# dschleef/schroedinger

Hardware: AMD Instinct MI355X
Metric: Mpix/s IIWT+OBMC decode, 2160p s16 (higher is better)
Workload: dtype s16

## Files before the change

schroedinger_amd/csrc/obmc.hip:

```cpp

#include "schro_hip_internal.h"
#include "obmc_common.h"
#include <algorithm>

namespace schro {
namespace {

constexpr int kThreads = 256;
constexpr int kTW = 64, kTH = 4;

template < int PC, bool SIMPLE >
__global__ __launch_bounds__ (kThreads)
void obmc_kernel (const ObmcJob * __restrict__ jobs, int njobs, uint32_t * __restrict__ overflow)
{
  __shared__ int s_wx[kMaxBlk], s_wy[kMaxBlk];

  const int bid = xcd_tile_id (blockIdx.x, gridDim.x);
  const ObmcJob job = jobs[find_job (jobs, njobs, bid)];
  const int t = bid - job.tile_base;
  const int tx = t % job.tiles_x, ty = t / job.tiles_x;
  const int tid = threadIdx.x;

  if (tid < job.xblen)
    s_wx[tid] = obmc_weight_1d (tid, job.xblen, job.xoff);
  if (tid >= 64 && tid - 64 < job.yblen)
    s_wy[tid - 64] = obmc_weight_1d (tid - 64, job.yblen, job.yoff);
  __syncthreads ();

  const int px = tx * kTW + (tid % kTW);
  const int py = ty * kTH + (tid / kTW);
  if (px >= job.w || py >= job.h)
    return;

  int bi[2], wxs[2], nx = 0;
  {
    int u = px + job.xoff;
    int i0 = u / job.xbsep, r = u - i0 * job.xbsep;
    int wa = 0, wb = 0;
    bool has_a = (r < 2 * job.xoff) && (i0 - 1 >= 0) && (i0 - 1 < job.nbx);
    bool has_b = (i0 < job.nbx);
    if (r < 2 * job.xoff) {
      wa = s_wx[r + job.xbsep];
      wb = s_wx[r];
      if (!has_a) { wb += wa; }
      if (!has_b) { wa += wb; }
    } else {
      wb = 8;
    }
    if (has_a) { bi[nx] = i0 - 1; wxs[nx] = wa; nx++; }
    if (has_b) { bi[nx] = i0; wxs[nx] = wb; nx++; }
  }
  int bj[2], wys[2], ny = 0;
  {
    int u = py + job.yoff;
    int j0 = u / job.ybsep, r = u - j0 * job.ybsep;
    int wa = 0, wb = 0;
    bool has_a = (r < 2 * job.yoff) && (j0 - 1 >= 0) && (j0 - 1 < job.nby);
    bool has_b = (j0 < job.nby);
    if (r < 2 * job.yoff) {
      wa = s_wy[r + job.ybsep];
      wb = s_wy[r];
      if (!has_a) { wb += wa; }
      if (!has_b) { wa += wb; }
    } else {
      wb = 8;
    }
    if (has_a) { bj[ny] = j0 - 1; wys[ny] = wa; ny++; }
    if (has_b) { bj[ny] = j0; wys[ny] = wb; ny++; }
  }

  const int prec = job.prec;
  const int expx = 32 << prec;
  const int max_fast_x = (job.w - job.xblen) * (1 << prec);
  const int max_fast_y = (job.h - job.yblen) * (1 << prec);
  const int wsum = job.w1 + job.w2;
  const bool noscale = (wsum == (1 << job.wbits));

  int acc = 0;
  for (int b = 0; b < ny; b++) {
    for (int a = 0; a < nx; a++) {
      const int i = bi[a], jj = bj[b];
      const uint8_t *mvp = job.mvs + (size_t) 20 * ((size_t) jj * job.nbx + i);
      const uint32_t flags = gload < uint32_t > (mvp);
      const uint32_t v01 = gload < uint32_t > (mvp + 12);
      const uint32_t v23 = gload < uint32_t > (mvp + 16);
      const int mode = flags & 3;
      const bool interior = i >= 1 && i < job.max_x_blocks && jj >= 1 && jj < job.max_y_blocks;
      const int bx = job.xbsep * i - job.xoff, by = job.ybsep * jj - job.yoff;
      const int wgt = wxs[a] * wys[b];
      int pred;

      if (mode == 0) {
        int dc = job.comp == 0 ? (int16_t) (v01 & 0xffff)
            : job.comp == 1 ? (int16_t) (v01 >> 16) : (int16_t) (v23 & 0xffff);
        pred = interior ? (int) (int16_t) (dc + 128) : (int) (uint8_t) (dc + 128);
        if (overflow && (unsigned) pred > 255u)
          __hip_atomic_store (overflow, 1u, __ATOMIC_RELAXED, __HIP_MEMORY_SCOPE_SYSTEM);
      } else {
        int val[2] = { 0, 0 };
#pragma unroll
        for (int r = 0; r < 2; r++) {
          if (!(mode & (r + 1)))
            continue;
          int dx = r == 0 ? (int16_t) (v01 & 0xffff) : (int16_t) (v01 >> 16);
          int dy = r == 0 ? (int16_t) (v23 & 0xffff) : (int16_t) (v23 >> 16);
          dx >>= job.mv_shift_x;
          dy >>= job.mv_shift_y;
          int fx = clampi (bx * (1 << prec) + dx, -expx, max_fast_x + expx - 1);
          int fy = clampi (by * (1 << prec) + dy, -expx, max_fast_y + expx - 1);
          int sx = fx + (px - bx) * (1 << prec);
          int sy = fy + (py - by) * (1 << prec);
          val[r] = fetch_ref < PC > (job.ref[r], job.ref_stride[r], job.w, job.h, sx, sy, prec, job.ref_ps, job.ref_cb);
        }
        if (mode == 3) {
          if constexpr (SIMPLE) {
            pred = (val[0] + val[1] + 1) >> 1;
          } else if (interior) {
            int16_t t1 = (int16_t) (val[0] * (int16_t) (job.w1 << (6 - job.wbits)));
            int16_t t2 = (int16_t) (val[1] * (int16_t) (job.w2 << (6 - job.wbits)));
            t1 = (int16_t) (t1 + t2);
            t1 = (int16_t) (t1 + 32);
            pred = (int16_t) (t1 >> 6);
          } else {
            int16_t t1 = (int16_t) (val[0] * job.w1);
            int16_t t2 = (int16_t) (val[1] * job.w2);
            t1 = (int16_t) (t1 + t2);
            t1 = (int16_t) (t1 + (int16_t) ((1 << job.wbits) >> 1));
            t1 = (int16_t) (t1 >> job.wbits);
            pred = clampi (t1, 0, 255);
          }
        } else {
          int s = val[mode - 1];
          if constexpr (SIMPLE) {
            pred = s;
          } else if (interior) {
            int16_t t1 = (int16_t) (s * (int16_t) (wsum << (6 - job.wbits)));
            t1 = (int16_t) (t1 + 32);
            pred = (int16_t) (t1 >> 6);
          } else if (noscale) {
            pred = s;
          } else {
            pred = (uint8_t) ((s * wsum + (1 << (job.wbits - 1))) >> job.wbits);
          }
        }
      }
      acc += pred * wgt;
    }
  }

  if (job.out_s16) {
    const int16_t t = (int16_t) ((int16_t) ((int16_t) acc - 8160) >> 6);
    gstore < int16_t > ((int16_t *) (job.out + (size_t) py * job.out_stride) + px, t);
    return;
  }
  int16_t t1 = (int16_t) ((int16_t) acc + 32);
  t1 = (int16_t) (t1 >> 6);
  int16_t res;
  if (!job.residual)
    res = 0;
  else if (job.res_bpp == 2)
    res = gload < int16_t > ((const int16_t *) ((const char *) job.residual
            + (size_t) py * job.residual_stride) + px);
  else
    res = (int16_t) gload < int32_t > ((const int32_t *) ((const char *) job.residual
            + (size_t) py * job.residual_stride) + px);
  t1 = (int16_t) (res + t1);
  gstore < uint8_t > (job.out + (size_t) py * job.out_stride + px, (uint8_t) clampi (t1, 0, 255));
}


constexpr int kFTW = 128, kFTH = 32;


constexpr int kAccStride = 136;

struct BlkInfo {
  int bx, by;
  int mode_dc;
  int fx[2], fy[2];
  int off[2];
  uint32_t wpk[2];
  int pad;
};

template < int PC >
__device__ __forceinline__ void
fetch4_inside (const uint8_t * __restrict__ p, int stride, uint32_t wpk, int *val)
{
  if constexpr (PC == 0) {
    uint32_t v = gload < u32_u > (p);
    val[0] = v & 0xff;
    val[1] = (v >> 8) & 0xff;
    val[2] = (v >> 16) & 0xff;
    val[3] = v >> 24;
  } else if constexpr (PC == 1) {
    const u32x2 q = gload < u32x2_u > (p);
    const uint64_t v = q.x | ((uint64_t) q.y << 32);
    val[0] = (int) (v & 0xff);
    val[1] = (int) ((v >> 16) & 0xff);
    val[2] = (int) ((v >> 32) & 0xff);
    val[3] = (int) ((v >> 48) & 0xff);
  } else {
    const u32x2 a = gload < u32x2_u > (p), b = gload < u32x2_u > (p + stride);
    const uint32_t alo = a.x, ahi = a.y, blo = b.x, bhi = b.y;
    val[0] = (int) (__builtin_amdgcn_udot4 (__builtin_amdgcn_perm (blo, alo, 0x05040100u), wpk, 8u, false) >> 4);
    val[1] = (int) (__builtin_amdgcn_udot4 (__builtin_amdgcn_perm (blo, alo, 0x07060302u), wpk, 8u, false) >> 4);
    val[2] = (int) (__builtin_amdgcn_udot4 (__builtin_amdgcn_perm (bhi, ahi, 0x05040100u), wpk, 8u, false) >> 4);
    val[3] = (int) (__builtin_amdgcn_udot4 (__builtin_amdgcn_perm (bhi, ahi, 0x07060302u), wpk, 8u, false) >> 4);
  }
}

constexpr int kAccMargin = 4;

struct TileCtx {
  int x_lo, x_hi, y_lo, y_hi;
  int xfold_hi, yfold_hi;
};

__device__ __forceinline__ void
acc_add_wrap (int *word, int high, int value)
{
  unsigned int old = __hip_atomic_load ((unsigned int *) word, __ATOMIC_RELAXED, __HIP_MEMORY_SCOPE_WORKGROUP), assumed;
  do {
    assumed = old;
    const unsigned int upd = high ? (assumed & 0xffffu) | ((assumed + ((unsigned int) value << 16)) & 0xffff0000u)
        : (assumed & 0xffff0000u) | ((assumed + (unsigned int) value) & 0xffffu);
    old = atomicCAS ((unsigned int *) word, assumed, upd);
  } while (old != assumed);
}

template < int PC >
__device__ __forceinline__ void
obmc_item_slow (const ObmcJob & job, const BlkInfo & bi, int row, int seg, const TileCtx & tc,
    const int *s_wx, const int *s_wy, int *acc, bool exact)
{
  const int prec = job.prec;
  const int y = bi.by + row, xs = bi.bx + 4 * seg;
  const int md = bi.mode_dc, mode = md & 3;
  int pred[4];
  if (mode == 0) {
    pred[0] = pred[1] = pred[2] = pred[3] = md >> 8;
  } else {
    int val[2][4];
    for (int r = 0; r < 2; r++) {
      if (!(mode & (r + 1)))
        continue;
      if constexpr (PC == 2) {
        const int sx = bi.fx[r] + 4 * seg * (1 << prec), sy = bi.fy[r] + row * (1 << prec);
        const int x8 = prec == 2 ? sx * 2 : sx, y8 = prec == 2 ? sy * 2 : sy;
        const int hx = x8 >> 2, hy = y8 >> 2, rx = x8 & 3, ry = y8 & 3;
        const int Y0 = clampi (hy, 0, 2 * job.h - 2), Y1 = clampi (hy + 1, 0, 2 * job.h - 2);
        int p[2][9];
#pragma unroll
        for (int j = 0; j < 9; j++) {
          const int X = clampi (hx + j, 0, 2 * job.w - 2);
          p[0][j] = gload < uint8_t > (job.ref[r] + hp_offset (X, Y0, job.ref_stride[r], job.ref_ps, job.ref_cb));
          p[1][j] = gload < uint8_t > (job.ref[r] + hp_offset (X, Y1, job.ref_stride[r], job.ref_ps, job.ref_cb));
        }
#pragma unroll
        for (int e = 0; e < 4; e++) {
          const int v = (4 - ry) * ((4 - rx) * p[0][2 * e] + rx * p[0][2 * e + 1])
              + ry * ((4 - rx) * p[1][2 * e] + rx * p[1][2 * e + 1]);
          val[r][e] = (v + 8) >> 4;
        }
      } else {
        for (int e = 0; e < 4; e++)
          val[r][e] = fetch_ref < PC > (job.ref[r], job.ref_stride[r], job.w, job.h,
              bi.fx[r] + (4 * seg + e) * (1 << prec), bi.fy[r] + row * (1 << prec), prec, job.ref_ps, job.ref_cb);
      }
    }
    for (int e = 0; e < 4; e++)
      pred[e] = mode == 3 ? (val[0][e] + val[1][e] + 1) >> 1 : (mode == 1 ? val[0][e] : val[1][e]);
  }
  int wy = s_wy[row];
  if (y < job.yoff)
    wy += s_wy[2 * job.yoff - row - 1];
  if (y >= tc.yfold_hi)
    wy += s_wy[2 * (job.yblen - job.yoff) - row - 1];
  const int yrel = y - tc.y_lo;
  int *arow = acc + (yrel & (kFTH / 2 - 1)) * kAccStride + kAccMargin - tc.x_lo;
  for (int e = 0; e < 4; e++) {
    const int x = xs + e, idx = 4 * seg + e;
    if (idx >= job.xblen)
      continue;
    int wx = s_wx[idx];
    if (x < job.xoff)
      wx += s_wx[2 * job.xoff - idx - 1];
    if (x >= tc.xfold_hi)
      wx += s_wx[2 * (job.xblen - job.xoff) - idx - 1];
    if (exact)
      acc_add_wrap (arow + x, yrel & (kFTH / 2), pred[e] * wx * wy);
    else
      atomicAdd (arow + x, (pred[e] * wx * wy) << (yrel & (kFTH / 2)));
  }
}

__device__ __forceinline__ void
obmc_finish (const ObmcJob & job, const int *acc, int tid, int x_lo, int y_lo, int x_hi, int y_hi)
{
  typedef short s16x2 __attribute__ ((ext_vector_type (2)));
  if (job.out_s16) {
    for (int it = tid; it < kFTH * kFTW; it += kThreads) {
      const int xx = it % kFTW, yy = it / kFTW;
      const int x = x_lo + xx, y = y_lo + yy;
      if (y >= y_hi || x >= x_hi)
        continue;
      const int a = acc[(yy & (kFTH / 2 - 1)) * kAccStride + kAccMargin + xx] >> (yy & (kFTH / 2));
      gstore < int16_t > ((int16_t *) (job.out + (size_t) y * job.out_stride) + x, (int16_t) ((int16_t) ((int16_t) a - 8160) >> 6));
    }
    return;
  }
  const bool fast = job.res_bpp == 2 && x_hi - x_lo == kFTW
      && ((((uintptr_t) job.residual) | (uintptr_t) job.residual_stride) & 15) == 0
      && ((((uintptr_t) job.out) | (uintptr_t) job.out_stride) & 7) == 0;
  if (fast) {
    for (int it = tid; it < (kFTH / 2) * (kFTW / 8); it += kThreads) {
      const int g = it & (kFTW / 8 - 1), yy = it >> 4;
      static_assert (kFTW / 8 == 16, "8-pixel groups per tile row");
      const int x = x_lo + 8 * g;
      const int4 *ap = reinterpret_cast < const int4 * >(acc + yy * kAccStride + kAccMargin + 8 * g);
      const int4 a0 = ap[0], a1 = ap[1];
#pragma unroll
      for (int half = 0; half < 2; half++) {
        const int y = y_lo + yy + half * (kFTH / 2);
        if (y >= y_hi)
          continue;
        const uint32_t sel = half ? 0x07060302u : 0x05040100u;
        const u32x4 r = job.residual ? gload < u32x4 > ((const char *) job.residual + (size_t) y * job.residual_stride + 2 * x)
            : (u32x4) { 0u, 0u, 0u, 0u };
        const uint32_t av[4] = {
          __builtin_amdgcn_perm ((uint32_t) a0.y, (uint32_t) a0.x, sel),
          __builtin_amdgcn_perm ((uint32_t) a0.w, (uint32_t) a0.z, sel),
          __builtin_amdgcn_perm ((uint32_t) a1.y, (uint32_t) a1.x, sel),
          __builtin_amdgcn_perm ((uint32_t) a1.w, (uint32_t) a1.z, sel)
        };
        const uint32_t rv[4] = { r.x, r.y, r.z, r.w };
        uint32_t t[4];
#pragma unroll
        for (int k = 0; k < 4; k++) {
          s16x2 v = (__builtin_bit_cast (s16x2, av[k]) + (short) 32) >> 6;
          v = v + __builtin_bit_cast (s16x2, rv[k]);
          v = __builtin_elementwise_min (__builtin_elementwise_max (v, (s16x2) (short) 0), (s16x2) (short) 255);
          t[k] = __builtin_bit_cast (uint32_t, v);
        }
        u32x2 o;
        o.x = __builtin_amdgcn_perm (t[1], t[0], 0x06040200u);
        o.y = __builtin_amdgcn_perm (t[3], t[2], 0x06040200u);
        gstore < u32x2 > (job.out + (size_t) y * job.out_stride + x, o);
      }
    }
    return;
  }
  for (int it = tid; it < kFTH * kFTW / 4; it += kThreads) {
    const int g = it % (kFTW / 4), yy = it / (kFTW / 4);
    const int x = x_lo + 4 * g, y = y_lo + yy;
    if (y >= y_hi || x >= x_hi)
      continue;
    const int *ap = acc + (yy & (kFTH / 2 - 1)) * kAccStride + kAccMargin + 4 * g;
    const int hs = yy & (kFTH / 2);
    const int av[4] = { ap[0] >> hs, ap[1] >> hs, ap[2] >> hs, ap[3] >> hs };
    const char *rrow = (const char *) job.residual + (size_t) y * job.residual_stride;
    uint8_t *orow = job.out + (size_t) y * job.out_stride + x;
    __attribute__ ((aligned (8))) int16_t res[4];
    const bool full = x + 4 <= job.w;
    if (!job.residual) {
      res[0] = res[1] = res[2] = res[3] = 0;
    } else if (job.res_bpp == 2) {
      const int16_t *rp = (const int16_t *) rrow + x;
      if (full && (((uintptr_t) rp) & 7) == 0) {
        *reinterpret_cast < u32x2 * >(res) = gload < u32x2 > (rp);
      } else {
        for (int e = 0; e < 4; e++)
          res[e] = x + e < job.w ? gload < int16_t > (rp + e) : (int16_t) 0;
      }
    } else {
      const int32_t *rp = (const int32_t *) rrow + x;
      for (int e = 0; e < 4; e++)
        res[e] = x + e < job.w ? (int16_t) gload < int32_t > (rp + e) : (int16_t) 0;
    }
    uint32_t pk = 0;
#pragma unroll
    for (int e = 0; e < 4; e++) {
      int16_t t1 = (int16_t) ((int16_t) av[e] + 32);
      t1 = (int16_t) (t1 >> 6);
      t1 = (int16_t) (res[e] + t1);
      pk |= (uint32_t) clampi (t1, 0, 255) << (8 * e);
    }
    if (full && (((uintptr_t) orow) & 3) == 0) {
      gstore < uint32_t > (orow, pk);
    } else {
      for (int e = 0; e < 4 && x + e < job.w; e++)
        gstore < uint8_t > (orow + e, (uint8_t) (pk >> (8 * e)));
    }
  }
}


constexpr int kItemBlkCap = 192;
constexpr int kItemCap = 1536;
constexpr int kItemWCap = 256;

struct __attribute__ ((aligned (16))) HotBlk {
  int y, x;
  int mode_dc;
  int rows;
  int off[2];
  uint32_t wpk[2];
  int ya[2];
};

struct ItemLane {
  int slot, seg;
  int seg_bytes;
  int tw3;
  bool active;
};

template < int PC >
__device__ __forceinline__ void
hp_predict4 (const ObmcJob & job, int r, int off_r, int ya, int row, int seg, uint32_t wpk, int *val)
{
  static_assert (PC >= 1, "plain references are linear");
  const int stride = job.ref_stride[r];
  const int ps = job.ref_ps;
  const int xp = ((off_r & 0xffff) + 4 * seg) << ps, px = (off_r >> 16) & 1, py = (off_r >> 17) & 1;
  const int y = ya + row;
  const uint32_t pick = job.ref_cb ? 0x07050301u : 0x06040200u;
  auto load4 = [&](const uint8_t * p) {
    if (ps) {
      const u32x2 q = gload < u32x2_u > (p);
      return __builtin_amdgcn_perm (q.y, q.x, pick);
    }
    return gload < u32_u > (p);
  };
  const uint8_t *a = job.ref[r] + hp_row_offset (y, stride) + hp_col_offset (xp) + (px + 2 * py) * 128;
  const uint32_t A = load4 (a);
  if constexpr (PC == 1) {
    val[0] = A & 0xff;
    val[1] = (A >> 8) & 0xff;
    val[2] = (A >> 16) & 0xff;
    val[3] = A >> 24;
    (void) wpk;
  } else {
    const int dB = px ? (1 << ps) - 128 : 128;
    const uint8_t *c = job.ref[r] + hp_row_offset (y + py, stride) + hp_col_offset (xp) + (px + 2 * (py ^ 1)) * 128;
    const uint32_t B = load4 (a + dB), C = load4 (c), D = load4 (c + dB);
#pragma unroll
    for (int e = 0; e < 4; e++) {
      const uint32_t sel = 0x0c0c0000u | (uint32_t) e | ((uint32_t) (4 + e) << 8);
      const uint32_t t = __builtin_amdgcn_perm (B, A, sel), u = __builtin_amdgcn_perm (D, C, sel);
      val[e] = (int) (__builtin_amdgcn_udot4 (__builtin_amdgcn_perm (u, t, 0x05040100u), wpk, 8u, false) >> 4);
    }
  }
}

template < int PC, int CLS, bool EXACT >
__device__ __forceinline__ void
item_pass (const ObmcJob & job, const ItemLane & il, const uint16_t * s_item, const HotBlk * s_hot,
    const uint32_t * s_w4, int nseg, int *acc, int i0, int hi)
{
  constexpr int kStep = PC == 0 ? 1 : 2;
  const int it = i0 + il.slot;
  const int e = s_item[min (it, hi - 1)];
  const HotBlk & hb = s_hot[e & 0xff];
  const int row = e >> 8;
  const int yrel = hb.y + row, xrel = hb.x + 4 * il.seg;
  const uint32_t w4 = s_w4[__umul24 (row, nseg) + il.seg];
  int v0[4], v1[4];
  if constexpr (CLS == 3) {
    v0[0] = v0[1] = v0[2] = v0[3] = v1[0] = v1[1] = v1[2] = v1[3] = hb.mode_dc >> 8;
  } else {
    constexpr int r0 = CLS == 2 ? 1 : 0;
    if constexpr (PC == 0) {
      fetch4_inside < PC > (job.ref[r0] + (hb.off[r0] + (row * kStep) * job.ref_stride[r0] + il.seg_bytes),
          job.ref_stride[r0], hb.wpk[r0], v0);
      if constexpr (CLS == 0)
        fetch4_inside < PC > (job.ref[1] + (hb.off[1] + (row * kStep) * job.ref_stride[1] + il.seg_bytes),
            job.ref_stride[1], hb.wpk[1], v1);
    } else {
      hp_predict4 < PC > (job, r0, hb.off[r0], hb.ya[r0], row, il.seg, hb.wpk[r0], v0);
      if constexpr (CLS == 0)
        hp_predict4 < PC > (job, 1, hb.off[1], hb.ya[1], row, il.seg, hb.wpk[1], v1);
    }
    if constexpr (CLS != 0) {
#pragma unroll
      for (int k = 0; k < 4; k++)
        v1[k] = v0[k];
    }
  }
  if (il.active && it < hi && (unsigned) (xrel + 3) < (unsigned) il.tw3) {
    int *ap = acc + (__umul24 (yrel & (kFTH / 2 - 1), kAccStride) + kAccMargin + xrel);
    const int hs = yrel & (kFTH / 2);
    static_assert (kFTH / 2 == 16, "the high half of an accumulator word is bit 16 up");
#pragma unroll
    for (int k = 0; k < 4; k++) {
      const int pred = CLS == 0 ? (v0[k] + v1[k] + 1) >> 1 : v0[k];
      const int v = __mul24 (pred, (int) ((w4 >> (8 * k)) & 0xff));
      if constexpr (EXACT)
        acc_add_wrap (ap + k, hs, v);
      else
        atomicAdd (ap + k, v << hs);
    }
  }
}

template < int PC, int CLS >
__device__ __forceinline__ void
item_class (const ObmcJob & job, const ItemLane & il, const uint16_t * s_item, const HotBlk * s_hot,
    const uint32_t * s_w4, int nseg, int *acc, int first, int hi, int stride, bool exact)
{
  if (exact) {
    for (int i0 = first; i0 < hi; i0 += stride)
      item_pass < PC, CLS, true > (job, il, s_item, s_hot, s_w4, nseg, acc, i0, hi);
  } else {
    for (int i0 = first; i0 < hi; i0 += stride)
      item_pass < PC, CLS, false > (job, il, s_item, s_hot, s_w4, nseg, acc, i0, hi);
  }
}

template < int PC >
__global__ __launch_bounds__ (kThreads) __attribute__ ((amdgpu_waves_per_eu (5, 5)))
void obmc_item_kernel (const ObmcJob * __restrict__ jobs, int njobs, const uint32_t * __restrict__ order,
    uint32_t * __restrict__ overflow)
{
  __shared__ __attribute__ ((aligned (16))) int acc[(kFTH / 2) * kAccStride];
  __shared__ int s_wx[kMaxBlk], s_wy[kMaxBlk];
  __shared__ HotBlk s_hot[kItemBlkCap];
  __shared__ uint16_t s_item[kItemCap];
  __shared__ uint32_t s_w4[kItemWCap];
  __shared__ uint16_t s_start[kThreads + 2];
  __shared__ int s_cnt[8];
  __shared__ int s_wide;

  const int bid = xcd_tile_id (blockIdx.x, gridDim.x);
  const uint32_t entry = order ? __builtin_amdgcn_readfirstlane (gload < uint32_t > (order + bid)) : 0u;
  const ObmcJob job = jobs[order ? (int) (entry >> 16) : find_job (jobs, njobs, bid)];
  const int t = order ? (int) (entry & 0xffffu) : bid - job.tile_base;
  const int ty = mdiv (t, job.tiles_x, job.m_tiles_x), tx = t - ty * job.tiles_x;
  const int tid = threadIdx.x, lane = tid & 63, wave = tid >> 6;
  const int x_lo = tx * kFTW, y_lo = ty * kFTH;
  const int x_hi = min (x_lo + kFTW, job.w), y_hi = min (y_lo + kFTH, job.h);

  static_assert (((kFTH / 2) * kAccStride) % 4 == 0, "accumulator tile is cleared 16 bytes at a time");
  for (int it = tid; it < (kFTH / 2) * kAccStride / 4; it += kThreads)
    reinterpret_cast < int4 * >(acc)[it] = make_int4 (0, 0, 0, 0);
  if (tid < job.xblen)
    s_wx[tid] = obmc_weight_1d (tid, job.xblen, job.xoff);
  if (tid >= 64 && tid - 64 < job.yblen)
    s_wy[tid - 64] = obmc_weight_1d (tid - 64, job.yblen, job.yoff);

  const int xblen = job.xblen, yblen = job.yblen, xbsep = job.xbsep, ybsep = job.ybsep;
  const int xoff = job.xoff, yoff = job.yoff, prec = job.prec;
  const int i_lo = max (0, mdiv (x_lo + xoff - xblen + 2 * xbsep, xbsep, job.m_xbsep) - 1);
  const int i_hi = min (job.nbx - 1, mdiv (x_hi - 1 + xoff, xbsep, job.m_xbsep));
  const int j_lo = max (0, mdiv (y_lo + yoff - yblen + 2 * ybsep, ybsep, job.m_ybsep) - 1);
  const int j_hi = min (job.nby - 1, mdiv (y_hi - 1 + yoff, ybsep, job.m_ybsep));
  const int nbi = i_hi - i_lo + 1, nbj = j_hi - j_lo + 1;
  const int nblk = nbi > 0 && nbj > 0 ? nbi * nbj : 0;
  const uint32_t m_nbi = nbi > 1 && nbi <= 1024 ? kDivMagic.m[nbi] : 0u;
  const int xfold_hi = job.nbx * xbsep - xoff, yfold_hi = job.nby * ybsep - yoff;
  const int gw = PC == 0 ? job.w - 1 : 2 * job.w - 2;
  const int gh = PC == 0 ? job.h - 1 : 2 * job.h - 2;
  constexpr int kStep = PC == 0 ? 1 : 2;
  const int nseg = job.nseg, lpi = job.lpi;
  const int IPW = job.ipw, chunk_cap = job.chunk_cap;
  ItemLane il;
  il.slot = mdiv (lane, lpi, job.m_lpi);
  const int sub = lane - il.slot * lpi;
  il.seg = min (sub, nseg - 1);
  il.seg_bytes = il.seg * (4 * kStep);
  il.tw3 = x_hi - x_lo + 3;
  il.active = il.slot < IPW && sub < nseg;
  TileCtx tc;
  tc.x_lo = x_lo;
  tc.x_hi = x_hi;
  tc.y_lo = y_lo;
  tc.y_hi = y_hi;
  tc.xfold_hi = xfold_hi;
  tc.yfold_hi = yfold_hi;
  __syncthreads ();
  for (int i = tid; i < yblen * nseg && i < kItemWCap; i += kThreads) {
    const int r = mdiv (i, nseg, job.m_nseg), sg = i - r * nseg;
    uint32_t w = 0;
#pragma unroll
    for (int k = 0; k < 4; k++)
      if (4 * sg + k < xblen)
        w |= (uint32_t) (s_wx[4 * sg + k] * s_wy[r]) << (8 * k);
    s_w4[i] = w;
  }

  bool exact = false;
  for (int chunk0 = 0; chunk0 < nblk; chunk0 += chunk_cap) {
    const int nb = min (chunk_cap, nblk - chunk0);
    if (tid < 8)
      s_cnt[tid] = 0;
    if (tid == 8)
      s_wide = 0;
    __syncthreads ();
    HotBlk info;
    int key = 0, rank = 0;
    const bool have = tid < nb;
    if (have) {
      const int blk = chunk0 + tid;
      const int bj = nbi == 1 ? blk : nbi <= 1024 ? (int) __umulhi ((uint32_t) blk, m_nbi) : blk / nbi;
      const int i = i_lo + (blk - bj * nbi), jj = j_lo + bj;
      const uint8_t *mvp = job.mvs + (size_t) 20 * ((size_t) jj * job.nbx + i);
      const uint32_t flags = gload < uint32_t > (mvp);
      const uint32_t v01 = gload < uint32_t > (mvp + 12);
      const uint32_t v23 = gload < uint32_t > (mvp + 16);
      const int bx = xbsep * i - xoff, by = ybsep * jj - yoff;
      info.x = bx - x_lo;
      info.y = by - y_lo;
      const int mode = flags & 3;
      const bool interior = i >= 1 && i < job.max_x_blocks && jj >= 1 && jj < job.max_y_blocks;
      int dc = job.comp == 0 ? (int16_t) (v01 & 0xffff)
          : job.comp == 1 ? (int16_t) (v01 >> 16) : (int16_t) (v23 & 0xffff);
      int p = interior ? (int) (int16_t) (dc + 128) : (int) (uint8_t) (dc + 128);
      int md = mode | (p << 8);
#pragma unroll
      for (int r = 0; r < 2; r++) {
        int fx, fy;
        mv_origin (job, bx, by, v01, v23, r, &fx, &fy);
        int gx0, gy0, gx1, gy1;
        uint32_t wpk = 0;
        if constexpr (PC == 2) {
          const int x8 = prec == 2 ? fx * 2 : fx, y8 = prec == 2 ? fy * 2 : fy;
          const int rx = x8 & 3, ry = y8 & 3;
          gx0 = x8 >> 2;
          gy0 = y8 >> 2;
          gx1 = gx0 + 2 * (nseg * 4 - 1) + 1;
          gy1 = gy0 + 2 * (yblen - 1) + 1;
          wpk = (uint32_t) ((4 - ry) * (4 - rx)) | ((uint32_t) ((4 - ry) * rx) << 8)
              | ((uint32_t) (ry * (4 - rx)) << 16) | ((uint32_t) (ry * rx) << 24);
        } else {
          gx0 = fx;
          gy0 = fy;
          gx1 = gx0 + kStep * (nseg * 4 - 1);
          gy1 = gy0 + kStep * (yblen - 1);
        }
        bool inside = gx0 >= 0 && gy0 >= 0 && gx1 <= gw && gy1 <= gh;
        if (!inside)
          md |= 4 << r;
        if constexpr (PC == 0) {
          info.off[r] = inside ? gy0 * job.ref_stride[r] + gx0 : 0;
          info.ya[r] = 0;
        } else {
          info.off[r] = inside ? ((gx0 >> 1) + kHpApron) | ((gx0 & 1) << 16) | ((gy0 & 1) << 17) : 0;
          info.ya[r] = inside ? gy0 >> 1 : 0;
        }
        info.wpk[r] = wpk;
      }
      info.mode_dc = md;
      const int ra = max (0, -info.y), rb = min (yblen, y_hi - by);
      info.rows = ra | ((rb - ra) << 8);
      const bool clamped = ((md >> 2) & md & 3) != 0;
      const bool fold = by < yoff || by + yblen > yfold_hi || bx < xoff || bx + nseg * 4 > xfold_hi;
      const bool wide_dc = mode == 0 && (unsigned) p > 255u;
      if (wide_dc) {
        s_wide = 1;
        if (overflow)
          __hip_atomic_store (overflow, 1u, __ATOMIC_RELAXED, __HIP_MEMORY_SCOPE_SYSTEM);
      }
      key = (clamped || fold || wide_dc || yblen * nseg > kItemWCap) ? 4 : (mode == 3 ? 0 : (mode == 0 ? 3 : mode));
      if (key == 4) {
        int fx, fy;
        mv_origin (job, bx, by, v01, v23, 0, &fx, &fy);
        info.off[0] = fx;
        info.off[1] = fy;
        mv_origin (job, bx, by, v01, v23, 1, &fx, &fy);
        info.wpk[0] = (uint32_t) fx;
        info.wpk[1] = (uint32_t) fy;
      }
      rank = atomicAdd (&s_cnt[key], 1);
    }
    __syncthreads ();
    if (s_wide && !exact) {
      exact = true;
      if (chunk0 > 0) {
        __syncthreads ();
        for (int it = tid; it < (kFTH / 2) * kAccStride / 4; it += kThreads)
          reinterpret_cast < int4 * >(acc)[it] = make_int4 (0, 0, 0, 0);
        chunk0 = -chunk_cap;
        continue;
      }
    }
    int cbase[6];
    cbase[0] = 0;
#pragma unroll
    for (int k = 0; k < 5; k++)
      cbase[k + 1] = cbase[k] + s_cnt[k];
    if (have) {
      int base = 0;
#pragma unroll
      for (int k = 0; k < 5; k++)
        base = key == k ? cbase[k] : base;
      s_hot[base + rank] = info;
    }
    __syncthreads ();
    int nrows = tid < cbase[4] ? ((s_hot[tid].rows >> 8) & 0xff) : 0, incl = nrows;
#pragma unroll
    for (int d = 1; d < 64; d <<= 1) {
      const int up = __shfl_up (incl, d);
      if (lane >= d)
        incl += up;
    }
    if (lane == 63)
      s_cnt[4 + wave] = incl;
    __syncthreads ();
    {
#pragma unroll
      for (int w = 0; w < kThreads / 64 - 1; w++)
        incl += wave > w ? s_cnt[4 + w] : 0;
      const int start = incl - nrows;
      s_start[tid] = (uint16_t) start;
      if (tid == kThreads - 1)
        s_start[kThreads] = (uint16_t) incl;
      if (tid < cbase[4]) {
        const int ra = s_hot[tid].rows & 0xff;
        for (int r = 0; r < nrows; r++)
          s_item[start + r] = (uint16_t) (tid | ((ra + r) << 8));
      }
    }
    __syncthreads ();

    const int first = wave * IPW, stride = (kThreads / 64) * IPW;
    item_class < PC, 0 > (job, il, s_item, s_hot, s_w4, nseg, acc, s_start[cbase[0]] + first, s_start[cbase[1]], stride, exact);
    item_class < PC, 1 > (job, il, s_item, s_hot, s_w4, nseg, acc, s_start[cbase[1]] + first, s_start[cbase[2]], stride, exact);
    item_class < PC, 2 > (job, il, s_item, s_hot, s_w4, nseg, acc, s_start[cbase[2]] + first, s_start[cbase[3]], stride, exact);
    item_class < PC, 3 > (job, il, s_item, s_hot, s_w4, nseg, acc, s_start[cbase[3]] + first, s_start[cbase[4]], stride, exact);

    {
      const int per_block = yblen * nseg;
      const uint32_t m_per_block = div_magic (per_block);
      const int nslow = cbase[5] - cbase[4];
      for (int item = tid; item < nslow * per_block; item += kThreads) {
        const int b = mdiv (item, per_block, m_per_block);
        const int rem = item - b * per_block;
        const int r2 = mdiv (rem, nseg, job.m_nseg), s2 = rem - r2 * nseg;
        const HotBlk & hb = s_hot[cbase[4] + b];
        BlkInfo bi;
        bi.bx = hb.x + x_lo;
        bi.by = hb.y + y_lo;
        const int y = bi.by + r2, xs = bi.bx + 4 * s2;
        if (y < y_lo || y >= y_hi || xs + 3 < x_lo || xs >= x_hi)
          continue;
        bi.mode_dc = hb.mode_dc;
        bi.fx[0] = hb.off[0];
        bi.fy[0] = hb.off[1];
        bi.fx[1] = (int) hb.wpk[0];
        bi.fy[1] = (int) hb.wpk[1];
        obmc_item_slow < PC > (job, bi, r2, s2, tc, s_wx, s_wy, acc, exact);
      }
    }
  }
  __syncthreads ();
  obmc_finish (job, acc, tid, x_lo, y_lo, x_hi, y_hi);
}

template < int PC >
int
launch_one (hipStream_t stream, const ObmcJob * d_jobs, int njobs, int total_tiles, int variant,
    const uint32_t * d_order, uint32_t * overflow)
{
  static const int lds_pad = SCHRO_ENV ("SCHRO_HIP_OBMC_LDS_PAD") ? atoi (SCHRO_ENV ("SCHRO_HIP_OBMC_LDS_PAD")) : 0;
  if (variant == 1)
    SCHRO_LAUNCH ((obmc_item_kernel < PC >), dim3 (total_tiles), dim3 (kThreads), lds_pad, stream,
        d_jobs, njobs, d_order, overflow);
  else
    SCHRO_LAUNCH ((obmc_kernel < PC, false >), dim3 (total_tiles), dim3 (kThreads), 0,
        stream, d_jobs, njobs, overflow);
  hipError_t e = hipGetLastError ();
  if (e != hipSuccess)
    return set_error (SCHRO_HIP_EDEVICE, "obmc launch: %s", hipGetErrorString (e));
  return 0;
}

}

void
obmc_item_geometry (ObmcJob * j)
{
  const int nseg = (j->xblen + 3) >> 2;
  const int lpi = nseg;
  j->nseg = nseg;
  j->lpi = lpi;
  j->ipw = 64 / lpi;
  j->chunk_cap = std::min (kItemBlkCap, kItemCap / std::min (j->yblen, kFTH));
  j->m_tiles_x = div_magic (j->tiles_x);
  j->m_xbsep = div_magic (j->xbsep);
  j->m_ybsep = div_magic (j->ybsep);
  j->m_nseg = div_magic (nseg);
  j->m_lpi = div_magic (lpi);
  j->m_xramp = div_magic (2 * j->xoff - 1);
  j->m_yramp = div_magic (2 * j->yoff - 1);
}

void
obmc_tiles (int variant, int w, int h, int xoff, int *tiles_x, int *tiles_y)
{
  (void) xoff;
  if (variant >= 1) {
    const int tw = variant >= 3 ? obmc_row_tile_width (variant == 4) : kFTW;
    const int th = variant >= 3 ? obmc_row_tile_height () : kFTH;
    *tiles_x = (w + tw - 1) / tw;
    *tiles_y = (h + th - 1) / th;
  } else {
    *tiles_x = (w + kTW - 1) / kTW;
    *tiles_y = (h + kTH - 1) / kTH;
  }
}

int
launch_obmc (hipStream_t stream, const ObmcJob * d_jobs, int njobs, int total_tiles, int prec,
    int variant, const uint32_t * d_order, uint32_t * overflow)
{
  switch (prec == 0 ? 0 : (prec == 1 ? 1 : 2)) {
    case 0: return launch_one < 0 > (stream, d_jobs, njobs, total_tiles, variant, d_order, overflow);
    case 1: return launch_one < 1 > (stream, d_jobs, njobs, total_tiles, variant, d_order, overflow);
    default: return launch_one < 2 > (stream, d_jobs, njobs, total_tiles, variant, d_order, overflow);
  }
}

}
```

schroedinger_amd/csrc/obmc_row.hip:

```cpp

#include "obmc_row_body.h"

namespace schro {
namespace {

SCHRO_ROW_KERNEL (obmc_row_kernel_2_1, 6, 2, 1)
SCHRO_ROW_KERNEL (obmc_row_kernel_2_2, 6, 2, 2)
SCHRO_ROW_KERNEL (obmc_row_kernel_3_1, 7, 3, 1)
SCHRO_ROW_KERNEL (obmc_row_kernel_3_2, 5, 3, 2)
SCHRO_ROW_KERNEL (obmc_row_kernel_4_1, 6, 4, 1)
SCHRO_ROW_KERNEL (obmc_row_kernel_4_2, 5, 4, 2)
SCHRO_ROW_KERNEL (obmc_row_kernel_uv_2, 5, 2, 1, true)
SCHRO_ROW_KERNEL (obmc_row_kernel_uv_3, 7, 3, 1, true)
SCHRO_ROW_KERNEL (obmc_row_kernel_uv_4, 6, 4, 1, true)
SCHRO_ROW_KERNEL (obmc_row_kernel_p_2_1, 6, 2, 1, false, kRTH, true)
SCHRO_ROW_KERNEL (obmc_row_kernel_p_3_1, 8, 3, 1, false, kRTH, true)
#ifdef SCHRO_HIP_EXPERIMENTS
SCHRO_ROW_KERNEL (obmc_row_kernel_p_3_1_pad, 8, 3, 1, false, kRTH, true, 1, 1, false, true)
#endif
SCHRO_ROW_KERNEL (obmc_row_kernel_p_4_1, 7, 4, 1, false, kRTH, true)
SCHRO_ROW_KERNEL (obmc_row_kernel_p_uv_2, 5, 2, 1, true, kRTH, true)
SCHRO_ROW_KERNEL (obmc_row_kernel_p_uv_3, 8, 3, 1, true, kRTH, true)
SCHRO_ROW_KERNEL (obmc_row_kernel_p_uv_4, 7, 4, 1, true, kRTH, true)
SCHRO_ROW_KERNEL (obmc_row_kernel_h2_3_1, 6, 3, 1, false, kRTH, false, 1, 2)
SCHRO_ROW_KERNEL (obmc_row_kernel_h2_uv_3, 6, 3, 1, true, kRTH, false, 1, 2)
SCHRO_ROW_KERNEL (obmc_row_kernel_p_h2_3_1, 7, 3, 1, false, kRTH, true, 1, 2)
SCHRO_ROW_KERNEL (obmc_row_kernel_p_h2_uv_3, 6, 3, 1, true, kRTH, true, 1, 2)
SCHRO_ROW_KERNEL (obmc_row_kernel_h2_4_1, 5, 4, 1, false, kRTH, false, 1, 2)
SCHRO_ROW_KERNEL (obmc_row_kernel_h2_uv_4, 5, 4, 1, true, kRTH, false, 1, 2)
SCHRO_ROW_KERNEL (obmc_row_kernel_p_h2_4_1, 6, 4, 1, false, kRTH, true, 1, 2)
SCHRO_ROW_KERNEL (obmc_row_kernel_p_h2_uv_4, 6, 4, 1, true, kRTH, true, 1, 2)

SCHRO_ROW_KERNEL (obmc_row_kernel_w_3_1, 6, 3, 1, false, kRTH, false, 1, 1, true)
SCHRO_ROW_KERNEL (obmc_row_kernel_w_uv_3, 6, 3, 1, true, kRTH, false, 1, 1, true)
SCHRO_ROW_KERNEL (obmc_row_kernel_w_p_3_1, 7, 3, 1, false, kRTH, true, 1, 1, true)
SCHRO_ROW_KERNEL (obmc_row_kernel_w_p_uv_3, 7, 3, 1, true, kRTH, true, 1, 1, true)
SCHRO_ROW_KERNEL (obmc_row_kernel_w_2_1, 5, 2, 1, false, kRTH, false, 1, 1, true)
SCHRO_ROW_KERNEL (obmc_row_kernel_w_4_1, 6, 4, 1, false, kRTH, false, 1, 1, true)
SCHRO_ROW_KERNEL (obmc_row_kernel_w_uv_2, 5, 2, 1, true, kRTH, false, 1, 1, true)
SCHRO_ROW_KERNEL (obmc_row_kernel_w_uv_4, 6, 4, 1, true, kRTH, false, 1, 1, true)
SCHRO_ROW_KERNEL (obmc_row_kernel_w_h2_3_1, 6, 3, 1, false, kRTH, false, 1, 2, true)
SCHRO_ROW_KERNEL (obmc_row_kernel_w_h2_uv_3, 6, 3, 1, true, kRTH, false, 1, 2, true)
SCHRO_ROW_KERNEL (obmc_row_kernel_w_h2_4_1, 6, 4, 1, false, kRTH, false, 1, 2, true)
SCHRO_ROW_KERNEL (obmc_row_kernel_w_h2_uv_4, 6, 4, 1, true, kRTH, false, 1, 2, true)

constexpr RowEntry kHalf[] = {
  ROW_ENTRY (obmc_row_kernel_2_1), ROW_ENTRY (obmc_row_kernel_2_2), ROW_ENTRY (obmc_row_kernel_3_1), ROW_ENTRY (obmc_row_kernel_3_2),
  ROW_ENTRY (obmc_row_kernel_4_1), ROW_ENTRY (obmc_row_kernel_4_2),
  ROW_ENTRY (obmc_row_kernel_uv_2), ROW_ENTRY (obmc_row_kernel_uv_3), ROW_ENTRY (obmc_row_kernel_uv_4),
  ROW_ENTRY (obmc_row_kernel_p_2_1), ROW_ENTRY (obmc_row_kernel_p_3_1), ROW_ENTRY (obmc_row_kernel_p_4_1),
  ROW_ENTRY (obmc_row_kernel_p_uv_2), ROW_ENTRY (obmc_row_kernel_p_uv_3), ROW_ENTRY (obmc_row_kernel_p_uv_4),
  ROW_ENTRY (obmc_row_kernel_h2_3_1), ROW_ENTRY (obmc_row_kernel_h2_uv_3), ROW_ENTRY (obmc_row_kernel_p_h2_3_1), ROW_ENTRY (obmc_row_kernel_p_h2_uv_3),
  ROW_ENTRY (obmc_row_kernel_h2_4_1), ROW_ENTRY (obmc_row_kernel_h2_uv_4), ROW_ENTRY (obmc_row_kernel_p_h2_4_1), ROW_ENTRY (obmc_row_kernel_p_h2_uv_4),
  ROW_ENTRY (obmc_row_kernel_w_3_1), ROW_ENTRY (obmc_row_kernel_w_uv_3), ROW_ENTRY (obmc_row_kernel_w_p_3_1), ROW_ENTRY (obmc_row_kernel_w_p_uv_3),
  ROW_ENTRY (obmc_row_kernel_w_2_1), ROW_ENTRY (obmc_row_kernel_w_4_1), ROW_ENTRY (obmc_row_kernel_w_uv_2), ROW_ENTRY (obmc_row_kernel_w_uv_4),
  ROW_ENTRY (obmc_row_kernel_w_h2_3_1), ROW_ENTRY (obmc_row_kernel_w_h2_uv_3), ROW_ENTRY (obmc_row_kernel_w_h2_4_1), ROW_ENTRY (obmc_row_kernel_w_h2_uv_4),
};
constexpr RowTable kHalfTable = { kHalf, (int) std::size (kHalf) };
static_assert (row_table_ok (kHalfTable, 1), "obmc_row.hip: one kernel per form");
static_assert (row_find (kHalfTable, RowForm { 1, 3, 1, 2, true, true }) == obmc_row_kernel_w_h2_3_1
    && row_find (kHalfTable, RowForm { 1, 2, 2, 1, true, false }) == obmc_row_kernel_2_2 && !row_find (kHalfTable, RowForm { 1, 3, 2, 1, false, true }),
    "obmc_row.hip: a prediction_only launch without a kernel of its form takes the residual form's; no kernel of two weighted planes");

}

RowTable
obmc_row_table_half ()
{
  return kHalfTable;
}

static RowKernel
row_kernel (const RowForm & f)
{
#ifdef SCHRO_HIP_EXPERIMENTS
  static const bool pad = SCHRO_ENV ("SCHRO_HIP_OBMC_PAD") && atoi (SCHRO_ENV ("SCHRO_HIP_OBMC_PAD")) != 0;
  if (pad && f == obmc_row_kernel_p_3_1_pad_form)
    return obmc_row_kernel_p_3_1_pad;
#endif
  return row_find (f.kind == 0 ? obmc_row_table_plain () : f.kind == 3 ? obmc_row_table_eighth () : obmc_row_table_half (), f);
}

bool
obmc_row_has_kernel (const RowForm & form)
{
  return row_kernel (form) != nullptr;
}

int
launch_obmc_row (hipStream_t stream, const ObmcJob * d_jobs, int njobs, int total_tiles, const RowForm & form,
    const uint32_t * d_order, uint32_t * overflow, const uint32_t * d_wtabs)
{
  const RowKernel k = row_kernel (form);
  if (!k)
    return set_error (SCHRO_HIP_EINVAL, "obmc (row): reference kind %d, %d dwords per row x %d segments x %d planes unsupported", form.kind,
        form.nd, form.ns, form.np);
  static const int lds_pad = SCHRO_ENV ("SCHRO_HIP_OBMC_LDS_PAD") ? atoi (SCHRO_ENV ("SCHRO_HIP_OBMC_LDS_PAD")) : 0;
  SCHRO_LAUNCH (k, dim3 (total_tiles), dim3 (kRThreads), (size_t) lds_pad, stream, d_jobs, njobs, d_order, overflow, d_wtabs);
  hipError_t e = hipGetLastError ();
  if (e != hipSuccess)
    return set_error (SCHRO_HIP_EDEVICE, "obmc (row) launch: %s", hipGetErrorString (e));
  return 0;
}

struct RowCaps {
  int tw, blk, item;
};
template < int ND, bool UV, int NS > constexpr RowCaps kRowCaps = { RowGeo < ND, UV, NS >::kTW, RowGeo < ND, UV, NS >::kBlk, RowGeo < ND, UV, NS >::kItem };
template < bool UV, int NS > constexpr RowCaps kRowCapsNd[3] = { kRowCaps < 2, UV, NS >, kRowCaps < 3, UV, NS >, kRowCaps < 4, UV, NS > };
static RowCaps
row_caps (int nd, int ns, bool uv)
{
  static constexpr const RowCaps *caps[2][2] = { { kRowCapsNd < false, 1 >, kRowCapsNd < false, 2 > }, { kRowCapsNd < true, 1 >, kRowCapsNd < true, 2 > } };
  return caps[uv][ns - 1][nd - 2];
}

RowForm
obmc_row_form (const ObmcJob & j, bool uv, bool nores)
{
  const int ps = uv ? 1 : 0;
  int ns = 1;
  if (j.ref_ps != (j.prec == 0 ? 0 : ps))
    return {};
  if (j.prec < 0 || j.prec > 3 || (j.xblen & 1) || j.xblen < 2 || j.yblen > 32)
    return {};
  if (j.w1 < 0 || j.w2 < 0 || j.wbits < 0 || j.wbits > 6 || j.w1 + j.w2 != (1 << j.wbits))
    return {};
  int seg_bytes = j.xblen << ps;
  if (seg_bytes > 16) {
    if (seg_bytes > 32 || (seg_bytes & 3))
      return {};
    ns = 2;
    seg_bytes /= 2;
  }
  if (((std::max (j.w, j.h) + 32) << j.prec) > 32767)
    return {};
  if (j.prec == 0) {
    if (((((uintptr_t) j.ref[0]) | ((uintptr_t) j.ref[1])) & 3) || ((j.ref_stride[0] | j.ref_stride[1]) & 3) || j.ref_stride[0] < j.w
        || j.ref_stride[1] < j.w || j.w < 4)
      return {};
    if (uv && (!j.ref_b[0] || !j.ref_b[1] || ((((uintptr_t) j.ref_b[0]) | ((uintptr_t) j.ref_b[1])) & 3)))
      return {};
  } else {
    if ((((uintptr_t) j.ref[0]) | ((uintptr_t) j.ref[1])) & 127)
      return {};
    if (((j.ref_stride[0] | j.ref_stride[1]) & 511) || j.ref_stride[0] < hp_chunks (j.w, ps) * 512 || j.ref_stride[1] < hp_chunks (j.w, ps) * 512)
      return {};
  }
  const int need = (seg_bytes + 3) / 4, nd = need <= 2 ? 2 : need;
  const RowForm form = { j.prec == 0 ? 0 : j.prec == 3 ? 3 : 1, nd, uv ? 3 : 1, ns, nores, j.w1 != 1 || j.wbits != 1 };
  if (!row_kernel (form))
    return {};
  const RowCaps caps = row_caps (nd, ns, uv);
  if ((long long) ((j.w + caps.tw - 1) / caps.tw) * ((j.h + kRTH - 1) / kRTH) > 0xffff)
    return {};
  const int nbi = ((caps.tw - 1 + j.xblen - 1) / j.xbsep + 1) * ns, nbj = (kRTH - 1 + j.yblen - 1) / j.ybsep + 1;
  const int rows_col = std::min (kRTH * ((j.yblen + j.ybsep - 1) / j.ybsep), kRTH + (kRTH / j.ybsep + 2) * 2 * j.yoff);
  if (nbi > 255 || nbi * nbj > caps.blk || nbi * rows_col > caps.item)
    return {};
  return form;
}

int
obmc_row_weight_words (int nd, int ns)
{
  const int wrow = 2 * nd * ns;
  return 32 * wrow + 4 * (ns == 1 ? 8 : wrow) + 128 + (ns == 1 ? 16 : 32) + 32;
}
static_assert (RowGeo < 3, false, 2 >::kWTab == 32 * 12 + 48 + 128 + 32 + 32 && RowGeo < 4, true, 2 >::kWTab == 32 * 16 + 64 + 128 + 32 + 32
    && RowGeo < 3, true >::kWTab == 64 * 3 + 32 + 128 + 16 + 32, "obmc_row_weight_words");

void
obmc_row_weight_table (const ObmcJob & j, int nd, int ns, bool uv, uint32_t * out)
{
  auto ramp = [](int x, int offset) { return offset == 1 ? (x == 0 ? 3 : 5) : 1 + (6 * x + offset - 1) / (2 * offset - 1); };
  auto weight = [&](int i, int blen, int offset) {
    if (offset == 0)
      return 8;
    if (i < 2 * offset)
      return ramp (i, offset);
    if (blen - 1 - i < 2 * offset)
      return ramp (blen - 1 - i, offset);
    return 8;
  };
  const int wrow = 2 * nd * ns, xf = ns == 1 ? 8 : wrow, wxn = ns == 1 ? 16 : 32;
  int wx[32] = { 0 }, wy[32] = { 0 };
  for (int i = 0; i < j.xblen && i < wxn; i++)
    wx[i] = weight (i, j.xblen, j.xoff);
  for (int i = 0; i < j.yblen && i < 32; i++)
    wy[i] = weight (i, j.yblen, j.yoff);
  auto folded = [](const int *w1, int idx, int blen, int bsep, int off, int type) {
    if (idx >= blen)
      return 0;
    int w = w1[idx];
    if ((type & 1) && idx < 2 * off)
      w += w1[2 * off - idx - 1];
    if ((type & 2) && idx >= bsep)
      w += w1[2 * (blen - off) - idx - 1];
    return w;
  };
  const int wcap = 32 * wrow;
  const int seg_words = ns == 1 ? wrow : 2 * nd, seg_units = ns == 1 ? (uv ? j.xblen : j.xblen >> 1) : (uv ? j.xblen / 2 : j.xblen >> 2);
  auto unit_of = [&](int pr) {
    const int seg = pr / seg_words, q = pr - seg * seg_words;
    return q < seg_units ? seg * seg_units + q : -1;
  };
  for (int i = 0; i < wcap; i++) {
    const int r = i / wrow, u = unit_of (i - r * wrow);
    uint32_t v = 0;
    if (r < j.yblen && u >= 0) {
      if (uv)
        v = (uint32_t) (wx[u] * wy[r]) * 0x00010001u;
      else
        v = (uint32_t) (wx[2 * u] * wy[r]) | ((uint32_t) (wx[2 * u + 1] * wy[r]) << 16);
    }
    out[i] = v;
  }
  for (int t = 0; t < 4 * xf; t++) {
    const int type = t / xf, pr = t - type * xf;
    const int u = ns == 1 ? pr : unit_of (pr);
    out[wcap + t] = u < 0 ? 0u : uv ? (uint32_t) folded (wx, u, j.xblen, j.xbsep, j.xoff, type) * 0x00010001u
        : (uint32_t) folded (wx, 2 * u, j.xblen, j.xbsep, j.xoff, type) | ((uint32_t) folded (wx, 2 * u + 1, j.xblen, j.xbsep, j.xoff, type) << 16);
  }
  const int fy = wcap + 4 * xf;
  for (int t = 0; t < 128; t++)
    out[fy + t] = (uint32_t) folded (wy, t & 31, j.yblen, j.ybsep, j.yoff, t >> 5);
  for (int i = 0; i < wxn; i++)
    out[fy + 128 + i] = (uint32_t) wx[i];
  for (int i = 0; i < 32; i++)
    out[fy + 128 + wxn + i] = (uint32_t) wy[i];
}

void
obmc_row_tile_record (const ObmcJob & j, bool uv, int ns, int tx, int ty, uint32_t * rec)
{
  const int tw = obmc_row_tile_width (uv);
  const int x_lo = tx * tw, y_lo = ty * kRTH, x_hi = std::min (x_lo + tw, j.w), y_hi = std::min (y_lo + kRTH, j.h);
  const int i_lo = std::max (0, (x_lo + j.xoff - j.xblen + 2 * j.xbsep) / j.xbsep - 1);
  const int i_hi = std::min (j.nbx - 1, (x_hi - 1 + j.xoff) / j.xbsep);
  const int j_lo = std::max (0, (y_lo + j.yoff - j.yblen + 2 * j.ybsep) / j.ybsep - 1);
  const int j_hi = std::min (j.nby - 1, (y_hi - 1 + j.yoff) / j.ybsep);
  const int nbi = std::max (0, std::min (255, (i_hi - i_lo + 1) * ns)), nbj = std::max (0, std::min (255, j_hi - j_lo + 1));
  const uint32_t m16 = nbi > 1 ? (65536u + (uint32_t) nbi - 1u) / (uint32_t) nbi : 0u;
  rec[0] = (uint32_t) x_lo | ((uint32_t) y_lo << 16);
  rec[1] = (uint32_t) i_lo | ((uint32_t) j_lo << 16);
  rec[2] = (uint32_t) nbi | ((uint32_t) nbj << 8) | (m16 << 16);
}

int
obmc_row_tile_height ()
{
  return kRTH;
}

int
obmc_row_tile_width (bool uv)
{
  return row_caps (3, 1, uv).tw;
}

}
```

schroedinger_amd/csrc/obmc_row_body.h:

```cpp

#pragma once

#include "schro_hip_internal.h"
#include "obmc_common.h"
#include <algorithm>
#include <cstdlib>

namespace schro {
namespace {

constexpr int kRThreads = 256;
constexpr int kRTH = 32;
template < int ND, bool UV, int NS = 1 > struct RowGeo {
  static constexpr int kTW = UV ? 64 : 128;
  static constexpr int kMargin = UV ? (ND <= 3 && NS == 1 ? 5 : 8) : (ND <= 2 ? 8 : 16);
  static constexpr int kAccW = UV ? (ND <= 3 && NS == 1 ? 75 : 81) : (ND <= 2 ? 73 : 85);
  static constexpr int kBlk = ND <= 2 ? 344 : (NS > 1 ? (UV ? 208 : 144) : UV ? (ND == 3 ? 180 : 192) : 128) * kRTH / 32,
      kItem = ND <= 2 ? 1792 : (NS > 1 ? 1664 : UV ? (ND == 3 ? 960 : 1152) : (ND == 3 ? 1024 : 1152)) * kRTH / 32;
  static constexpr int kWRow = 2 * ND * NS;
  static constexpr int kWCap = 32 * kWRow;
  static constexpr int kXF = NS == 1 ? 8 : kWRow, kWxN = NS == 1 ? 16 : 32;
  static constexpr bool kPadBlk = UV || ND > 2;
  static constexpr int kWFoldY = kWCap + 4 * kXF, kWRampX = kWFoldY + 128, kWRampY = kWRampX + kWxN;
  static constexpr int kWTab = kWRampY + 32;
};
constexpr int kRBoth = 0, kRRef0 = 1, kRRef1 = 2, kRDc = 3, kREdge = 4, kRRim = 5;
constexpr int kRSlots = 16 + 4 + 4 + 3;
__host__ __device__ constexpr int
row_slot_base (int cls)
{
  return cls == kRBoth ? 0 : cls == kRRef0 ? 16 : cls == kRRef1 ? 20 : cls == kRDc ? 24 : cls == kREdge ? 25 : 26;
}

typedef unsigned short u16x2 __attribute__ ((ext_vector_type (2)));
typedef short s16x2 __attribute__ ((ext_vector_type (2)));

struct __attribute__ ((aligned (4))) RowRef {
  int base;
  uint32_t ydb;
  int dci;
};

template < bool PAD > struct alignas (PAD ? 4 : 8) RowBlkT {
  int16_t y, x;
  uint32_t fr;
  RowRef r[2];
  uint32_t pad[PAD ? 1 : 0];
};
static_assert (sizeof (RowBlkT < true >) == 36 && sizeof (RowBlkT < false >) == 32, "block records: an odd number of words / r03's");

template < typename B >
__device__ __forceinline__ uint32_t
blk_flags (const B & hb)
{
  return hb.fr >> 16;
}

template < typename B >
__device__ __forceinline__ uint32_t
blk_ry (const B & hb, int r)
{
  return (hb.fr >> (16 + 6 + r)) & 1u;
}

template < typename B >
__device__ __forceinline__ int
blk_dc (const B & hb, int pl)
{
  return pl ? hb.r[0].base >> 16 : (int) (int16_t) hb.r[0].base;
}


struct __attribute__ ((aligned (8))) PlaneIO {
  const uint8_t *ref[2];
  const void *residual;
  uint8_t *out;
  int residual_stride, out_stride;
};

__device__ __forceinline__ uint32_t
lerp1 (uint32_t a, uint32_t b)
{
  return __builtin_amdgcn_lerp (a, b, 0x01010101u);
}

__device__ __forceinline__ void
acc_add_exact (uint32_t * word, int high, uint32_t value)
{
  unsigned int old = __hip_atomic_load (word, __ATOMIC_RELAXED, __HIP_MEMORY_SCOPE_WORKGROUP), assumed;
  do {
    assumed = old;
    const unsigned int upd = high ? (assumed & 0xffffu) | ((assumed + (value << 16)) & 0xffff0000u)
        : (assumed & 0xffff0000u) | ((assumed + value) & 0xffffu);
    old = atomicCAS (word, assumed, upd);
  } while (old != assumed);
}

template < typename G, bool UV >
__device__ __forceinline__ uint32_t *
acc_word (uint32_t * acc, int par, int x, int y, int *half)
{
  if constexpr (UV) {
    *half = 0;
    return acc + y * G::kAccW + (x + G::kMargin);
  } else {
    const int idx = x + G::kMargin + par;
    *half = idx & 1;
    return acc + y * G::kAccW + (idx >> 1);
  }
}

template < int ND > struct RawRun {
  uint32_t c[ND + 1];
  uint32_t sh;
};

#if defined (SCHRO_HIP_EXPERIMENTS) && defined (SCHRO_ROW_GATHER_AUX)
constexpr int kGatherAux = SCHRO_ROW_GATHER_AUX;
#else
constexpr int kGatherAux = 0;
#endif

template < int ND >
__device__ __forceinline__ void
issue_run (__amdgpu_buffer_rsrc_t ref, uint32_t off, RawRun < ND > &r)
{
  const uint32_t al = off & ~3u;
  r.sh = off & 3u;
  if constexpr (ND == 1) {
    const u32x2 q = __builtin_amdgcn_raw_buffer_load_b64 (ref, (int) al, 0, kGatherAux);
    r.c[0] = q.x;
    r.c[1] = q.y;
  } else if constexpr (ND == 2) {
    typedef uint32_t u32x3 __attribute__ ((ext_vector_type (3)));
    const u32x3 q = __builtin_amdgcn_raw_buffer_load_b96 (ref, (int) al, 0, kGatherAux);
    r.c[0] = q.x;
    r.c[1] = q.y;
    r.c[2] = q.z;
  } else if constexpr (ND == 3) {
    const u32x4 q = __builtin_amdgcn_raw_buffer_load_b128 (ref, (int) al, 0, kGatherAux);
    r.c[0] = q.x;
    r.c[1] = q.y;
    r.c[2] = q.z;
    r.c[3] = q.w;
  } else {
    const u32x4 q = __builtin_amdgcn_raw_buffer_load_b128 (ref, (int) al, 0, kGatherAux);
    const u32x2 q2 = __builtin_amdgcn_raw_buffer_load_b64 (ref, (int) al + 16, 0, kGatherAux);
    r.c[0] = q.x;
    r.c[1] = q.y;
    r.c[2] = q.z;
    r.c[3] = q.w;
    r.c[4] = q2.x;
  }
}

template < int ND >
__device__ __forceinline__ void
align_run (const RawRun < ND > &r, uint32_t * d)
{
#pragma unroll
  for (int k = 0; k < ND; k++)
    d[k] = __builtin_amdgcn_alignbyte (r.c[k + 1], r.c[k], r.sh);
}

__device__ __forceinline__ uint32_t
row_ofs (uint32_t y, uint32_t stride)
{
  return __umul24 (y >> 2, stride) + ((y & 3u) << 5);
}

template < int ND, bool ABS = false, bool W = false >
__device__ __forceinline__ void
predict_row (const ObmcJob & job, __amdgpu_buffer_rsrc_t ref, uint32_t stride, const RowRef & rr, uint32_t ry, int row, uint32_t * out)
{
  const int dB = (int) rr.ydb >> 16;
  uint32_t offA, offC = 0;
  bool any_b, any_c;
  if constexpr (ABS) {
    const int hy = (int) (int16_t) (rr.ydb & 0xffffu) + 2 * row, gh = 2 * job.h - 2;
    const uint32_t Y0 = (uint32_t) clampi (hy, 0, gh), Y1 = (uint32_t) clampi (hy + (int) ry, 0, gh);
    offA = (uint32_t) rr.base + ((Y0 & 1u) << 8) + row_ofs (Y0 >> 1, stride);
    offC = (uint32_t) rr.base + ((Y1 & 1u) << 8) + row_ofs (Y1 >> 1, stride);
    any_b = any_c = true;
  } else {
    const uint32_t y = (rr.ydb & 0xffffu) + (uint32_t) row;
    offA = (uint32_t) rr.base + row_ofs (y, stride);
    any_b = __ballot (dB != 0) != 0;
    any_c = __ballot ((W ? rr.dci & ~0xf0 : rr.dci) != 0) != 0;
    if (any_c)
      offC = (uint32_t) (rr.base + (rr.dci >> 16)) + row_ofs (y + ((uint32_t) rr.dci & 1u), stride);
  }
  RawRun < ND > qa, qb, qc, qd;
  issue_run < ND > (ref, offA, qa);
  if (any_b)
    issue_run < ND > (ref, offA + (uint32_t) dB, qb);
  if (any_c) {
    issue_run < ND > (ref, offC, qc);
    if (any_b)
      issue_run < ND > (ref, offC + (uint32_t) dB, qd);
  }
  uint32_t a[ND];
  align_run < ND > (qa, a);
  if constexpr (W) {
    const uint32_t rx = ((uint32_t) rr.dci >> 4) & 3u, rw = ((uint32_t) rr.dci >> 6) & 3u;
    const uint32_t w00 = (4u - rw) * (4u - rx), w01 = (4u - rw) * rx, w10 = rw * (4u - rx), w11 = rw * rx;
    uint32_t lo[ND], hi[ND];
#pragma unroll
    for (int k = 0; k < ND; k++) {
      lo[k] = __umul24 (__builtin_amdgcn_perm (0u, a[k], 0x0c010c00u), w00) + 0x00080008u;
      hi[k] = __umul24 (__builtin_amdgcn_perm (0u, a[k], 0x0c030c02u), w00) + 0x00080008u;
    }
    auto add_tap = [&] (const RawRun < ND > &q, uint32_t w) {
      uint32_t t[ND];
      align_run < ND > (q, t);
#pragma unroll
      for (int k = 0; k < ND; k++) {
        lo[k] += __umul24 (__builtin_amdgcn_perm (0u, t[k], 0x0c010c00u), w);
        hi[k] += __umul24 (__builtin_amdgcn_perm (0u, t[k], 0x0c030c02u), w);
      }
    };
    if (any_b)
      add_tap (qb, w01);
    if (any_c) {
      add_tap (qc, w10);
      if (any_b)
        add_tap (qd, w11);
    }
#pragma unroll
    for (int k = 0; k < ND; k++)
      out[k] = __builtin_amdgcn_perm (hi[k] >> 4, lo[k] >> 4, 0x06040200u);
    return;
  }
  if (!any_c) {
    if (!any_b) {
#pragma unroll
      for (int k = 0; k < ND; k++)
        out[k] = a[k];
    } else {
      uint32_t b[ND];
      align_run < ND > (qb, b);
#pragma unroll
      for (int k = 0; k < ND; k++)
        out[k] = lerp1 (a[k], b[k]);
    }
  } else if (!any_b) {
    uint32_t c[ND];
    align_run < ND > (qc, c);
#pragma unroll
    for (int k = 0; k < ND; k++)
      out[k] = lerp1 (a[k], c[k]);
  } else {
    uint32_t b[ND], c[ND], d[ND];
    align_run < ND > (qb, b);
    align_run < ND > (qc, c);
    align_run < ND > (qd, d);
#pragma unroll
    for (int k = 0; k < ND; k++) {
      const uint32_t h0 = lerp1 (a[k], b[k]), h1 = lerp1 (c[k], d[k]);
      out[k] = __builtin_amdgcn_lerp (h0, h1, ~((a[k] ^ b[k]) | (c[k] ^ d[k])));
    }
  }
}

template < int ND > struct TapRuns {
  RawRun < ND > qa, qb, qc, qd;
  bool any_b, any_c;
};

template < int ND >
__device__ __forceinline__ void
issue_taps (__amdgpu_buffer_rsrc_t ref, uint32_t stride, const RowRef & rr, int row, TapRuns < ND > &t)
{
  const int dB = (int) rr.ydb >> 16;
  const uint32_t y = (rr.ydb & 0xffffu) + (uint32_t) row;
  const uint32_t offA = (uint32_t) rr.base + row_ofs (y, stride);
  t.any_b = __ballot (dB != 0) != 0;
  t.any_c = __ballot (rr.dci != 0) != 0;
  issue_run < ND > (ref, offA, t.qa);
  if (t.any_b)
    issue_run < ND > (ref, offA + (uint32_t) dB, t.qb);
  if (t.any_c) {
    const uint32_t offC = (uint32_t) (rr.base + (rr.dci >> 16)) + row_ofs (y + ((uint32_t) rr.dci & 1u), stride);
    issue_run < ND > (ref, offC, t.qc);
    if (t.any_b)
      issue_run < ND > (ref, offC + (uint32_t) dB, t.qd);
  }
}

template < int ND >
__device__ __forceinline__ void
finish_taps (const TapRuns < ND > &t, uint32_t * out)
{
  uint32_t a[ND];
  align_run < ND > (t.qa, a);
  if (!t.any_c) {
    if (!t.any_b) {
#pragma unroll
      for (int k = 0; k < ND; k++)
        out[k] = a[k];
    } else {
      uint32_t b[ND];
      align_run < ND > (t.qb, b);
#pragma unroll
      for (int k = 0; k < ND; k++)
        out[k] = lerp1 (a[k], b[k]);
    }
  } else if (!t.any_b) {
    uint32_t c[ND];
    align_run < ND > (t.qc, c);
#pragma unroll
    for (int k = 0; k < ND; k++)
      out[k] = lerp1 (a[k], c[k]);
  } else {
    uint32_t b[ND], c[ND], d[ND];
    align_run < ND > (t.qb, b);
    align_run < ND > (t.qc, c);
    align_run < ND > (t.qd, d);
#pragma unroll
    for (int k = 0; k < ND; k++) {
      const uint32_t h0 = lerp1 (a[k], b[k]), h1 = lerp1 (c[k], d[k]);
      out[k] = __builtin_amdgcn_lerp (h0, h1, ~((a[k] ^ b[k]) | (c[k] ^ d[k])));
    }
  }
}

template < int ND >
__device__ __forceinline__ void
predict_row_plain (__amdgpu_buffer_rsrc_t ref, uint32_t stride, const RowRef & rr, int row, uint32_t * out)
{
  RawRun < ND > qa;
  issue_run < ND > (ref, (uint32_t) rr.base + __umul24 ((rr.ydb & 0xffffu) + (uint32_t) row, stride), qa);
  align_run < ND > (qa, out);
}

template < int ND >
__device__ __forceinline__ void
predict_row_plain_abs (const ObmcJob & job, __amdgpu_buffer_rsrc_t ref, uint32_t stride, const RowRef & rr, int row, uint32_t * out)
{
  const int Y = clampi ((int) (int16_t) (rr.ydb & 0xffffu) + row, 0, job.h - 1);
  const uint32_t rofs = __umul24 ((uint32_t) Y, stride);
  u32x2 q[ND];
  uint32_t sh[ND];
  int d[ND];
#pragma unroll
  for (int k = 0; k < ND; k++) {
    const int t = rr.base + 4 * k, xs = clampi (t, 0, job.w - 4);
    const uint32_t off = rofs + (uint32_t) xs;
    d[k] = t - xs;
    sh[k] = off & 3u;
    q[k] = __builtin_amdgcn_raw_buffer_load_b64 (ref, (int) (off & ~3u), 0, 0);
  }
#pragma unroll
  for (int k = 0; k < ND; k++) {
    const uint32_t v = __builtin_amdgcn_alignbyte (q[k].y, q[k].x, sh[k]);
    const uint32_t sel = (uint32_t) clampi (d[k], 0, 3) | ((uint32_t) clampi (d[k] + 1, 0, 3) << 8)
        | ((uint32_t) clampi (d[k] + 2, 0, 3) << 16) | ((uint32_t) clampi (d[k] + 3, 0, 3) << 24);
    out[k] = __builtin_amdgcn_perm (0u, v, sel);
  }
}

template < int ND >
__device__ __forceinline__ void
interleave_uv (const uint32_t * u, const uint32_t * v, uint32_t * out)
{
#pragma unroll
  for (int k = 0; k < ND; k++)
    out[k] = __builtin_amdgcn_perm (v[k >> 1], u[k >> 1], (k & 1) ? 0x07030602u : 0x05010400u);
}

template < int ND, int RK, bool ABS, bool UV >
__device__ __forceinline__ void
predict (const ObmcJob & job, __amdgpu_buffer_rsrc_t ref, __amdgpu_buffer_rsrc_t ref_b, uint32_t stride, const RowRef & rr, uint32_t ry, int row,
    uint32_t * out)
{
  if constexpr (RK == 0 && UV) {
    constexpr int NH = (ND + 1) / 2;
    uint32_t u[NH], v[NH];
    if constexpr (ABS) {
      predict_row_plain_abs < NH > (job, ref, stride, rr, row, u);
      predict_row_plain_abs < NH > (job, ref_b, stride, rr, row, v);
    } else {
      RawRun < NH > qu, qv;
      const uint32_t off = (uint32_t) rr.base + __umul24 ((rr.ydb & 0xffffu) + (uint32_t) row, stride);
      issue_run < NH > (ref, off, qu);
      issue_run < NH > (ref_b, off, qv);
      align_run < NH > (qu, u);
      align_run < NH > (qv, v);
    }
    interleave_uv < ND > (u, v, out);
  } else if constexpr (RK == 0) {
    if constexpr (ABS)
      predict_row_plain_abs < ND > (job, ref, stride, rr, row, out);
    else
      predict_row_plain < ND > (ref, stride, rr, row, out);
  } else if constexpr (RK == 3) {
    predict_row < ND, ABS, true > (job, ref, stride, rr, ABS ? (((uint32_t) rr.dci & 0xc0u) ? 1u : 0u) : 0u, row, out);
  } else {
    predict_row < ND, ABS > (job, ref, stride, rr, ry, row, out);
  }
}

__device__ __forceinline__ uint32_t
blend_weighted (uint32_t a, uint32_t b, uint32_t w1, uint32_t w2, uint32_t round2, uint32_t bits)
{
  const uint32_t lo = __umul24 (__builtin_amdgcn_perm (0u, a, 0x0c010c00u), w1) + __umul24 (__builtin_amdgcn_perm (0u, b, 0x0c010c00u), w2) + round2;
  const uint32_t hi = __umul24 (__builtin_amdgcn_perm (0u, a, 0x0c030c02u), w1) + __umul24 (__builtin_amdgcn_perm (0u, b, 0x0c030c02u), w2) + round2;
  return __builtin_amdgcn_perm (hi >> bits, lo >> bits, 0x06040200u);
}

struct RowRefs {
  __amdgpu_buffer_rsrc_t rsrc[2];
  uint32_t stride[2];
  __amdgpu_buffer_rsrc_t rsrc_b[2];
};

template < bool UV, typename B >
__device__ __forceinline__ uint32_t
dc_bytes (const B & hb, int pl)
{
  if constexpr (UV)
    return ((uint32_t) (blk_dc (hb, 0) & 0xff) | ((uint32_t) (blk_dc (hb, 1) & 0xff) << 8)) * 0x00010001u;
  else
    return (uint32_t) (blk_dc (hb, pl) & 0xff) * 0x01010101u;
}

template < int ND, bool UV, int CLS, bool EXACT, int RK, int NS, bool WP, bool PAD = false >
__device__ __forceinline__ void
row_pass (const ObmcJob & job, int pl, const RowRefs & refs, const uint16_t * s_item, const RowBlkT < RowGeo < ND, UV, NS >::kPadBlk > *s_hot,
    const uint32_t * s_wp, uint32_t * acc, int par, int it, int hi)
{
  typedef RowGeo < ND, UV, NS > G;
  const int e = s_item[min (it, hi - 1)];
  const auto & hb = s_hot[e & 0x1ff];
  const int row = PAD ? (e >> 9) & 63 : e >> 9;
  constexpr bool weighted = WP;
  const uint32_t wround = WP ? (uint32_t) ((1 << job.wbits) >> 1) * 0x00010001u : 0u;
  uint32_t p[ND];
  if constexpr (CLS == kRDc) {
#pragma unroll
    for (int k = 0; k < ND; k++)
      p[k] = dc_bytes < UV > (hb, pl);
  } else if constexpr (CLS == kREdge) {
    uint32_t p1[ND];
    predict < ND, RK, true, UV > (job, refs.rsrc[0], refs.rsrc_b[0], refs.stride[0], hb.r[0], blk_ry (hb, 0), row, p);
    __builtin_amdgcn_sched_barrier (0);
    predict < ND, RK, true, UV > (job, refs.rsrc[1], refs.rsrc_b[1], refs.stride[1], hb.r[1], blk_ry (hb, 1), row, p1);
    const uint32_t mode = blk_flags (hb) & 3u;
    const uint32_t dc = dc_bytes < UV > (hb, pl);
    const uint32_t m0 = (mode & 1u) ? 0xffffffffu : 0u, m1 = (mode & 2u) ? 0xffffffffu : 0u;
#pragma unroll
    for (int k = 0; k < ND; k++) {
      const uint32_t a = (p[k] & m0) | (p1[k] & ~m0), b = (p1[k] & m1) | (p[k] & ~m1);
      p[k] = mode ? (weighted ? blend_weighted (a, b, (uint32_t) job.w1, (uint32_t) job.w2, wround, (uint32_t) job.wbits) : lerp1 (a, b)) : dc;
    }
  } else if constexpr (CLS == kRBoth) {
    uint32_t p1[ND];
#if defined (SCHRO_HIP_EXPERIMENTS) && defined (SCHRO_ROW_BOTH_AT_ONCE)
    if constexpr (RK == 1) {
      TapRuns < ND > t0, t1;
      issue_taps < ND > (refs.rsrc[0], refs.stride[0], hb.r[0], row, t0);
      issue_taps < ND > (refs.rsrc[1], refs.stride[1], hb.r[1], row, t1);
      __builtin_amdgcn_sched_barrier (0);
      finish_taps < ND > (t0, p);
      finish_taps < ND > (t1, p1);
    } else
#endif
    {
    predict < ND, RK, false, UV > (job, refs.rsrc[0], refs.rsrc_b[0], refs.stride[0], hb.r[0], 0u, row, p);
    __builtin_amdgcn_sched_barrier (0);
    predict < ND, RK, false, UV > (job, refs.rsrc[1], refs.rsrc_b[1], refs.stride[1], hb.r[1], 0u, row, p1);
    }
    if (weighted) {
#pragma unroll
      for (int k = 0; k < ND; k++)
        p[k] = blend_weighted (p[k], p1[k], (uint32_t) job.w1, (uint32_t) job.w2, wround, (uint32_t) job.wbits);
    } else {
#pragma unroll
      for (int k = 0; k < ND; k++)
        p[k] = lerp1 (p[k], p1[k]);
    }
  } else {
    constexpr int r = CLS == kRRef1 ? 1 : 0;
    predict < ND, RK, false, UV > (job, refs.rsrc[r], refs.rsrc_b[r], refs.stride[r], hb.r[r], 0u, row, p);
  }
  if (it >= hi || (PAD && (e & 0x8000)))
    return;
#if defined (SCHRO_HIP_EXPERIMENTS) && defined (SCHRO_ROW_PASS_LOADS_ONLY)
  {
    uint32_t x = 0;
#pragma unroll
    for (int k = 0; k < ND; k++)
      x ^= p[k];
    atomicAdd (acc + (it & 1023), x);
    return;
  }
#endif
  int half;
  uint32_t *aw = acc_word < G, UV > (acc, par, hb.x, hb.y + row, &half);
  const int seg_w = NS > 1 ? (int) ((blk_flags (hb) >> 8) & 1u) * 2 * ND : 0;
  uint32_t w[2 * ND];
  if constexpr (CLS == kREdge) {
    const uint32_t fb = (blk_flags (hb) >> 2) & 15u;
    const uint32_t *wxf = s_wp + G::kWCap + G::kXF * (fb >> 2) + seg_w, *wyf = s_wp + G::kWFoldY + 32 * (fb & 3u);
    const uint32_t wy2 = wyf[row] * 0x00010001u;
#pragma unroll
    for (int k = 0; k < 2 * ND; k++)
      w[k] = __builtin_bit_cast (uint32_t, (u16x2) (__builtin_bit_cast (u16x2, wxf[k]) * __builtin_bit_cast (u16x2, wy2)));
  } else {
    const u32x2 *wp = reinterpret_cast < const u32x2 * >(s_wp + G::kWRow * row + seg_w);
#pragma unroll
    for (int k = 0; k < ND; k++) {
      const u32x2 q = wp[k];
      w[2 * k] = q.x;
      w[2 * k + 1] = q.y;
    }
  }
#pragma unroll
  for (int k = 0; k < 2 * ND; k++) {
    const uint32_t px = __builtin_amdgcn_perm (0u, p[k >> 1], (k & 1) ? 0x0c030c02u : 0x0c010c00u);
    const uint32_t v = __builtin_bit_cast (uint32_t, (u16x2) (__builtin_bit_cast (u16x2, px) * __builtin_bit_cast (u16x2, w[k])));
    if constexpr (EXACT) {
      acc_add_exact (aw + k, 0, v & 0xffffu);
      acc_add_exact (aw + k, 1, v >> 16);
    } else {
      atomicAdd (aw + k, v);
    }
  }
}

template < int ND, bool UV, int CLS, int RK, int NS, bool WP, bool PAD = false >
__device__ __forceinline__ void
row_class (const ObmcJob & job, int pl, const RowRefs & refs, const uint16_t * s_item, const RowBlkT < RowGeo < ND, UV, NS >::kPadBlk > *s_hot,
    const uint32_t * s_wp, uint32_t * acc, int par, int lo, int hi, bool exact, int *turn)
{
  const int wave = __builtin_amdgcn_readfirstlane ((int) (threadIdx.x >> 6)), lane = threadIdx.x & 63;
  const int npass = (hi - lo + 63) >> 6;
  constexpr int kWaves = kRThreads / 64;
  const int k0 = (wave - *turn) & (kWaves - 1);
  *turn = (*turn + npass) & (kWaves - 1);
#if defined (SCHRO_HIP_EXPERIMENTS) && defined (SCHRO_ROW_PRIO_PASS)
  __builtin_amdgcn_s_setprio (SCHRO_ROW_PRIO_PASS);
#endif
  if (exact) {
    for (int k = k0; k < npass; k += kWaves)
      row_pass < ND, UV, CLS, true, RK, NS, WP, PAD > (job, pl, refs, s_item, s_hot, s_wp, acc, par, lo + 64 * k + lane, hi);
  } else {
    for (int k = k0; k < npass; k += kWaves)
      row_pass < ND, UV, CLS, false, RK, NS, WP, PAD > (job, pl, refs, s_item, s_hot, s_wp, acc, par, lo + 64 * k + lane, hi);
  }
}

template < int PC, typename G, bool UV >
__device__ __forceinline__ void
row_slow (const ObmcJob & job, const PlaneIO & io, int cb, int bx, int by, int md, const int *fx, const int *fy, int row, int seg,
    int x_lo, int y_lo, int xfold_hi, int yfold_hi, const int *s_wx, const int *s_wy, uint32_t * acc, int par, bool exact)
{
  constexpr int ps = UV ? 1 : 0;
  const uint8_t *const refs[2] = { io.ref[0], io.ref[1] };
  const int prec = job.prec;
  const int y = by + row, xs = bx + 4 * seg;
  const int mode = md & 3;
  int pred[4];
  if (mode == 0) {
    pred[0] = pred[1] = pred[2] = pred[3] = md >> 8;
  } else {
    int val[2][4] = { {0, 0, 0, 0}, {0, 0, 0, 0} };
#pragma unroll
    for (int r = 0; r < 2; r++) {
      if (!(mode & (r + 1)))
        continue;
      if constexpr (PC == 2) {
        const int sx = fx[r] + 4 * seg * (1 << prec), sy = fy[r] + row * (1 << prec);
        const int x8 = prec == 2 ? sx * 2 : sx, y8 = prec == 2 ? sy * 2 : sy;
        const int hx = x8 >> 2, hy = y8 >> 2, rx = x8 & 3, ry = y8 & 3;
        const int Y0 = clampi (hy, 0, 2 * job.h - 2), Y1 = clampi (hy + 1, 0, 2 * job.h - 2);
        int p0[9], p1[9];
#pragma unroll
        for (int j = 0; j < 9; j++) {
          const int X = clampi (hx + j, 0, 2 * job.w - 2);
          const bool need = (j & 1) == 0 || rx != 0;
          p0[j] = need ? (int) gload < uint8_t > (refs[r] + hp_offset (X, Y0, job.ref_stride[r], ps, cb)) : 0;
          p1[j] = need && ry != 0 ? (int) gload < uint8_t > (refs[r] + hp_offset (X, Y1, job.ref_stride[r], ps, cb)) : 0;
        }
#pragma unroll
        for (int e = 0; e < 4; e++) {
          const int v = (4 - ry) * ((4 - rx) * p0[2 * e] + rx * p0[2 * e + 1])
              + ry * ((4 - rx) * p1[2 * e] + rx * p1[2 * e + 1]);
          val[r][e] = (v + 8) >> 4;
        }
      } else {
#pragma unroll
        for (int e = 0; e < 4; e++)
          val[r][e] = fetch_ref < PC > (refs[r], job.ref_stride[r], job.w, job.h,
              fx[r] + (4 * seg + e) * (1 << prec), fy[r] + row * (1 << prec), prec, ps, cb);
      }
    }
#pragma unroll
    for (int e = 0; e < 4; e++)
      pred[e] = mode == 3 ? (val[0][e] + val[1][e] + 1) >> 1 : (mode == 1 ? val[0][e] : val[1][e]);
  }
  int wy = s_wy[row];
  if (y < job.yoff)
    wy += s_wy[2 * job.yoff - row - 1];
  if (y >= yfold_hi)
    wy += s_wy[2 * (job.yblen - job.yoff) - row - 1];
#pragma unroll
  for (int e = 0; e < 4; e++) {
    const int x = xs + e, idx = 4 * seg + e;
    if (idx >= job.xblen)
      continue;
    int wx = s_wx[idx];
    if (x < job.xoff)
      wx += s_wx[2 * job.xoff - idx - 1];
    if (x >= xfold_hi)
      wx += s_wx[2 * (job.xblen - job.xoff) - idx - 1];
    int half;
    uint32_t *aw = acc_word < G, UV > (acc, par, x - x_lo, y - y_lo, &half);
    if constexpr (UV)
      half = cb;
    const uint32_t v = (uint32_t) (pred[e] * wx * wy);
    if (exact)
      acc_add_exact (aw, half, v & 0xffffu);
    else
      atomicAdd (aw, (v & 0xffffu) << (16 * half));
  }
}

template < typename G >
__device__ __forceinline__ bool
row_finish_is_fast (const ObmcJob & job, const PlaneIO & io, int x_lo, int x_hi)
{
  return job.res_bpp == 2 && x_hi - x_lo == G::kTW
      && ((((uintptr_t) io.residual) | (uintptr_t) io.residual_stride) & 15) == 0
      && ((((uintptr_t) io.out) | (uintptr_t) io.out_stride) & 7) == 0;
}

template < int TH, typename G > constexpr int kRFinishRounds = (TH * (G::kTW / 8) + kRThreads - 1) / kRThreads;

template < int TH, typename G, int STEP, int FIRST >
__device__ __forceinline__ void
row_finish_prefetch (const PlaneIO & io, int tid, int x_lo, int y_lo, int y_hi, u32x4 * res)
{
  constexpr int kG = G::kTW / 8;
#pragma unroll
  for (int n = 0; n < kRFinishRounds < TH, G >; n++) {
    const int it = tid + n * kRThreads, g = it & (kG - 1), y = y_lo + it / kG;
    if (!io.residual)
      res[STEP * n + FIRST] = (u32x4) { 0u, 0u, 0u, 0u };
    else if (y < y_hi && it < TH * kG)
      res[STEP * n + FIRST] = __builtin_nontemporal_load ((const SCHRO_GLOBAL u32x4 *) ((const char *) io.residual + (size_t) y * io.residual_stride + 2 * (x_lo + 8 * g)));
  }
}

template < int TH, typename G, bool UV >
__device__ __forceinline__ void
row_finish_plain (const ObmcJob & job, const PlaneIO & io, int cb, const uint32_t * acc, int par, int tid, int x_lo, int y_lo,
    int x_hi, int y_hi)
{
  for (int it = tid; it < TH * G::kTW; it += kRThreads) {
    const int xx = it & (G::kTW - 1), yy = it / G::kTW;
    const int x = x_lo + xx, y = y_lo + yy;
    if (y >= y_hi || x >= x_hi)
      continue;
    int half;
    const uint32_t *aw = acc_word < G, UV > (const_cast < uint32_t * >(acc), par, xx, yy, &half);
    if constexpr (UV)
      half = cb;
    const int16_t a = (int16_t) (*aw >> (16 * half));
    const char *rrow = (const char *) io.residual + (size_t) y * io.residual_stride;
    const int16_t res = !io.residual ? (int16_t) 0 : job.res_bpp == 2 ? gload < int16_t > ((const int16_t *) rrow + x)
        : (int16_t) gload < int32_t > ((const int32_t *) rrow + x);
    int16_t t1 = (int16_t) (a + 32);
    t1 = (int16_t) (t1 >> 6);
    t1 = (int16_t) (res + t1);
    gstore < uint8_t > (io.out + (size_t) y * io.out_stride + x, (uint8_t) clampi (t1, 0, 255));
  }
}

template < int TH, typename G, bool NOCLAMP = false >
__device__ __forceinline__ void
row_finish (const ObmcJob & job, const PlaneIO & io, uint32_t * acc, int par, int tid, int x_lo, int y_lo,
    int x_hi, int y_hi, bool fast, const u32x4 * res)
{
  constexpr int kG = G::kTW / 8;
  if (fast) {
#pragma unroll
    for (int n = 0; n < kRFinishRounds < TH, G >; n++) {
      const int it = tid + n * kRThreads;
      const int g = it & (kG - 1), yy = it / kG;
      const int y = y_lo + yy;
      if (y >= y_hi || it >= TH * kG)
        continue;
      const uint32_t *ap = acc + yy * G::kAccW + (G::kMargin / 2 + 4 * g);
      uint32_t av[4];
      if (par) {
        const uint32_t w0 = ap[0], w1 = ap[1], w2 = ap[2], w3 = ap[3], w4 = ap[4];
        av[0] = __builtin_amdgcn_alignbit (w1, w0, 16);
        av[1] = __builtin_amdgcn_alignbit (w2, w1, 16);
        av[2] = __builtin_amdgcn_alignbit (w3, w2, 16);
        av[3] = __builtin_amdgcn_alignbit (w4, w3, 16);
      } else {
        av[0] = ap[0];
        av[1] = ap[1];
        av[2] = ap[2];
        av[3] = ap[3];
      }
      const int x = x_lo + 8 * g;
      const u32x4 r = res[n];
      const uint32_t rv[4] = { r.x, r.y, r.z, r.w };
      uint32_t t[4];
#pragma unroll
      for (int k = 0; k < 4; k++) {
        s16x2 v = (__builtin_bit_cast (s16x2, av[k]) + (short) 32) >> 6;
        v = v + __builtin_bit_cast (s16x2, rv[k]);
        if constexpr (!NOCLAMP)
          v = __builtin_elementwise_min (__builtin_elementwise_max (v, (s16x2) (short) 0), (s16x2) (short) 255);
        t[k] = __builtin_bit_cast (uint32_t, v);
      }
      u32x2 o;
      o.x = __builtin_amdgcn_perm (t[1], t[0], 0x06040200u);
      o.y = __builtin_amdgcn_perm (t[3], t[2], 0x06040200u);
      __builtin_nontemporal_store (o, (SCHRO_GLOBAL u32x2 *) (io.out + (size_t) y * io.out_stride + x));
    }
    return;
  }
  row_finish_plain < TH, G, false > (job, io, 0, acc, par, tid, x_lo, y_lo, x_hi, y_hi);
}

template < int TH, typename G, bool NOCLAMP = false >
__device__ __forceinline__ void
row_finish_uv (const PlaneIO & iou, const PlaneIO & iov, const uint32_t * acc, int tid, int x_lo, int y_lo, int y_hi, const u32x4 * res)
{
  constexpr int kG = G::kTW / 8;
#pragma unroll
  for (int n = 0; n < kRFinishRounds < TH, G >; n++) {
    const int it = tid + n * kRThreads;
    const int g = it & (kG - 1), yy = it / kG;
    const int y = y_lo + yy;
    if (y >= y_hi || it >= TH * kG)
      continue;
    const uint32_t *ap = acc + yy * G::kAccW + (G::kMargin + 8 * g);
    const u32x4 ru = res[2 * n], rv = res[2 * n + 1];
    const uint32_t ruw[4] = { ru.x, ru.y, ru.z, ru.w }, rvw[4] = { rv.x, rv.y, rv.z, rv.w };
    uint32_t t[8];
#pragma unroll
    for (int k = 0; k < 8; k++) {
      const uint32_t r = __builtin_amdgcn_perm (rvw[k >> 1], ruw[k >> 1], (k & 1) ? 0x07060302u : 0x05040100u);
      s16x2 v = (__builtin_bit_cast (s16x2, ap[k]) + (short) 32) >> 6;
      v = v + __builtin_bit_cast (s16x2, r);
      if constexpr (!NOCLAMP)
        v = __builtin_elementwise_min (__builtin_elementwise_max (v, (s16x2) (short) 0), (s16x2) (short) 255);
      t[k] = __builtin_bit_cast (uint32_t, v);
    }
    const uint32_t a01 = __builtin_amdgcn_perm (t[1], t[0], 0x06020400u), a23 = __builtin_amdgcn_perm (t[3], t[2], 0x06020400u);
    const uint32_t a45 = __builtin_amdgcn_perm (t[5], t[4], 0x06020400u), a67 = __builtin_amdgcn_perm (t[7], t[6], 0x06020400u);
    u32x2 ou, ov;
    ou.x = __builtin_amdgcn_perm (a23, a01, 0x05040100u);
    ou.y = __builtin_amdgcn_perm (a67, a45, 0x05040100u);
    ov.x = __builtin_amdgcn_perm (a23, a01, 0x07060302u);
    ov.y = __builtin_amdgcn_perm (a67, a45, 0x07060302u);
    const int x = x_lo + 8 * g;
    __builtin_nontemporal_store (ou, (SCHRO_GLOBAL u32x2 *) (iou.out + (size_t) y * iou.out_stride + x));
    __builtin_nontemporal_store (ov, (SCHRO_GLOBAL u32x2 *) (iov.out + (size_t) y * iov.out_stride + x));
  }
}

template < typename G >
__device__ __forceinline__ bool
row_finish_s16_is_fast (const PlaneIO & io, int x_lo, int x_hi)
{
  return x_hi - x_lo == G::kTW && ((((uintptr_t) io.out) | (uintptr_t) io.out_stride) & 15) == 0;
}

template < int TH, typename G, bool UV >
__device__ __forceinline__ void
row_finish_s16_plain (const PlaneIO & io, int cb, const uint32_t * acc, int par, int tid, int x_lo, int y_lo, int x_hi, int y_hi)
{
  for (int it = tid; it < TH * G::kTW; it += kRThreads) {
    const int xx = it & (G::kTW - 1), yy = it / G::kTW;
    const int x = x_lo + xx, y = y_lo + yy;
    if (y >= y_hi || x >= x_hi)
      continue;
    int half;
    const uint32_t *aw = acc_word < G, UV > (const_cast < uint32_t * >(acc), par, xx, yy, &half);
    if constexpr (UV)
      half = cb;
    const int16_t a = (int16_t) (*aw >> (16 * half));
    gstore < int16_t > ((int16_t *) (io.out + (size_t) y * io.out_stride) + x, (int16_t) ((int16_t) ((int16_t) a - 8160) >> 6));
  }
}

template < int TH, typename G >
__device__ __forceinline__ void
row_finish_s16 (const PlaneIO & io, const uint32_t * acc, int par, int tid, int x_lo, int y_lo, int x_hi, int y_hi, bool fast)
{
  constexpr int kG = G::kTW / 8;
  if (fast) {
#pragma unroll
    for (int n = 0; n < kRFinishRounds < TH, G >; n++) {
      const int it = tid + n * kRThreads;
      const int g = it & (kG - 1), yy = it / kG;
      const int y = y_lo + yy;
      if (y >= y_hi || it >= TH * kG)
        continue;
      const uint32_t *ap = acc + yy * G::kAccW + (G::kMargin / 2 + 4 * g);
      uint32_t av[4];
      if (par) {
        const uint32_t w0 = ap[0], w1 = ap[1], w2 = ap[2], w3 = ap[3], w4 = ap[4];
        av[0] = __builtin_amdgcn_alignbit (w1, w0, 16);
        av[1] = __builtin_amdgcn_alignbit (w2, w1, 16);
        av[2] = __builtin_amdgcn_alignbit (w3, w2, 16);
        av[3] = __builtin_amdgcn_alignbit (w4, w3, 16);
      } else {
        av[0] = ap[0];
        av[1] = ap[1];
        av[2] = ap[2];
        av[3] = ap[3];
      }
      uint32_t t[4];
#pragma unroll
      for (int k = 0; k < 4; k++)
        t[k] = __builtin_bit_cast (uint32_t, (s16x2) ((__builtin_bit_cast (s16x2, av[k]) - (short) 8160) >> 6));
      const int x = x_lo + 8 * g;
      __builtin_nontemporal_store ((u32x4) { t[0], t[1], t[2], t[3] },
          (SCHRO_GLOBAL u32x4 *) (io.out + (size_t) y * io.out_stride + 2 * x));
    }
    return;
  }
  row_finish_s16_plain < TH, G, false > (io, 0, acc, par, tid, x_lo, y_lo, x_hi, y_hi);
}

template < int TH, typename G >
__device__ __forceinline__ void
row_finish_s16_uv (const PlaneIO & iou, const PlaneIO & iov, const uint32_t * acc, int tid, int x_lo, int y_lo, int y_hi)
{
  constexpr int kG = G::kTW / 8;
#pragma unroll
  for (int n = 0; n < kRFinishRounds < TH, G >; n++) {
    const int it = tid + n * kRThreads;
    const int g = it & (kG - 1), yy = it / kG;
    const int y = y_lo + yy;
    if (y >= y_hi || it >= TH * kG)
      continue;
    const uint32_t *ap = acc + yy * G::kAccW + (G::kMargin + 8 * g);
    uint32_t t[8];
#pragma unroll
    for (int k = 0; k < 8; k++)
      t[k] = __builtin_bit_cast (uint32_t, (s16x2) ((__builtin_bit_cast (s16x2, ap[k]) - (short) 8160) >> 6));
    u32x4 ou, ov;
    ou.x = __builtin_amdgcn_perm (t[1], t[0], 0x05040100u);
    ou.y = __builtin_amdgcn_perm (t[3], t[2], 0x05040100u);
    ou.z = __builtin_amdgcn_perm (t[5], t[4], 0x05040100u);
    ou.w = __builtin_amdgcn_perm (t[7], t[6], 0x05040100u);
    ov.x = __builtin_amdgcn_perm (t[1], t[0], 0x07060302u);
    ov.y = __builtin_amdgcn_perm (t[3], t[2], 0x07060302u);
    ov.z = __builtin_amdgcn_perm (t[5], t[4], 0x07060302u);
    ov.w = __builtin_amdgcn_perm (t[7], t[6], 0x07060302u);
    const int x = x_lo + 8 * g;
    __builtin_nontemporal_store (ou, (SCHRO_GLOBAL u32x4 *) (iou.out + (size_t) y * iou.out_stride + 2 * x));
    __builtin_nontemporal_store (ov, (SCHRO_GLOBAL u32x4 *) (iov.out + (size_t) y * iov.out_stride + 2 * x));
  }
}

constexpr int kRPadItems = 344;

template < int ND, int NP, bool UV = false, int TH = kRTH, bool NORES = false, int RK = 1, int NS = 1, bool WP = false, bool PAD = false >
__device__ __forceinline__ void
obmc_row_body (const ObmcJob * __restrict__ jobs, int njobs, const uint32_t * __restrict__ order, uint32_t * __restrict__ overflow,
    const uint32_t * __restrict__ wtabs)
{
  typedef RowGeo < ND, UV, NS > G;
  static_assert (!UV || NP == 1, "a UV job is one virtual plane of (U, V) samples");
  static_assert (NS == 1 || (NS == 2 && (ND == 3 || ND == 4)), "segments: halves of 12 or 16 bytes");
  constexpr int kRTW = G::kTW, ps = UV ? 1 : 0;
  __shared__ __attribute__ ((aligned (16))) uint32_t acc[TH * G::kAccW + 3];
  static_assert (!PAD || (RK != 0 && NS == 1), "line-aligned quads: the tiled planes, one segment");
  constexpr int kRBlkCap = G::kBlk, kRItemCap = G::kItem + (PAD ? kRPadItems : 0);
  typedef RowBlkT < G::kPadBlk > RowBlk;
  __shared__ RowBlk s_hot[kRBlkCap];
  __shared__ uint16_t s_meta[kRBlkCap];
  __shared__ uint16_t s_rim[kRBlkCap];
  __shared__ uint16_t s_item[kRItemCap];
  __shared__ __attribute__ ((aligned (16))) uint32_t s_wp[G::kWTab];
  const int *const s_wx = reinterpret_cast < const int * >(s_wp + G::kWRampX), *const s_wy = reinterpret_cast < const int * >(s_wp + G::kWRampY);
  __shared__ int s_icnt[kRSlots];
  __shared__ int s_nrim, s_wide, s_padleft;

  const uint64_t t_start = __builtin_amdgcn_s_memtime ();
#if defined (SCHRO_HIP_EXPERIMENTS) && defined (SCHRO_ROW_PRIO_SETUP)
  __builtin_amdgcn_s_setprio (SCHRO_ROW_PRIO_SETUP);
#endif
  const int bid = xcd_tile_id (blockIdx.x, gridDim.x);
#ifdef SCHRO_HIP_EXPERIMENTS
  const bool have_rec = order != nullptr;
#else
  constexpr bool have_rec = true;
#endif
  const u32x4 rec = have_rec ? *reinterpret_cast < const u32x4 * >(order + 4 * (size_t) bid) : (u32x4) { 0u, 0u, 0u, 0u };
  const uint32_t entry = rec.x;
  const int ji = have_rec ? (int) (entry >> 16) : find_job (jobs, njobs, bid);
  const ObmcJob job = jobs[ji];
#ifdef SCHRO_HIP_EXPERIMENTS
#define RSTAMP(n) do { if (job.stamps && threadIdx.x == 0 && blockIdx.x < 16384) \
    job.stamps[blockIdx.x * 16 + (n)] = __builtin_amdgcn_s_memtime () - t_start; } while (0)
#else
#define RSTAMP(n) do { } while (0)
#endif
  RSTAMP (7);
  const int tid = threadIdx.x;
  int x_lo = (int) (rec.y & 0xffffu), y_lo = (int) (rec.y >> 16);
  if (!have_rec) {
    const int t = bid - job.tile_base;
    const int ty = mdiv (t, job.tiles_x, job.m_tiles_x), tx = t - ty * job.tiles_x;
    x_lo = tx * kRTW;
    y_lo = ty * TH;
  }
  const int x_hi = min (x_lo + kRTW, job.w), y_hi = min (y_lo + TH, job.h);
  constexpr int nplanes = NP;

#if defined (SCHRO_HIP_EXPERIMENTS) && defined (SCHRO_ROW_REP_SETUP)
  constexpr int kRepSetup = SCHRO_ROW_REP_SETUP;
#else
  constexpr int kRepSetup = 1;
#endif
#if defined (SCHRO_HIP_EXPERIMENTS) && defined (SCHRO_ROW_REP_PASSES)
  constexpr int kRepPasses = SCHRO_ROW_REP_PASSES;
#else
  constexpr int kRepPasses = 1;
#endif
#if defined (SCHRO_HIP_EXPERIMENTS) && defined (SCHRO_ROW_REP_FINISH)
  constexpr int kRepFinish = SCHRO_ROW_REP_FINISH;
#else
  constexpr int kRepFinish = 1;
#endif
  const int xblen = job.xblen, yblen = job.yblen;
  const int par = UV ? 0 : job.xoff & 1;
  const int xfold_hi = job.nbx * job.xbsep - job.xoff, yfold_hi = job.nby * job.ybsep - job.yoff;
  int ibase[kRRim + 1];
  bool exact = false;
  int nrim = 0;
  constexpr int kAccQuads = (TH * G::kAccW + 3) / 4;
#pragma unroll
  for (int rep_ = 0; rep_ < kRepSetup; rep_++) {
  if (rep_)
    __syncthreads ();
  for (int it = tid; it < kAccQuads; it += kRThreads)
    reinterpret_cast < u32x4 * >(acc)[it] = (u32x4) { 0u, 0u, 0u, 0u };
  constexpr int kWQuads = G::kWTab / 4, kWQ = (kWQuads + kRThreads / 2 - 1) / (kRThreads / 2);
  static_assert (G::kWTab % 4 == 0 && kWQ <= 2, "one or two quads of the weight table per lane of the last two waves");
  u32x4 wq[kWQ];
#pragma unroll
  for (int n = 0; n < kWQ; n++) {
    wq[n] = (u32x4) { 0u, 0u, 0u, 0u };
    const int q = tid - kRThreads / 2 + n * (kRThreads / 2);
    if (tid >= kRThreads / 2 && q < kWQuads)
      wq[n] = gload < u32x4 > (wtabs + (size_t) job.ipw * G::kWTab + 4 * q);
  }
  if (tid >= 128 && tid < 128 + kRSlots)
    s_icnt[tid - 128] = 0;
  if (tid == 192) {
    s_nrim = 0;
    s_wide = 0;
    s_padleft = kRPadItems;
  }

  int nblk;
  {
    const int xbsep = job.xbsep, ybsep = job.ybsep, xoff = job.xoff, yoff = job.yoff, prec = job.prec;
    int i_lo = (int) (rec.z & 0xffffu), j_lo = (int) (rec.z >> 16), nbi = (int) (rec.w & 0xffu), nbj = (int) ((rec.w >> 8) & 0xffu);
    static_assert (kRBlkCap * 128 < 65536, "the 16-bit block-row division below");
    uint32_t m16_nbi = rec.w >> 16;
    if (!have_rec) {
      i_lo = max (0, mdiv (x_lo + xoff - xblen + 2 * xbsep, xbsep, job.m_xbsep) - 1);
      const int i_hi = min (job.nbx - 1, mdiv (x_hi - 1 + xoff, xbsep, job.m_xbsep));
      j_lo = max (0, mdiv (y_lo + yoff - yblen + 2 * ybsep, ybsep, job.m_ybsep) - 1);
      const int j_hi = min (job.nby - 1, mdiv (y_hi - 1 + yoff, ybsep, job.m_ybsep));
      nbi = i_hi - i_lo + 1;
      nbj = j_hi - j_lo + 1;
      m16_nbi = nbi > 1 ? (65536u + (uint32_t) nbi - 1u) / (uint32_t) nbi : 0u;
    }
    if (!have_rec && NS > 1) {
      nbi *= NS;
      m16_nbi = (65536u + (uint32_t) nbi - 1u) / (uint32_t) nbi;
    }
    nblk = nbi > 0 && nbj > 0 ? min (nbi * nbj, kRBlkCap) : 0;
    const int gh = 2 * job.h - 2;
    const int seglen = NS > 1 ? xblen / NS : xblen;
    uint32_t mv_pre[3] = { 0u, 0u, 0u };
    if (tid < nblk) {
      const int bj = nbi == 1 ? tid : (int) (((uint32_t) tid * m16_nbi) >> 16);
      const uint8_t *mvp = job.mvs + (size_t) 20 * ((size_t) (j_lo + bj) * job.nbx + (i_lo + (tid - bj * nbi) / NS));
      mv_pre[0] = gload < uint32_t > (mvp);
      mv_pre[1] = gload < uint32_t > (mvp + 12);
      mv_pre[2] = gload < uint32_t > (mvp + 16);
    }
    RSTAMP (10);
    __syncthreads ();
    RSTAMP (8);
#pragma unroll
    for (int n = 0; n < kWQ; n++) {
      const int q = tid - kRThreads / 2 + n * (kRThreads / 2);
      if (tid >= kRThreads / 2 && q < kWQuads)
        reinterpret_cast < u32x4 * >(s_wp)[q] = wq[n];
    }
    RSTAMP (1);
    for (int blk = tid; blk < nblk; blk += kRThreads) {
      const int bj = nbi == 1 ? blk : (int) (((uint32_t) blk * m16_nbi) >> 16);
      const int vi = blk - bj * nbi, seg = NS > 1 ? vi % NS : 0;
      const int i = i_lo + vi / NS, jj = j_lo + bj;
      uint32_t flags = mv_pre[0], v01 = mv_pre[1], v23 = mv_pre[2];
      if (blk >= kRThreads) {
        const uint8_t *mvp = job.mvs + (size_t) 20 * ((size_t) jj * job.nbx + i);
        flags = gload < uint32_t > (mvp);
        v01 = gload < uint32_t > (mvp + 12);
        v23 = gload < uint32_t > (mvp + 16);
      }
      const int bx = xbsep * i - xoff, by = ybsep * jj - yoff;
      RowBlk info;
      info.x = (int16_t) (bx + seg * seglen - x_lo);
      info.y = (int16_t) (by - y_lo);
      const int mode = flags & 3;
      const bool interior = i >= 1 && i < job.max_x_blocks && jj >= 1 && jj < job.max_y_blocks;
      auto dc_of = [&] (int comp) {
        const int dc = comp == 0 ? (int16_t) (v01 & 0xffff) : comp == 1 ? (int16_t) (v01 >> 16) : (int16_t) (v23 & 0xffff);
        return interior ? (int) (int16_t) (dc + 128) : (int) (uint8_t) (dc + 128);
      };
      const int pdc = dc_of (job.comp), pdc_b = (nplanes > 1 || UV) ? dc_of (job.comp_b) : 0;
      const int dcs = (int) (((uint32_t) pdc & 0xffffu) | ((uint32_t) pdc_b << 16));
      uint32_t bflags = (uint32_t) mode | ((uint32_t) seg << 8);
      int taps[2] = { 0, 0 };
      RowRef in_ref[2], edge_ref[2];
      bool off_h = false, clamped_v = false;
#pragma unroll
      for (int r = 0; r < 2; r++) {
        int fx, fy;
        mv_origin (job, bx, by, v01, v23, r, &fx, &fy);
        fx += (seg * seglen) * (1 << prec);
        const bool used = (mode & (r + 1)) != 0;
        if constexpr (RK == 0) {
          const bool in_h = fx >= 0 && fx + seglen <= job.w, in_v = fy >= 0 && fy + yblen <= job.h;
          clamped_v |= used && !(in_h && in_v);
          in_ref[r].base = used && in_h && in_v ? fx : 0;
          in_ref[r].ydb = used && in_h && in_v ? (uint32_t) fy : 0u;
          in_ref[r].dci = 0;
          edge_ref[r].base = used ? fx : 0;
          edge_ref[r].ydb = used ? (uint32_t) fy & 0xffffu : 0u;
          edge_ref[r].dci = 0;
        } else {
          const int hx = RK == 3 ? fx >> 2 : prec >= 2 ? fx >> 1 : fx, hy = RK == 3 ? fy >> 2 : prec >= 2 ? fy >> 1 : fy;
          const int rx = RK == 3 ? fx & 3 : prec >= 2 ? fx & 1 : 0, ry = RK == 3 ? fy & 3 : prec >= 2 ? fy & 1 : 0;
          const int wbits = RK == 3 ? (rx << 4) | (ry << 6) : 0;
          const int xp = ((hx >> 1) + kHpApron) << ps, px = hx & 1, py = hy & 1;
          const bool in_h = xp >= 0 && (xp >> 4) < (job.ref_stride[r] >> 9) && (unsigned) (hy + 16384) < 32768u;
          const bool in_v = hy >= 0 && hy + 2 * (yblen - 1) + 1 <= gh;
          off_h |= used && !in_h;
          clamped_v |= used && !in_v;
          const int colbase = in_h && used ? (xp >> 4) * 512 + (xp & 15) + px * 128 : 0;
          const uint32_t dB = in_h && used && rx ? (uint32_t) (px ? (1 << ps) - 128 : 128) : 0u;
          in_ref[r].base = colbase + (in_h && used ? py * 256 : 0);
          in_ref[r].ydb = (in_h && in_v && used ? (uint32_t) (hy >> 1) : 0u) | (dB << 16);
          in_ref[r].dci = in_h && used ? ((ry ? (py ? (int) (((uint32_t) -256 << 16) | 1u) : (int) (256u << 16)) : 0) | wbits) : 0;
          edge_ref[r].base = colbase;
          edge_ref[r].ydb = (in_h && used ? (uint32_t) hy & 0xffffu : 0u) | (dB << 16);
          edge_ref[r].dci = in_h && used ? wbits : 0;
          bflags |= (uint32_t) (in_h && used && ry ? 1 : 0) << (6 + r);
          taps[r] = in_h && used ? (rx ? 1 : 0) | (ry ? 2 : 0) : 0;
        }
      }
      info.r[0] = in_ref[0];
      info.r[1] = in_ref[1];
      const int ra = max (0, -(int) info.y), rb = min (yblen, y_hi - by);
      int fold = (by < yoff ? 1 : 0) | (by + yblen > yfold_hi ? 2 : 0) | (bx < xoff ? 4 : 0) | (bx + xblen > xfold_hi ? 8 : 0);
      if (NS > 1)
        fold &= seg == 0 ? ~8 : ~4;
      const bool wide_dc = mode == 0 && ((unsigned) pdc > 255u || (unsigned) pdc_b > 255u);
      if (wide_dc) {
        s_wide = 1;
        if (overflow)
          __hip_atomic_store (overflow, 1u, __ATOMIC_RELAXED, __HIP_MEMORY_SCOPE_SYSTEM);
      }
      int key, nrows = rb - ra;
      if (off_h || wide_dc || yblen > 32 || xblen > NS * (UV ? 8 : 16)) {
        key = kRRim;
        if (seg == 0) {
          int fx, fy;
          mv_origin (job, bx, by, v01, v23, 0, &fx, &fy);
          info.r[0].base = (int) (((uint32_t) fx & 0xffffu) | ((uint32_t) fy << 16));
          mv_origin (job, bx, by, v01, v23, 1, &fx, &fy);
          info.r[1].base = (int) (((uint32_t) fx & 0xffffu) | ((uint32_t) fy << 16));
          s_rim[atomicAdd (&s_nrim, 1)] = (uint16_t) blk;
        }
      } else if (fold || clamped_v) {
        key = kREdge;
        info.r[0] = edge_ref[0];
        info.r[1] = edge_ref[1];
        bflags |= (uint32_t) fold << 2;
      } else if (mode == 3) {
        key = kRBoth;
      } else if (mode == 0) {
        key = kRDc;
      } else {
        key = mode == 1 ? kRRef0 : kRRef1;
      }
      if (NS > 1 && ((int) info.x + seglen <= 0 || (int) info.x >= kRTW))
        nrows = 0;
      int nitems = nrows;
      if constexpr (PAD) {
        if ((key == kRBoth || key == kRRef0 || key == kRRef1) && nrows > 0) {
          const uint32_t y_first = (info.r[key == kRRef1 ? 1 : 0].ydb & 0xffffu) + (uint32_t) ra;
          const int front = (int) (y_first & 3u), padded = (front + nrows + 3) & ~3, pad = padded - nrows;
          if (pad && atomicSub (&s_padleft, pad) < pad) {
            key = kREdge;
            info.r[0] = edge_ref[0];
            info.r[1] = edge_ref[1];
          } else {
            bflags |= (uint32_t) front << 9;
            nitems = padded;
          }
        }
      }
      const int slot = row_slot_base (key) + (key == kRBoth ? taps[0] | (taps[1] << 2) : key == kRRef0 ? taps[0] : key == kRRef1 ? taps[1] : 0);
      if (mode == 0)
        info.r[0].base = dcs;
      info.fr = (uint32_t) ra | ((uint32_t) nrows << 8) | (bflags << 16);
      s_hot[blk] = info;
      const int istart = key == kRRim ? 0 : atomicAdd (&s_icnt[slot], nitems);
      s_meta[blk] = (uint16_t) (slot | (istart << 5));
    }
  }
  __syncthreads ();
  RSTAMP (2);
  int sbase;
  {
    const int lane = tid & 63;
    const int cnt = lane < kRSlots ? s_icnt[lane] : 0;
    static_assert (kRSlots <= 32, "the scan covers two rows of 16 lanes");
    int incl = cnt;
    incl += __builtin_amdgcn_update_dpp (0, incl, 0x111, 0xf, 0xf, true);
    incl += __builtin_amdgcn_update_dpp (0, incl, 0x112, 0xf, 0xf, true);
    incl += __builtin_amdgcn_update_dpp (0, incl, 0x114, 0xf, 0xf, true);
    incl += __builtin_amdgcn_update_dpp (0, incl, 0x118, 0xf, 0xf, true);
    incl += __builtin_amdgcn_update_dpp (0, incl, 0x142, 0xa, 0xf, false);
    sbase = incl - cnt;
  }
#pragma unroll
  for (int c = 0; c <= kRRim; c++)
    ibase[c] = __builtin_amdgcn_readlane (sbase, row_slot_base (c));
  for (int b0 = 0; b0 < nblk; b0 += kRThreads) {
    const int blk = b0 + tid;
    const bool have = blk < nblk;
    const int meta = have ? s_meta[blk] : 0, slot = meta & 31;
    const int ib = __shfl (sbase, slot);
    if (!have || slot == row_slot_base (kRRim))
      continue;
    const int rows = (int) s_hot[blk].fr, ra = rows & 0xff, n = (rows >> 8) & 0xff;
    uint16_t *ip = s_item + ib + (meta >> 5);
    typedef uint32_t u32_a2 __attribute__ ((aligned (2), may_alias));
    typedef u32x2 u32x2_a2 __attribute__ ((aligned (2), may_alias));
    if constexpr (PAD) {
      if (slot < row_slot_base (kRDc) && n > 0) {
        const int front = (rows >> 25) & 3, total = (front + n + 3) & ~3;
#pragma clang loop vectorize(disable) unroll(disable)
        for (int j = 0; j < total; j += 4) {
          uint32_t it4[4];
#pragma unroll
          for (int q = 0; q < 4; q++) {
            const int idx = j + q - front;
            it4[q] = (uint32_t) (blk | ((ra + min (max (idx, 0), n - 1)) << 9)) | ((unsigned) idx >= (unsigned) n ? 0x8000u : 0u);
          }
          *reinterpret_cast < u32x2_a2 * >(ip + j) = (u32x2) { it4[0] | (it4[1] << 16), it4[2] | (it4[3] << 16) };
        }
        continue;
      }
    }
    uint32_t pair = (uint32_t) (blk | (ra << 9)) * 0x00010001u + 0x02000000u;
    int r = 0;
#pragma clang loop vectorize(disable) unroll(disable)
    for (; r + 4 <= n; r += 4, pair += 0x08000800u)
      *reinterpret_cast < u32x2_a2 * >(ip + r) = (u32x2) { pair, pair + 0x04000400u };
    if (n & 2) {
      *reinterpret_cast < u32_a2 * >(ip + r) = pair;
      r += 2;
      pair += 0x04000400u;
    }
    if (n & 1)
      ip[r] = (uint16_t) pair;
  }
  exact = __builtin_amdgcn_readfirstlane (s_wide) != 0;
  nrim = __builtin_amdgcn_readfirstlane (s_nrim);
  __syncthreads ();
  RSTAMP (3);
  }

#pragma unroll
  for (int pl = 0; pl < nplanes; pl++) {
    PlaneIO io;
    io.ref[0] = pl ? job.ref_b[0] : job.ref[0];
    io.ref[1] = pl ? job.ref_b[1] : job.ref[1];
    io.residual = pl ? job.residual_b : job.residual;
    io.out = pl ? job.out_b : job.out;
    io.residual_stride = pl ? job.residual_stride_b : job.residual_stride;
    io.out_stride = pl ? job.out_stride_b : job.out_stride;
    PlaneIO iov = io;
    if constexpr (UV) {
      if constexpr (RK == 0) {
        iov.ref[0] = job.ref_b[0];
        iov.ref[1] = job.ref_b[1];
      }
      iov.residual = job.residual_b;
      iov.out = job.out_b;
      iov.residual_stride = job.residual_stride_b;
      iov.out_stride = job.out_stride_b;
    }
    constexpr bool kEarlyRes = ND >= 3 && NP == 1 && !NORES;
    const bool s16 = !NORES && job.out_s16;
    const bool fast = s16 ? row_finish_s16_is_fast < G > (io, x_lo, x_hi) && (!UV || row_finish_s16_is_fast < G > (iov, x_lo, x_hi))
        : row_finish_is_fast < G > (job, io, x_lo, x_hi) && (!UV || row_finish_is_fast < G > (job, iov, x_lo, x_hi));
    constexpr int kRounds = kRFinishRounds < TH, G >;
    u32x4 res[UV ? 2 * kRounds : kRounds];
#define SCHRO_ROW_PREFETCH() do { \
      if constexpr (UV) { \
        row_finish_prefetch < TH, G, 2, 0 > (io, tid, x_lo, y_lo, y_hi, res); \
        row_finish_prefetch < TH, G, 2, 1 > (iov, tid, x_lo, y_lo, y_hi, res); \
      } else { \
        row_finish_prefetch < TH, G, 1, 0 > (io, tid, x_lo, y_lo, y_hi, res); \
      } } while (0)
    if constexpr (kEarlyRes) {
      if (fast)
        SCHRO_ROW_PREFETCH ();
      __builtin_amdgcn_sched_barrier (0);
    }
    int turn = 0;
    RowRefs refs;
#pragma unroll
    for (int r = 0; r < 2; r++) {
      refs.stride[r] = (uint32_t) job.ref_stride[r];
      const uint32_t bytes = RK == 0 ? (uint32_t) job.ref_stride[r] * (uint32_t) (job.h - 1) + (((uint32_t) job.w + 3u) & ~3u)
          : (uint32_t) job.ref_stride[r] * (uint32_t) ((job.h + 3) >> 2);
      refs.rsrc[r] = __builtin_amdgcn_make_buffer_rsrc ((void *) io.ref[r], 0, (int) bytes, 0x00020000);
      refs.rsrc_b[r] = refs.rsrc[r];
      if constexpr (UV && RK == 0)
        refs.rsrc_b[r] = __builtin_amdgcn_make_buffer_rsrc ((void *) iov.ref[r], 0, (int) bytes, 0x00020000);
    }
#define SCHRO_ROW_CLASS(C) row_class < ND, UV, C, RK, NS, WP, PAD > (job, pl, refs, s_item, s_hot, s_wp, acc, par, \
    ibase[C], ibase[C + 1], exact, &turn)
#pragma unroll
    for (int rep_ = 0; rep_ < kRepPasses; rep_++) {
      SCHRO_ROW_CLASS (kRBoth);
      SCHRO_ROW_CLASS (kRRef0);
      SCHRO_ROW_CLASS (kRRef1);
      SCHRO_ROW_CLASS (kRDc);
      SCHRO_ROW_CLASS (kREdge);
    }
#undef SCHRO_ROW_CLASS
    RSTAMP (4);
    if (nrim > 0) {
      const int nseg = (xblen + 3) >> 2, per_block = yblen * nseg;
      const uint32_t m_per_block = div_magic (per_block), m_nseg = div_magic (nseg);
      for (int item = tid; item < nrim * per_block; item += kRThreads) {
        const int b = mdiv (item, per_block, m_per_block);
        const int rem = item - b * per_block;
        const int r2 = mdiv (rem, nseg, m_nseg), s2 = rem - r2 * nseg;
        const RowBlk & hb = s_hot[s_rim[b]];
        const int bx = hb.x + x_lo, by = hb.y + y_lo;
        const int y = by + r2, xs = bx + 4 * s2;
        if (y < y_lo || y >= y_hi || xs + 3 < x_lo || xs >= x_hi)
          continue;
        const int fx[2] = { (int) (int16_t) hb.r[0].base, (int) (int16_t) hb.r[1].base }, fy[2] = { hb.r[0].base >> 16, hb.r[1].base >> 16 };
#define SCHRO_ROW_SLOW(cb, dcpl) do { \
          const int md = (int) (blk_flags (hb) & 3u) | (blk_dc (hb, dcpl) << 8);        \
          if constexpr (RK == 0) \
            row_slow < 0, G, UV > (job, (UV && cb) ? iov : io, cb, bx, by, md, fx, fy, r2, s2, x_lo, y_lo, xfold_hi, yfold_hi, s_wx, s_wy, acc, par, exact); \
          else if (RK == 1 && job.prec == 1) \
            row_slow < 1, G, UV > (job, io, cb, bx, by, md, fx, fy, r2, s2, x_lo, y_lo, xfold_hi, yfold_hi, s_wx, s_wy, acc, par, exact); \
          else \
            row_slow < 2, G, UV > (job, io, cb, bx, by, md, fx, fy, r2, s2, x_lo, y_lo, xfold_hi, yfold_hi, s_wx, s_wy, acc, par, exact); \
        } while (0)
        if constexpr (UV) {
          SCHRO_ROW_SLOW (0, 0);
          SCHRO_ROW_SLOW (1, 1);
        } else {
          SCHRO_ROW_SLOW (0, pl);
        }
#undef SCHRO_ROW_SLOW
      }
    }
    RSTAMP (5);
    if constexpr (NORES) {
#pragma unroll
      for (int n = 0; n < (UV ? 2 * kRounds : kRounds); n++)
        res[n] = (u32x4) { 0u, 0u, 0u, 0u };
    } else if constexpr (!kEarlyRes) {
      if (fast)
        SCHRO_ROW_PREFETCH ();
    }
#undef SCHRO_ROW_PREFETCH
    __syncthreads ();
    RSTAMP (6);
#pragma unroll
    for (int rep_ = 0; rep_ < kRepFinish; rep_++)
    if (s16) {
      if constexpr (UV) {
        if (fast) {
          row_finish_s16_uv < TH, G > (io, iov, acc, tid, x_lo, y_lo, y_hi);
        } else {
          row_finish_s16_plain < TH, G, true > (io, 0, acc, par, tid, x_lo, y_lo, x_hi, y_hi);
          row_finish_s16_plain < TH, G, true > (iov, 1, acc, par, tid, x_lo, y_lo, x_hi, y_hi);
        }
      } else {
        row_finish_s16 < TH, G > (io, acc, par, tid, x_lo, y_lo, x_hi, y_hi, fast);
      }
    } else if constexpr (UV) {
      if (fast) {
        if (NORES && !exact)
          row_finish_uv < TH, G, NORES > (io, iov, acc, tid, x_lo, y_lo, y_hi, res);
        else
          row_finish_uv < TH, G > (io, iov, acc, tid, x_lo, y_lo, y_hi, res);
      } else {
        row_finish_plain < TH, G, true > (job, io, 0, acc, par, tid, x_lo, y_lo, x_hi, y_hi);
        row_finish_plain < TH, G, true > (job, iov, 1, acc, par, tid, x_lo, y_lo, x_hi, y_hi);
      }
    } else {
      if (NORES && !exact)
        row_finish < TH, G, NORES > (job, io, acc, par, tid, x_lo, y_lo, x_hi, y_hi, fast, res);
      else
        row_finish < TH, G > (job, io, acc, par, tid, x_lo, y_lo, x_hi, y_hi, fast, res);
    }
    if (pl + 1 < nplanes) {
      __syncthreads ();
      for (int it = tid; it < kAccQuads; it += kRThreads)
        reinterpret_cast < u32x4 * >(acc)[it] = (u32x4) { 0u, 0u, 0u, 0u };
      __syncthreads ();
    }
  }
  RSTAMP (9);
#ifdef SCHRO_HIP_EXPERIMENTS
  if (job.stamps && threadIdx.x == 0 && blockIdx.x < 16384) {
    job.stamps[blockIdx.x * 16 + 12] = t_start;
    job.stamps[blockIdx.x * 16 + 13] = __builtin_amdgcn_s_memtime ();
    job.stamps[blockIdx.x * 16 + 14] = __builtin_amdgcn_s_getreg ((4 << 0) | (0 << 6) | (31 << 11));
    job.stamps[blockIdx.x * 16 + 15] = __builtin_amdgcn_s_getreg ((20 << 0) | (0 << 6) | (31 << 11));
  }
#else
  (void) t_start;
#endif
#undef RSTAMP
}

template < int ND, int NP, bool UV = false, int TH = kRTH, bool NORES = false, int RK = 1, int NS = 1, bool WP = false, bool PAD = false >
constexpr RowForm
row_form ()
{
  return RowForm { RK, ND, UV ? 3 : NP, NS, NORES, WP };
}

#define SCHRO_ROW_KERNEL(name, waves, ...) \
__global__ __launch_bounds__ (kRThreads) __attribute__ ((amdgpu_waves_per_eu (waves, waves))) \
void name (const ObmcJob * __restrict__ jobs, int njobs, const uint32_t * __restrict__ order, uint32_t * __restrict__ overflow, \
    const uint32_t * __restrict__ wtabs) \
{ \
  obmc_row_body < __VA_ARGS__ > (jobs, njobs, order, overflow, wtabs); \
} \
constexpr RowForm name##_form = row_form < __VA_ARGS__ > ();

}

typedef void (*RowKernel) (const ObmcJob *, int, const uint32_t *, uint32_t *, const uint32_t *);

struct RowEntry {
  RowForm form;
  RowKernel kernel;
};
#define ROW_ENTRY(name) RowEntry { name##_form, name }
struct RowTable {
  const RowEntry *e;
  int n;
};
RowTable obmc_row_table_half (), obmc_row_table_plain (), obmc_row_table_eighth ();

constexpr RowKernel
row_find (const RowTable & t, const RowForm & f)
{
  for (int i = 0; i < t.n; i++)
    if (t.e[i].form == f)
      return t.e[i].kernel;
  return f.nores ? row_find (t, RowForm { f.kind, f.nd, f.np, f.ns, false, f.weighted }) : nullptr;
}

constexpr bool
row_table_ok (const RowTable & t, int kind)
{
  for (int i = 0; i < t.n; i++) {
    if (t.e[i].form.kind != kind)
      return false;
    for (int k = 0; k < i; k++)
      if (t.e[k].form == t.e[i].form)
        return false;
  }
  return true;
}

}
```

schroedinger_amd/csrc/plane_obmc.cpp:

```cpp

#include "schro_hip_internal.h"

#include <cstdio>
#include <cstdlib>
#include <cstring>
#include <algorithm>

using namespace schro;

static_assert (sizeof (ObmcJob) * kMaxJobs <= SchroHipContext::kArgSlotBytes, "a launch group of kMaxJobs OBMC jobs fits a table slot");

extern "C" {

static int
obmc_row_merge_mode ()
{
  static const int mode = SCHRO_ENV ("SCHRO_HIP_OBMC_MERGE") ? atoi (SCHRO_ENV ("SCHRO_HIP_OBMC_MERGE")) : 1;
  return mode;
}

static unsigned long long *g_stamps;
static unsigned long long *
obmc_stamp_buffer ()
{
  static const bool on = SCHRO_ENV ("SCHRO_HIP_OBMC_STAMPS") != nullptr;
  if (on && !g_stamps) {
    if (hipMalloc ((void **) &g_stamps, 16384 * 16 * 8) != hipSuccess)
      g_stamps = nullptr;
    else
      (void) hipMemset (g_stamps, 0, 16384 * 16 * 8);
  }
  return g_stamps;
}

extern "C" void
schro_hip_obmc_stamps_dump (void)
{
  if (!g_stamps)
    return;
  (void) hipDeviceSynchronize ();
  std::vector < unsigned long long >h (16384 * 16);
  (void) hipMemcpy (h.data (), g_stamps, h.size () * 8, hipMemcpyDeviceToHost);
  for (int n = 1; n <= 11; n++) {
    std::vector < unsigned long long >v;
    for (int b = 0; b < 16384; b++)
      if (h[b * 16 + 9])
        v.push_back (h[b * 16 + n]);
    if (v.empty ())
      continue;
    std::sort (v.begin (), v.end ());
    unsigned long long sum = 0;
    for (auto x : v)
      sum += x;
    fprintf (stderr, "stamp %d: median %llu  p10 %llu  p90 %llu  p99 %llu  max %llu  mean %llu  (n=%zu)\n", n, v[v.size () / 2],
        v[v.size () / 10], v[v.size () * 9 / 10], v[v.size () * 99 / 100], v.back (), sum / v.size (), v.size ());
  }
  {
    unsigned long simd[4] = { 0, 0, 0, 0 };
    for (int b = 0; b < 16384; b++)
      if (h[b * 16 + 9])
        simd[(h[b * 16 + 14] >> 4) & 3]++;
    fprintf (stderr, "wave 0 of a workgroup on SIMD 0 / 1 / 2 / 3: %lu %lu %lu %lu\n", simd[0], simd[1], simd[2], simd[3]);
  }
  std::vector < std::pair < int, int > >by_cu;
  for (int b = 0; b < 16384; b++)
    if (h[b * 16 + 9])
      by_cu.push_back ({ (int) (((h[b * 16 + 14] >> 8) & 0xff) | ((h[b * 16 + 15] & 0xf) << 8)), b });
  std::sort (by_cu.begin (), by_cu.end ());
  double life_all = 0, cap_all = 0;
  unsigned long long span_max = 0, span_min = ~0ull;
  size_t ncu = 0;
  for (size_t i = 0; i < by_cu.size ();) {
    size_t j = i;
    unsigned long long t0 = ~0ull, t1 = 0, life = 0;
    for (; j < by_cu.size () && by_cu[j].first == by_cu[i].first; j++) {
      const int b = by_cu[j].second;
      t0 = std::min (t0, h[b * 16 + 12]);
      t1 = std::max (t1, h[b * 16 + 13]);
      life += h[b * 16 + 13] - h[b * 16 + 12];
    }
    life_all += (double) life;
    cap_all += (double) (t1 - t0);
    span_max = std::max (span_max, t1 - t0);
    span_min = std::min (span_min, t1 - t0);
    ncu++;
    i = j;
  }
  for (int x = 0; x < 16; x++) {
    unsigned long long t0 = ~0ull, t1 = 0, life = 0;
    size_t nw = 0;
    for (int b = 0; b < 16384; b++)
      if (h[b * 16 + 9] && (int) (h[b * 16 + 15] & 0xf) == x) {
        t0 = std::min (t0, h[b * 16 + 12]);
        t1 = std::max (t1, h[b * 16 + 13]);
        life += h[b * 16 + 13] - h[b * 16 + 12];
        nw++;
      }
    if (nw)
      fprintf (stderr, "  XCD %d: %zu workgroups, span %llu ticks, mean lifetime %llu\n", x, nw, t1 - t0, life / nw);
  }
  if (ncu)
    fprintf (stderr, "%zu workgroups on %zu CUs: per-CU span %llu .. %llu ticks, resident workgroups per CU %.2f\n",
        by_cu.size (), ncu, span_min, span_max, life_all / cap_all);
}

static int
obmc_tile_order (SchroHipContext * ctx, const std::vector < ObmcJob > &jobs, int variant, int total,
    const uint32_t ** d_order, int row_uv = -1, int row_ns = 1)
{
  *d_order = nullptr;
  static const bool enabled = !SCHRO_ENV ("SCHRO_HIP_OBMC_ORDER") || atoi (SCHRO_ENV ("SCHRO_HIP_OBMC_ORDER")) != 0;
  if (!enabled || variant < 1 || jobs.empty () || jobs.size () > 0xffff)
    return 0;
  const bool row = row_uv >= 0;
  const size_t words = row ? 4 : 1;
  uint64_t h = 1469598103934665603ull;
  auto mix = [&h] (uint64_t v) {
    for (int k = 0; k < 8; k++) {
      h ^= (v >> (8 * k)) & 0xff;
      h *= 1099511628211ull;
    }
  };
  std::vector < int >tiles_y (jobs.size ());
  std::vector < uint32_t > ref_class (jobs.size ());
  mix ((uint64_t) variant);
  for (size_t j = 0; j < jobs.size (); j++) {
    int tx;
    obmc_tiles (variant, jobs[j].w, jobs[j].h, jobs[j].xoff, &tx, &tiles_y[j]);
    if (tx * tiles_y[j] > 0xffff)
      return 0;
    size_t first = 0;
    while (jobs[first].ref[0] != jobs[j].ref[0])
      first++;
    ref_class[j] = (uint32_t) first;
    mix ((uint64_t) tx);
    mix ((uint64_t) tiles_y[j]);
    mix ((uint64_t) first);
    if (row) {
      const ObmcJob & g = jobs[j];
      mix ((uint64_t) g.w | ((uint64_t) g.h << 20) | ((uint64_t) row_uv << 40) | (1ull << 41) | ((uint64_t) row_ns << 42));
      mix ((uint64_t) g.xbsep | ((uint64_t) g.ybsep << 8) | ((uint64_t) g.xblen << 16) | ((uint64_t) g.yblen << 24) | ((uint64_t) g.xoff << 32)
          | ((uint64_t) g.yoff << 40));
      mix ((uint64_t) g.nbx | ((uint64_t) g.nby << 20));
    }
  }
  constexpr int per_queue = SchroHipContext::kOrderSlots / SchroHipContext::kQueues;
  const int k0 = ctx->cur * per_queue;
  SchroHipContext::OrderSlot * slot = nullptr, *lru = &ctx->order_slots[k0];
  for (int k = k0; k < k0 + per_queue; k++) {
    SchroHipContext::OrderSlot & o = ctx->order_slots[k];
    if (o.d && o.hash == h && o.count == (size_t) total * words)
      slot = &o;
    if (o.last_use < lru->last_use)
      lru = &o;
  }
  if (!slot) {
    struct Key {
      uint32_t row;
      uint32_t ref;
      uint32_t entry;
    };
    std::vector < Key > keys;
    keys.reserve ((size_t) total);
    static const int sup_x = SCHRO_ENV ("SCHRO_HIP_OBMC_SUPER_X") ? std::max (1, atoi (SCHRO_ENV ("SCHRO_HIP_OBMC_SUPER_X"))) : 4;
    static const int sup_y = SCHRO_ENV ("SCHRO_HIP_OBMC_SUPER_Y") ? std::max (1, atoi (SCHRO_ENV ("SCHRO_HIP_OBMC_SUPER_Y"))) : 4;
    for (size_t j = 0; j < jobs.size (); j++) {
      const int sx = variant == 4 ? sup_x : jobs[j].nplanes == 2 ? std::max (1, sup_x / 2) : sup_x;
      const int sy = variant == 4 ? std::max (1, sup_y / 2) : sup_y;
      const int nsx = div_up (jobs[j].tiles_x, sx);
      for (int ty = 0; ty < tiles_y[j]; ty++)
        for (int tx = 0; tx < jobs[j].tiles_x; tx++)
          keys.push_back (Key { (uint32_t) ((ty / sy) * nsx + tx / sx), ref_class[j],
              (uint32_t) (j << 16) | (uint32_t) (ty * jobs[j].tiles_x + tx) });
    }
    if (keys.size () != (size_t) total)
      return set_error (SCHRO_HIP_EINVAL, "obmc tile order: %zu tiles, %d expected", keys.size (), total);
    std::stable_sort (keys.begin (), keys.end (),[](const Key & a, const Key & b) {
          return a.row != b.row ? a.row < b.row : a.ref < b.ref;
        });
    {
      auto is_rim = [&](const Key & k) {
        const size_t j = k.entry >> 16;
        const int t = (int) (k.entry & 0xffffu), tx = t % jobs[j].tiles_x, ty = t / jobs[j].tiles_x;
        return tx == 0 || ty == 0 || tx == jobs[j].tiles_x - 1 || ty == tiles_y[j] - 1;
      };
      constexpr size_t kXcd = 8;
      std::vector < Key > rim_sorted, rim, inner;
      for (const Key & k : keys)
        (is_rim (k) ? rim_sorted : inner).push_back (k);
      for (size_t x = 0; x < kXcd; x++)
        for (size_t k = x; k < rim_sorted.size (); k += kXcd)
          rim.push_back (rim_sorted[k]);
      const size_t q = keys.size () / kXcd, r = keys.size () % kXcd;
      size_t ri = 0, ii = 0, out = 0;
      for (size_t x = 0; x < kXcd; x++) {
        const size_t n = q + (x < r ? 1 : 0);
        size_t nr = rim.size () / kXcd + (x < rim.size () % kXcd ? 1 : 0);
        nr = std::min (nr, n);
        if (n - nr > inner.size () - ii)
          nr = n - (inner.size () - ii);
        for (size_t k = 0; k < nr; k++)
          keys[out++] = rim[ri++];
        for (size_t k = nr; k < n; k++)
          keys[out++] = inner[ii++];
      }
      if (ri != rim.size () || ii != inner.size () || out != keys.size ())
        return set_error (SCHRO_HIP_EINVAL, "obmc tile order: rim / inner split does not add up");
    }
    slot = lru;
    if (slot->copy_pending) {
      SCHRO_HIP_CHECK (hipEventSynchronize (slot->copied));
      slot->copy_pending = false;
    }
    if (slot->cap < keys.size () * words) {
      if (slot->d)
        SCHRO_HIP_CHECK (hipFree (slot->d));
      if (slot->h)
        SCHRO_HIP_CHECK (hipHostFree (slot->h));
      slot->d = nullptr;
      slot->h = nullptr;
      slot->cap = 0;
      const size_t cap = (keys.size () + keys.size () / 4) * words;
      SCHRO_HIP_CHECK (hipMalloc ((void **) &slot->d, cap * sizeof (uint32_t)));
      SCHRO_HIP_CHECK (hipHostMalloc ((void **) &slot->h, cap * sizeof (uint32_t), hipHostMallocDefault));
      slot->cap = cap;
    }
    if (!slot->copied)
      SCHRO_HIP_CHECK (hipEventCreateWithFlags (&slot->copied, hipEventDisableTiming));
    for (size_t k = 0; k < keys.size (); k++) {
      slot->h[k * words] = keys[k].entry;
      if (row) {
        const ObmcJob & g = jobs[keys[k].entry >> 16];
        const int t = (int) (keys[k].entry & 0xffffu);
        obmc_row_tile_record (g, row_uv != 0, row_ns, t % g.tiles_x, t / g.tiles_x, &slot->h[k * words + 1]);
      }
    }
    SCHRO_HIP_CHECK (hipMemcpyAsync (slot->d, slot->h, keys.size () * words * sizeof (uint32_t), hipMemcpyHostToDevice,
            ctx->stream));
    SCHRO_HIP_CHECK (hipEventRecord (slot->copied, ctx->stream));
    slot->copy_pending = true;
    slot->hash = h;
    slot->count = keys.size () * words;
  }
  slot->last_use = ++ctx->arg_clock;
  *d_order = slot->d;
  return 0;
}

int
schro_hip_obmc_batch (SchroHipContext * ctx, const SchroHipObmcPlane * planes, int nplanes)
{
  SCHRO_HIP_REQUIRE (ctx && planes && nplanes > 0 && nplanes <= kMaxJobs,
      "obmc_batch: bad arguments");
  (void) hipSetDevice (ctx->device);
  auto variant_of = [](const SchroHipObmcPlane & pl) {
    return (pl.picture_weight_1 == 1 && pl.picture_weight_2 == 1 && pl.picture_weight_bits == 1) ? 1 : 0;
  };
  static const bool use_row = !SCHRO_ENV ("SCHRO_HIP_OBMC_KERNEL") || strcmp (SCHRO_ENV ("SCHRO_HIP_OBMC_KERNEL"), "row") == 0;
  std::vector < ObmcJob > all (nplanes);
  struct LaunchKey {
    int prec;
    int variant;
    RowForm form;
    bool pred_only, out_s16;
    bool operator== (const LaunchKey & o) const
    {
      return prec == o.prec && variant == o.variant && form == o.form && pred_only == o.pred_only && out_s16 == o.out_s16;
    }
  };
  std::vector < LaunchKey > key (nplanes);
  uint32_t pred_epoch = 0;
  struct OvfDone {
    SchroHipContext *c = nullptr;
    int k = 0;
    void arm (SchroHipContext * ctx_, int k_) { c = ctx_; k = k_; }
    ~OvfDone () { if (c && c->ovf_ev[k]) (void) hipEventRecord (c->ovf_ev[k], c->stream); }
  } ovf_done;
  for (int p = 0; p < nplanes; p++) {
    const SchroHipObmcPlane & pl = planes[p];
    SCHRO_HIP_REQUIRE (pl.mvs && pl.ref1 && pl.out, "obmc_batch: plane %d has a NULL pointer", p);
    SCHRO_HIP_REQUIRE (pl.mv_precision >= 0 && pl.mv_precision <= 3,
        "obmc_batch: mv_precision %d out of range", pl.mv_precision);
    SCHRO_HIP_REQUIRE (pl.component >= 0 && pl.component <= 2, "obmc_batch: bad component");
    SCHRO_HIP_REQUIRE (!pl.residual || pl.residual_bpp == 2 || pl.residual_bpp == 4, "obmc_batch: residual bpp");
    SCHRO_HIP_REQUIRE (pl.prediction_only >= 0 && pl.prediction_only <= 2, "obmc_batch: plane %d: prediction_only is 0, 1 or 2", p);
    SCHRO_HIP_REQUIRE (pl.prediction_only != 2 || (!pl.residual && ((uintptr_t) pl.out | (uintptr_t) pl.out_stride) % 2 == 0),
        "obmc_batch: plane %d: prediction_only 2 needs residual NULL and an s16 plane in `out`", p);
    SCHRO_HIP_REQUIRE (pl.prediction_only != 1 || (!pl.residual && pl.picture_weight_1 >= 0 && pl.picture_weight_2 >= 0
            && pl.picture_weight_1 + pl.picture_weight_2 <= (1 << pl.picture_weight_bits)),
        "obmc_batch: plane %d: prediction_only needs residual NULL and picture weights >= 0 that sum to at most 1 << bits "
        "(a prediction of 8 bits); other pictures take the residual form", p);
    SCHRO_HIP_REQUIRE (pl.picture_weight_bits >= 0 && pl.picture_weight_bits <= 6,
        "obmc_batch: picture_weight_bits %d unsupported", pl.picture_weight_bits);
    SCHRO_HIP_REQUIRE (pl.picture_weight_bits > 0 || pl.picture_weight_1 + pl.picture_weight_2 == 1,
        "obmc_batch: picture_weight_bits 0 needs weights that sum to 1");
    ObmcJob & j = all[p];
    memset (&j, 0, sizeof (j));
    const int hs = pl.component ? pl.chroma_h_shift : 0, vs = pl.component ? pl.chroma_v_shift : 0;
    j.xbsep = pl.xbsep_luma >> hs;
    j.ybsep = pl.ybsep_luma >> vs;
    j.xblen = pl.xblen_luma >> hs;
    j.yblen = pl.yblen_luma >> vs;
    SCHRO_HIP_REQUIRE (((pl.xblen_luma | pl.yblen_luma | pl.xbsep_luma | pl.ybsep_luma) & 3) == 0,
        "obmc_batch: plane %d: luma block sizes and separations must be multiples of 4", p);
    SCHRO_HIP_REQUIRE (j.xbsep > 0 && j.ybsep > 0 && j.xblen >= j.xbsep && j.yblen >= j.ybsep
        && j.xblen <= 2 * j.xbsep && j.yblen <= 2 * j.ybsep && j.xblen <= 64 && j.yblen <= 64,
        "obmc_batch: plane %d block geometry %dx%d sep %dx%d unsupported", p, j.xblen, j.yblen,
        j.xbsep, j.ybsep);
    j.xoff = (j.xblen - j.xbsep) / 2;
    j.yoff = (j.yblen - j.ybsep) / 2;
    SCHRO_HIP_REQUIRE (pl.width >= j.xblen && pl.height >= j.yblen,
        "obmc_batch: plane %d smaller than one block", p);
    j.nbx = pl.x_num_blocks;
    j.nby = pl.y_num_blocks;
    SCHRO_HIP_REQUIRE (j.nbx > 0 && j.nby > 0, "obmc_batch: plane %d has no blocks", p);
    j.max_x_blocks = std::min (j.nbx - 1, (pl.width - j.xoff) / j.xbsep);
    j.max_y_blocks = std::min (j.nby - 1, (pl.height - j.yoff) / j.ybsep);
    j.mv_shift_x = hs;
    j.mv_shift_y = vs;
    j.prec = pl.mv_precision;
    j.wbits = pl.picture_weight_bits;
    j.w1 = pl.picture_weight_1;
    j.w2 = pl.picture_weight_2;
    j.comp = pl.component;
    j.mvs = (const uint8_t *) pl.mvs;
    j.ref[0] = pl.ref1;
    j.ref_stride[0] = pl.ref1_stride;
    j.ref[1] = pl.ref2 ? pl.ref2 : pl.ref1;
    j.ref_stride[1] = pl.ref2 ? pl.ref2_stride : pl.ref1_stride;
    j.residual = pl.residual;
    j.residual_stride = pl.residual ? pl.residual_stride : 0;
    j.res_bpp = pl.residual ? pl.residual_bpp : 2;
    j.out = pl.out;
    j.out_stride = pl.out_stride;
    j.w = pl.width;
    j.h = pl.height;
    SCHRO_HIP_REQUIRE (!pl.ref_pair || (pl.mv_precision >= 1 && pl.component >= 1),
        "obmc_batch: plane %d: ref_pair is for the chroma components of half-pel references", p);
    j.ref_ps = pl.ref_pair ? 1 : 0;
    j.ref_cb = pl.ref_pair ? pl.component - 1 : 0;
    if (pl.mv_precision >= 1)
      for (int r = 0; r < 2; r++)
        SCHRO_HIP_REQUIRE (j.ref_stride[r] % 512 == 0 && j.ref_stride[r] >= hp_chunks (j.w, j.ref_ps) * 512
            && ((uintptr_t) j.ref[r] & 127) == 0,
            "obmc_batch: plane %d: reference %d is not a half-pel image of this component (128-byte aligned, stride from "
            "schro_hip_upsampled_bytes / _pair_bytes)", p, r + 1);
    j.out_s16 = pl.prediction_only == 2;
    const bool pred_only = pl.prediction_only == 1;
    const RowForm form = use_row ? obmc_row_form (j, false, pred_only) : RowForm {};
    key[p] = LaunchKey { pl.mv_precision, form ? 3 : variant_of (pl), form, pred_only, (bool) j.out_s16 };
  }
  long pair_tiles = 0;
  for (int p = 0; p < nplanes; p++)
    if (key[p].form && all[p].comp != 0)
      pair_tiles += (long) ((all[p].w + 127) / 128) * ((all[p].h + 31) / 32);
  const bool pairs_pay = obmc_row_merge_mode () == 2 || (obmc_row_merge_mode () == 1 && pair_tiles > 6L * ctx->cus);
  auto same_blocks = [](const ObmcJob & a, const ObmcJob & b) {
    return a.comp == 1 && b.comp == 2
        && a.mvs == b.mvs && a.w == b.w && a.h == b.h && a.nbx == b.nbx && a.nby == b.nby && a.xblen == b.xblen
        && a.yblen == b.yblen && a.xbsep == b.xbsep && a.ybsep == b.ybsep && a.mv_shift_x == b.mv_shift_x
        && a.mv_shift_y == b.mv_shift_y && a.res_bpp == b.res_bpp && a.ref_stride[0] == b.ref_stride[0]
        && a.ref_stride[1] == b.ref_stride[1] && a.prec == b.prec && a.w1 == b.w1 && a.w2 == b.w2 && a.wbits == b.wbits;
  };
  for (int p = 0; p + 1 < nplanes; p++) {
    const ObmcJob & a = all[p], &b = all[p + 1];
    const bool uv_plain = a.prec == 0 && b.prec == 0 && !a.ref_ps && !b.ref_ps;
    if (((a.ref_ps && b.ref_ps && a.ref[0] == b.ref[0] && a.ref[1] == b.ref[1]) || uv_plain)
        && use_row && same_blocks (a, b)
        && planes[p].prediction_only == planes[p + 1].prediction_only) {
      ObmcJob au = a;
      au.ref_b[0] = b.ref[0];
      au.ref_b[1] = b.ref[1];
      const RowForm uv = obmc_row_form (au, true, key[p].pred_only);
      if (uv) {
        key[p] = key[p + 1] = LaunchKey { a.prec, 4, uv, key[p].pred_only, (bool) a.out_s16 };
        p++;
        continue;
      }
      if (!uv_plain)
        continue;
    }
    if (pairs_pay && key[p].form && key[p] == key[p + 1] && same_blocks (a, b)) {
      LaunchKey two = key[p];
      two.form.np = 2;
      if (obmc_row_has_kernel (two.form)) {
        key[p] = key[p + 1] = two;
        p++;
      }
    }
  }
  std::vector < char >done (nplanes, 0);
  for (int first = 0; first < nplanes; first++) {
    if (done[first])
      continue;
    const LaunchKey & group = key[first];
    const RowForm & form = group.form;
    const bool row = (bool) form, paired = form.np == 2, uv = form.np == 3;
    uint32_t *overflow = nullptr;
    if (group.pred_only) {
      if (!ctx->dc_gave_up) {
        SCHRO_HIP_CHECK (hipHostMalloc ((void **) &ctx->dc_gave_up, 64, hipHostMallocDefault));
        memset (ctx->dc_gave_up, 0, 64);
      }
      if (!pred_epoch) {
        pred_epoch = ++ctx->pred_epoch;
        if (pred_epoch == 0)
          pred_epoch = ++ctx->pred_epoch;
        const int rc = pred_overflow_claim (ctx, pred_epoch);
        if (rc)
          return rc;
        ovf_done.arm (ctx, (int) (pred_epoch % SchroHipContext::kOvfRing));
      }
      overflow = ctx->dc_gave_up + 4 + pred_epoch % SchroHipContext::kOvfRing;
    }
    std::vector < ObmcJob > jobs;
    int tile_base = 0;
    long long group_planes = 0;
    for (int p = first; p < nplanes; p++) {
      if (done[p] || !(key[p] == group))
        continue;
      done[p] = 1;
      group_planes++;
      ObmcJob j = all[p];
      int tiles_y;
      obmc_tiles (group.variant, j.w, j.h, j.xoff, &j.tiles_x, &tiles_y);
      j.tile_base = tile_base;
      obmc_item_geometry (&j);
      j.stamps = obmc_stamp_buffer ();
      j.nplanes = 1;
      if ((paired || uv) && j.comp == 2) {
        ObmcJob & a = jobs.back ();
        a.nplanes = 2;
        a.comp_b = j.comp;
        a.ref_b[0] = j.ref[0];
        a.ref_b[1] = j.ref[1];
        a.residual_b = j.residual;
        a.out_b = j.out;
        a.residual_stride_b = j.residual_stride;
        a.out_stride_b = j.out_stride;
        continue;
      }
      tile_base += j.tiles_x * tiles_y;
      jobs.push_back (j);
    }
#ifdef SCHRO_HIP_EXPERIMENTS
    static const bool use_strip = SCHRO_ENV ("SCHRO_HIP_OBMC_STRIP") && atoi (SCHRO_ENV ("SCHRO_HIP_OBMC_STRIP")) != 0;
    bool strip = use_strip && row && form.np == 1 && form.nd == 3 && form.ns == 1;
    for (size_t k = 0; strip && k < jobs.size (); k++)
      strip = obmc_strip_ok (jobs[k]);
    if (strip) {
      const int seg_rows = 8;
      int wave_base = 0;
      for (ObmcJob & j : jobs) {
        int strips, segs;
        obmc_strip_tiles (j, seg_rows, &strips, &segs);
        j.tiles_x = strips;
        j.tile_base = wave_base;
        wave_base += strips * segs;
      }
      void *d_sjobs;
      int rs = push_args (ctx, jobs.data (), sizeof (ObmcJob) * jobs.size (), &d_sjobs);
      if (rs)
        return rs;
      ProfileScope ps (ctx, SCHRO_HIP_KERNEL_OBMC);
      rs = launch_obmc_strip (ctx->stream, (const ObmcJob *) d_sjobs, (int) jobs.size (), wave_base, seg_rows, group.pred_only, overflow, ctx->cus);
      if (rs)
        return rs;
      ctx->obmc_routes[SCHRO_HIP_OBMC_ROUTE_STRIP] += group_planes;
      continue;
    }
#endif
    std::vector < ObmcJob > all_jobs;
    all_jobs.swap (jobs);
    const int all_tiles = tile_base;
    int r = 0;
    for (size_t first_job = 0; first_job < all_jobs.size () && !r;) {
      void *d_wtabs = nullptr;
      size_t end_job = all_jobs.size ();
      std::vector < uint32_t > tabs;
      if (row) {
        const size_t words = (size_t) obmc_row_weight_words (form.nd, form.ns);
        std::vector < uint32_t > one (words);
        for (size_t n = first_job; n < end_job; n++) {
          ObmcJob & j = all_jobs[n];
          obmc_row_weight_table (j, form.nd, form.ns, uv, one.data ());
          size_t k = 0;
          while (k * words < tabs.size () && memcmp (&tabs[k * words], one.data (), words * 4))
            k++;
          if (k * words == tabs.size ()) {
            if ((k + 1) * words * 4 > SchroHipContext::kArgSlotBytes) {
              end_job = n;
              break;
            }
            tabs.insert (tabs.end (), one.begin (), one.end ());
          }
          j.ipw = (int) k;
        }
        r = push_args (ctx, tabs.data (), tabs.size () * 4, &d_wtabs);
        if (r)
          return r;
      }
      jobs.assign (all_jobs.begin () + (long) first_job, all_jobs.begin () + (long) end_job);
      const int base = jobs.front ().tile_base;
      tile_base = (end_job < all_jobs.size () ? all_jobs[end_job].tile_base : all_tiles) - base;
      for (ObmcJob & j : jobs)
        j.tile_base -= base;
      first_job = end_job;
      void *d_jobs;
      r = push_args (ctx, jobs.data (), sizeof (ObmcJob) * jobs.size (), &d_jobs);
      if (r)
        return r;
      const uint32_t *d_order;
      r = obmc_tile_order (ctx, jobs, group.variant, tile_base, &d_order, row ? (uv ? 1 : 0) : -1, form.ns);
      if (r)
        return r;
#ifndef SCHRO_HIP_EXPERIMENTS
      if (row && !d_order)
        return set_error (SCHRO_HIP_EINVAL, "obmc_batch: internal: no tile table for a row launch of %zu jobs", jobs.size ());
#endif
      if (g_stamps)
        (void) hipMemsetAsync (g_stamps, 0, 16384 * 16 * 8, ctx->stream);
      {
        ProfileScope ps (ctx, SCHRO_HIP_KERNEL_OBMC);
        r = row ? launch_obmc_row (ctx->stream, (const ObmcJob *) d_jobs, (int) jobs.size (), tile_base, form, d_order, overflow, (const uint32_t *) d_wtabs)
            : launch_obmc (ctx->stream, (const ObmcJob *) d_jobs, (int) jobs.size (), tile_base, group.prec, group.variant, d_order, overflow);
      }
    }
    if (r)
      return r;
    ctx->obmc_routes[row ? SCHRO_HIP_OBMC_ROUTE_ROW : group.variant == 1 ? SCHRO_HIP_OBMC_ROUTE_ITEM : SCHRO_HIP_OBMC_ROUTE_GENERAL] += group_planes;
  }
  return 0;
}

}

extern "C" {

unsigned int
schro_hip_obmc_prediction_epoch (SchroHipContext * ctx)
{
  return ctx ? ctx->pred_epoch : 0u;
}

int
schro_hip_obmc_routes (SchroHipContext * ctx, long long counts[SCHRO_HIP_OBMC_ROUTES], int reset)
{
  SCHRO_HIP_REQUIRE (ctx && counts, "obmc_routes: bad arguments");
  for (int k = 0; k < SCHRO_HIP_OBMC_ROUTES; k++) {
    counts[k] = ctx->obmc_routes[k];
    if (reset)
      ctx->obmc_routes[k] = 0;
  }
  return 0;
}

}
```

schroedinger_amd/csrc/schro_hip_internal.h:

```cpp
#pragma once

#include <hip/hip_runtime.h>
#include <hip/hip_ext.h>
#include <cstdint>
#include <cstddef>
#include <vector>

#include "schro_hip.h"

#ifdef SCHRO_HIP_DRY
#include "schro_hip_dry.h"
#endif

#ifdef SCHRO_HIP_EXPERIMENTS
#define SCHRO_ENV(name) getenv (name)
#else
#define SCHRO_ENV(name) ((const char *) nullptr)
#endif

namespace schro {

int set_error (int code, const char *fmt, ...);
int set_status (int code, const char *fmt, ...);

static inline int
div_up (int a, int b)
{
  return (a + b - 1) / b;
}

static inline size_t
round_up (size_t a, size_t b)
{
  return (a + b - 1) / b * b;
}

#define SCHRO_HIP_CHECK(expr)                                                  \
  do {                                                                         \
    hipError_t _e = (expr);                                                    \
    if (_e != hipSuccess)                                                      \
      return schro::set_error (SCHRO_HIP_EDEVICE, "%s:%d: %s -> %s", __FILE__, \
          __LINE__, #expr, hipGetErrorString (_e));                            \
  } while (0)

#define SCHRO_HIP_REQUIRE(cond, ...)                                           \
  do {                                                                         \
    if (!(cond))                                                               \
      return schro::set_error (SCHRO_HIP_EINVAL, __VA_ARGS__);                 \
  } while (0)

bool profile_launch_events (hipEvent_t * start, hipEvent_t * stop);

#ifdef SCHRO_HIP_DRY
#define SCHRO_LAUNCH(kernel, grid, block, shmem, stream, ...)                                      \
  do {                                                                                             \
    const dim3 g_ = (grid), b_ = (block);                                                          \
    (void) g_; (void) b_; (void) (shmem); (void) (stream);                                         \
  } while (0)
#else
#define SCHRO_LAUNCH(kernel, grid, block, shmem, stream, ...)                                      \
  do {                                                                                             \
    hipEvent_t pa_, pb_;                                                                           \
    if (schro::profile_launch_events (&pa_, &pb_))                                                 \
      hipExtLaunchKernelGGL (kernel, grid, block, shmem, stream, pa_, pb_, 0, __VA_ARGS__);       \
    else                                                                                           \
      hipLaunchKernelGGL (kernel, grid, block, shmem, stream, __VA_ARGS__);                        \
  } while (0)
#endif


struct IwtJob {
  const void *sb[4];
  int sb_stride[4];
  void *dst;
  int dst_stride;
  int w, h;
  int tiles_x;
  int tile_base;
  int flags;
  int pad;
  int dep_rows2, dep_tiles_y, dep_tiles_x, dep_ctr;
  int ctr, small;
  const uint8_t *pred;
  int pred_stride;
  int out_w, out_h;
  int pad2;
  const void *l1_sb[4];
  int l1_sb_stride[4];
};

struct IwtFwdJob {
  const void *src;
  int src_stride;
  int flags;
  void *band[4];
  int band_stride[4];
  int w, h;
  int tiles_x;
  int tile_base;
  uint32_t m_tiles_x;
  int pad;
};

struct DownsampleJob {
  const uint8_t *src;
  uint8_t *dst;
  int src_stride, dst_stride;
  int sw, sh;
  int dw, dh;
  int ext;
  int xorg;
  int tiles_x;
  int tile_base;
  uint32_t m_tiles_x;
  int pad;
};

struct ScanPicture {
  const uint8_t *frame;
  const uint8_t *ref;
  SchroHipMetricScanResult *results;
  uint32_t *metrics;
  int frame_stride, ref_stride;
  int width, height;
  int scan_base;
  int pad[3];
};
struct ScanJob {
  int x, y, bw, bh;
  int ref_x, ref_y, sw, sh;
  int gi, gj;
  int dx, dy;
  int pic;
  uint32_t m_sh;
  int pad[2];
};
static_assert (sizeof (ScanJob) == 64 && sizeof (ScanPicture) == 64, "scan tables: 64-byte records");

struct RoughLevel {
  const uint8_t *frame;
  const uint8_t *ref;
  uint8_t *field;
  const uint8_t *hint;
  int frame_stride, ref_stride;
  int w, h;
  int ext;
  int shift, dist;
  int pad;
};
struct RoughChain {
  int nbx, nby, xb, yb;
  int ref;
  int nlevels;
  int pad[2];
  RoughLevel level[SCHRO_HIP_MAX_HIER_LEVELS];
};
static_assert (sizeof (RoughLevel) == 64 && sizeof (RoughChain) == 32 + 64 * SCHRO_HIP_MAX_HIER_LEVELS, "rough search tables");

struct HbmLevel {
  const uint8_t *frame[3];
  const uint8_t *ref[3];
  uint8_t *field;
  const uint8_t *hint;
  int frame_stride[3], ref_stride[3];
  int w, h;
  int hs, vs;
  int ext;
  int shift, range;
  int pad[3];
};
struct HbmChain {
  int nbx, nby, xb, yb;
  int ref;
  int nlevels;
  int pad[2];
  HbmLevel level[SCHRO_HIP_MAX_HIER_LEVELS + 1];
};
static_assert (sizeof (HbmLevel) == 128 && sizeof (HbmChain) == 32 + 128 * (SCHRO_HIP_MAX_HIER_LEVELS + 1), "block matching tables");

struct SubpelChain {
  const uint8_t *src;
  const uint8_t *up;
  uint8_t *field;
  int32_t *table;
  double lambda;
  int src_stride, up_stride;
  int w, h, ext;
  int nbx, nby, xb, yb;
  int ref;
  int tile_base;
  int pad;
};
static_assert (sizeof (SubpelChain) == 88, "sub-pel tables");

struct HaarPackJob {
  const void *src[3];
  int src_stride[3];
  int w, h;
  uint8_t *dst;
  int dst_stride;
  int tiles_x;
  int tile_base;
};

struct V210Job {
  const void *src[3];
  int src_stride[3];
  const void *ll[3];
  int ll_stride[3];
  int w, h;
  int out_w, out_h;
  uint8_t *dst;
  int dst_stride;
  int tiles_x;
  int tile_base;
  int flags;
};

struct Pack8Job {
  const void *src[3];
  int src_stride[3];
  const void *ll[3];
  int ll_stride[3];
  const uint8_t *pred[3];
  int pred_stride[3];
  int w, h;
  int out_w, out_h;
  uint8_t *dst;
  int dst_stride;
  int tiles_x;
  int tile_base;
  int flags;
};

struct WideJob {
  const void *src[3];
  int src_stride[3];
  const void *ll[3];
  int ll_stride[3];
  int w, h;
  int out_w, out_h;
  uint8_t *dst;
  int dst_stride;
  int tiles_x;
  int tile_base;
  int flags;
  int shift;
};

struct ConvertJob {
  const void *src;
  uint8_t *dst;
  int src_stride, dst_stride;
  int w, h;
  int tiles_x;
  int tile_base;
  const uint8_t *pred;
  int pred_stride;
  int pad;
};

struct PackJob {
  const uint8_t *src[3];
  uint8_t *dst;
  int src_stride[3];
  int dst_stride;
  int sw, sh;
  int hs, vs;
  int w, h;
  int format;
  int src_bpp;
  int tiles_x;
  int tile_base;
};

struct UpsampleJob {
  const uint8_t *src;
  uint8_t *dst;
  int src_stride, dst_stride;
  int w, h;
  int tiles_x;
  int tile_base;
  const uint8_t *src_b;
  int src_b_stride;
  int pad;
};

struct ObmcJob {
  const uint8_t *mvs;
  const uint8_t *ref[2];
  const void *residual;
  uint8_t *out;
  int ref_stride[2];
  int residual_stride;
  int out_stride;
  int w, h;
  int nbx, nby;
  int xblen, yblen, xbsep, ybsep, xoff, yoff;
  int max_x_blocks, max_y_blocks;
  int mv_shift_x, mv_shift_y;
  int prec, wbits, w1, w2;
  int comp;
  int res_bpp;
  int tiles_x;
  int tile_base;
  int nseg, ref_ps, lpi, ref_cb, ipw, chunk_cap;
  uint32_t m_tiles_x, m_xbsep, m_ybsep, m_nseg, m_lpi;
  uint32_t m_xramp, m_yramp;
  int out_s16;
  unsigned long long *stamps;
  int nplanes;
  int comp_b;
  const uint8_t *ref_b[2];
  const void *residual_b;
  uint8_t *out_b;
  int residual_stride_b, out_stride_b;
};
static_assert (sizeof (ObmcJob) == 256, "ObmcJob: four 64-byte scalar loads");

struct SliceJob {
  const uint8_t *data;
  uint32_t data_bytes;
  int pad;
  void *comp[3];
  int stride[3];
  int pad2;
};

struct SliceParams {
  int depth;
  int iwt_lw, iwt_lh, iwt_cw, iwt_ch;
  int nh, nv;
  int n_bytes, remainder, denom;
  int quant_matrix[SCHRO_HIP_LIMIT_SUBBANDS];
  int run_cap;
};

struct EncJob {
  const void *comp[3];
  int stride[3];
  int pad;
  uint8_t *out;
  uint8_t *index;
  uint32_t *overrun;
  uint32_t *est;
  int16_t *recon;
  int16_t *work;
};
struct EncChooseLayout {
  int coef[3];
  int top[3];
  int left[3];
  int row;
  int per_thread;
  int threads, lds_bytes, in_lds;
  int recon_off[3];
};

struct DcJob {
  void *data;
  int stride;
  int w, h;
  int pad;
};

struct DequantJob {
  void *dst;
  const void *src;
  int dst_stride;
  int w, h;
  int src_bytes;
  uint32_t factor, offset;
  int tiles_x;
  int tile_base;
};

struct DequantGeo {
  int dst_offset;
  int dst_stride;
  int w, h;
  int tiles_x;
  int tile_base;
  int plane;
  int rec;
};
struct DequantPlaneDyn {
  void *dst;
  const void *values;
  int is_intra;
  int pad;
};

enum QuantForm {
  kQuantCopy = 0,
  kQuantShift = 1,
  kQuantRecip32 = 2,
  kQuantRecip16 = 3,
  kQuantDivide = 4
};
struct QuantJob {
  void *coeffs;
  void *quant;
  SchroHipCodeblockSummary *summary;
  int stride;
  int w, h;
  int form;
  uint32_t factor;
  uint32_t offset;
  int32_t qoff;
  int shift;
  uint32_t inverse;
  int tiles_x;
  int tile_base;
  int pad;
};
struct QuantDcJob {
  void *coeffs;
  void *quant;
  SchroHipCodeblockSummary *summary;
  int stride;
  int w, h;
  int rec_base, nrec;
  int pad;
};
struct QuantDcRec {
  int x0, y0, x1, y1;
  uint32_t factor, offset;
  int index;
  int pad;
};
struct HistJob {
  const void *base;
  uint32_t *counts;
  int stride;
  int w;
  int skip_shift;
  int dc;
  uint32_t gpr;
  uint32_t items;
  uint32_t step_rows, step_groups;
  int tile_base;
  int pad;
};

constexpr int kMaxJobs = 256;

#ifdef __HIPCC__
#define SCHRO_GLOBAL __attribute__ ((address_space (1)))
typedef uint32_t u32x2 __attribute__ ((ext_vector_type (2)));
typedef uint32_t u32x4 __attribute__ ((ext_vector_type (4)));
typedef uint32_t u32_u __attribute__ ((aligned (1)));
typedef u32x2 u32x2_u __attribute__ ((aligned (1)));
typedef u32x4 u32x4_u __attribute__ ((aligned (1)));

template < typename V, typename P > __device__ __forceinline__ V
gload (const P * p)
{
  return *(const SCHRO_GLOBAL V *) p;
}

template < typename V, typename P > __device__ __forceinline__ void
gstore (P * p, V v)
{
  *(SCHRO_GLOBAL V *) p = v;
}

template < typename T >
__device__ __forceinline__ uint8_t
combine_pred (T s, uint32_t p)
{
  const int v = (int16_t) ((int16_t) s + (int16_t) p);
  return (uint8_t) min (max (v, 0), 255);
}

struct DivMagic {
  uint32_t m[1025];
};
constexpr DivMagic
make_div_magic ()
{
  DivMagic t = { };
  for (uint32_t d = 2; d <= 1024; d++)
    t.m[d] = (uint32_t) ((0x100000000ull + d - 1) / d);
  return t;
}
static __device__ __constant__ DivMagic kDivMagic = make_div_magic ();

__device__ __forceinline__ int
mdiv (int n, int d, uint32_t m)
{
  return d == 1 ? n : (int) __umulhi ((uint32_t) n, m);
}

__device__ __forceinline__ int
fdiv (int n, int d)
{
  if (d > 1024)
    return n / d;
  return d == 1 ? n : (int) __umulhi ((uint32_t) n, kDivMagic.m[d]);
}

__host__ __device__ inline uint32_t
div_magic (int d)
{
  return d <= 1 ? 0u : (uint32_t) ((0x100000000ull + (uint32_t) d - 1) / (uint32_t) d);
}

constexpr int kHpApron = 32;
constexpr int kHpBandRows = 4;

__host__ __device__ __forceinline__ int
hp_chunks (int w, int ps = 0)
{
  return (((w + 2 * kHpApron) << ps) + 15) / 16 + 1;
}

__host__ __device__ __forceinline__ size_t
hp_col_offset (int xp)
{
  return (size_t) (xp >> 4) * 512 + (size_t) (xp & 15);
}

__host__ __device__ __forceinline__ size_t
hp_row_offset (int y, int stride)
{
  return (size_t) (y >> 2) * (size_t) stride + (size_t) ((y & 3) * 32);
}

__host__ __device__ __forceinline__ size_t
hp_offset (int X, int Y, int stride, int ps = 0, int cb = 0)
{
  return hp_row_offset (Y >> 1, stride) + hp_col_offset ((((X >> 1) + kHpApron) << ps) + cb) + (size_t) (((X & 1) + 2 * (Y & 1)) * 128);
}

__device__ __forceinline__ int
xcd_tile_id (int bid, int nblocks)
{
  constexpr int kXcd = 8;
  const int q = nblocks / kXcd, r = nblocks % kXcd;
  const int x = bid % kXcd, k = bid / kXcd;
  return x * q + (x < r ? x : r) + k;
}

template < typename JOB >
__device__ __forceinline__ int
find_job (const JOB * jobs, int njobs, int bid)
{
  const int lane = threadIdx.x & 63;
  int n = 0;
  for (int base = 0; base < njobs; base += 64) {
    const int idx = base + lane;
    const bool le = idx < njobs && gload < int > (&jobs[idx].tile_base) <= bid;
    n += __popcll (__ballot (le));
  }
  return __builtin_amdgcn_readfirstlane (n - 1);
}

template < typename JOB >
__device__ __forceinline__ int
find_dequant_job (const JOB * jobs, int njobs, int bid)
{
  const int lane = threadIdx.x & 63;
  const int *first = reinterpret_cast < const int *>(jobs + njobs);
  const int n64 = (njobs + 63) / 64;
  int lo = 0;
  if (njobs > 4096) {
    const int idx = lane;
    const bool le = idx * 4096 < njobs && gload < int > (first + njobs + n64 + idx) <= bid;
    lo = (__popcll (__ballot (le)) - 1) * 4096;
  }
  if (njobs > 64) {
    const int idx = (lo >> 6) + lane;
    const bool le = idx < n64 && gload < int > (first + njobs + idx) <= bid;
    lo += (__popcll (__ballot (le)) - 1) * 64;
  }
  const int idx = lo + lane;
  const bool le = idx < njobs && gload < int > (first + idx) <= bid;
  return __builtin_amdgcn_readfirstlane (lo + __popcll (__ballot (le)) - 1);
}
#endif

int launch_iiwt_level (hipStream_t stream, const IwtJob * d_jobs, int njobs,
    int total_tiles, int filter, int bpp);

size_t iiwt_fused_job_size (void);
int iiwt_fused_max_levels (int filter, int bpp);
void iiwt_fused_job_fill (void *job, const void *src, int src_stride, int bpp, int nl,
    const void *ll, int ll_stride, void *dst, int dst_stride, int w, int h, int tiles_x,
    int tile_base);
int launch_iiwt_fused (hipStream_t stream, const void *d_jobs, int njobs, int total_tiles,
    int filter, int bpp, int nl);
bool iiwt_haar_supported (int filter, int bpp);
bool iiwt_haar_job_ok (const IwtJob & j);
void iiwt_haar_geometry (int *cols, int *rows);
int launch_iiwt_haar (hipStream_t stream, const IwtJob * d_jobs, int njobs, int total_tiles, int filter);
bool iiwt_haar3_job_ok (const void *src, int src_stride, const void *dst, int dst_stride, int w, int h);
void iiwt_haar3_geometry (int *blocks_x, int *blocks_y);
int launch_iiwt_haar3 (hipStream_t stream, const IwtJob * d_jobs, int njobs, int total_tiles, int filter);
bool iiwt_reg_supported (int filter, int bpp);
void iiwt_reg_geometry (int filter, int small, int *useful_cols, int *useful_row_pairs,
    int *min_row_pairs);
int launch_iiwt_reg (hipStream_t stream, const IwtJob * d_jobs, int njobs, int total_tiles,
    int filter, int small, int combine, int l1_inline = 0);
bool iiwt_reg_l1_supported (int filter);
void iiwt_reg_l1_geometry (int filter, int *useful_cols, int *useful_row_pairs, int *min_row_pairs);
int launch_iiwt_chain (hipStream_t stream, const IwtJob * d_jobs, const uint32_t * d_order, int n_tiles, uint32_t * ctrl,
    uint32_t run, uint32_t * gave_up, uint32_t epoch, int filter);
void iiwt_tile_geometry (int filter, int bpp, int *useful_cols,
    int *useful_row_pairs);
void iwt_fwd_tile_geometry (int filter, int bpp, int *useful_cols, int *useful_row_pairs);
int launch_iwt_fwd_level (hipStream_t stream, const IwtFwdJob * d_jobs, int njobs, int total_tiles, int filter, int bpp);
void downsample_tile_geometry (int *cols, int *rows);
int launch_downsample (hipStream_t stream, const DownsampleJob * d_jobs, int njobs, int total_tiles);
size_t scan_lds_bytes (int bw, int bh, int sw, int sh);
size_t scan_lds_limit ();
int launch_metric_scan (hipStream_t stream, const ScanPicture * d_pics, const ScanJob * d_scans, int nscans, size_t lds_per_wave);
int launch_rough_hint (hipStream_t stream, const RoughChain * d_chains, int nchains, size_t lds_per_wave);
int launch_hier_bm (hipStream_t stream, const HbmChain * d_chains, int nchains, size_t lds_per_wave);
int subpel_error_blocks ();
int launch_subpel_error (hipStream_t stream, const SubpelChain * d_chains, int nchains, int total_groups, int mvprec);
int launch_subpel_choose (hipStream_t stream, const SubpelChain * d_chains, int nchains, int mvprec);
int launch_convert (hipStream_t stream, const ConvertJob * d_jobs, int njobs,
    int total_tiles, int bpp);
void convert_tile_geometry (int *tw, int *th);
int launch_pack (hipStream_t stream, const PackJob * d_jobs, int njobs, int total_tiles);
int launch_shift_right (hipStream_t stream, const ConvertJob * d_jobs, int njobs, int total_tiles, int bpp, int shift);
int launch_add (hipStream_t stream, const ConvertJob * d_jobs, int njobs, int total_tiles, int src_bpp, bool subtract);
void pack_tile_geometry (int *groups_x, int *rows);
int launch_upsample (hipStream_t stream, const UpsampleJob * d_jobs,
    int njobs, int total_tiles, int persist_grid);
void upsample_tile_geometry (int *tw, int *th);
int launch_slices (hipStream_t stream, const SliceJob * d_jobs, int njobs, const SliceParams & P, int bpp, int arith,
    bool aligned16);
bool dc_skew_ok (const DcJob * jobs, int njobs, int bpp);
int launch_dc_predict (hipStream_t stream, const DcJob * d_jobs, int njobs, int max_rows, int bpp,
    unsigned long long *edge, int edge_pitch, uint32_t epoch, uint32_t * gave_up);
int dc_edge_for (SchroHipContext * ctx, int njobs, int max_rows, int max_w, unsigned long long **edge,
    int *edge_pitch, uint32_t * epoch);
int dc_gave_up (SchroHipContext * ctx);
int pred_overflow_poll (SchroHipContext * ctx);
int pred_overflow_claim (SchroHipContext * ctx, uint32_t epoch);
}
extern "C" bool schro_hip_dequant_plan_matches (const SchroHipDequantPlan * plan, const SchroHipDequantPlane * planes, int nplanes, int bpp, int arith);
namespace schro {
bool iiwt_haar3_v210_ok (const HaarPackJob & j);
int iiwt_haar3_v210_strip_width ();
int launch_iiwt_haar3_v210 (hipStream_t stream, const HaarPackJob * d_jobs, int njobs, int total_tiles, int filter);
void iiwt_v210_geometry (int filter, int bpp, int *cols, int *rows);
int launch_iiwt_v210 (hipStream_t stream, const V210Job * d_jobs, int njobs, int total_tiles, int filter, int bpp);
void iiwt_pack8_geometry (int filter, int ayuv, int *cols, int *rows);
int launch_iiwt_pack8 (hipStream_t stream, const Pack8Job * d_jobs, int njobs, int total_tiles, int filter, int ayuv);
void iiwt_wide_geometry (int filter, int v216, int *cols, int *rows);
int launch_iiwt_wide (hipStream_t stream, const WideJob * d_jobs, int njobs, int total_tiles, int filter, int bpp, int v216);
int launch_dequant (hipStream_t stream, const DequantJob * d_jobs, int njobs, int total_tiles, int bpp, int arith);
int launch_dequant_plan (hipStream_t stream, const DequantGeo * d_geo, int njobs, int total_tiles,
    const SchroHipCodeblock * d_recs, const DequantPlaneDyn * d_planes, int bpp, int arith);
void dequant_tile_geometry (int *tw, int *th);
void quant_tile_geometry (int *tw, int *th);
void quant_job_constants (QuantJob * job, int quant_index, int is_intra, int bpp);
int launch_quantise (hipStream_t stream, const QuantJob * d_jobs, int njobs, int total_tiles, int bpp);
int launch_quantise_dc (hipStream_t stream, const QuantDcJob * d_jobs, int njobs, const QuantDcRec * d_recs, int max_rows, int bpp);
int launch_lowdelay_encode (hipStream_t stream, const EncJob * d_jobs, int njobs, const SliceParams & P,
    const EncChooseLayout & L, int stages);
void hist_tile_geometry (int *group_bytes, int *groups_per_tile, int *groups_per_step);
int launch_histogram (hipStream_t stream, const HistJob * d_jobs, int njobs, int total_tiles, int bpp);
int launch_table_copy (hipStream_t stream, void *dst, const void *src, size_t bytes);
void dequant_tables (int quant_index, int is_intra, uint32_t * factor, uint32_t * offset);
int launch_obmc (hipStream_t stream, const ObmcJob * d_jobs, int njobs,
    int total_tiles, int prec, int variant, const uint32_t * d_order, uint32_t * overflow);
struct RowForm {
  int kind, nd, np, ns;
  bool nores, weighted;
  constexpr explicit operator bool () const { return nd != 0; }
  constexpr bool operator== (const RowForm & o) const
  {
    return kind == o.kind && nd == o.nd && np == o.np && ns == o.ns && nores == o.nores && weighted == o.weighted;
  }
};
RowForm obmc_row_form (const ObmcJob & job, bool uv, bool nores);
bool obmc_row_has_kernel (const RowForm & form);
bool obmc_strip_ok (const ObmcJob & j);
void obmc_strip_tiles (const ObmcJob & j, int seg_rows, int *strips, int *segs);
int launch_obmc_strip (hipStream_t stream, const ObmcJob * d_jobs, int njobs, int total_items, int seg_rows, bool nores, uint32_t * overflow,
    int cus);
int obmc_row_tile_width (bool uv);
int obmc_row_tile_height ();
int launch_obmc_row (hipStream_t stream, const ObmcJob * d_jobs, int njobs, int total_tiles, const RowForm & form,
    const uint32_t * d_order, uint32_t * overflow, const uint32_t * d_wtabs);
void obmc_row_tile_record (const ObmcJob & job, bool uv, int ns, int tx, int ty, uint32_t * rec);
int obmc_row_weight_words (int nd, int ns);
void obmc_row_weight_table (const ObmcJob & job, int nd, int ns, bool uv, uint32_t * out);
void obmc_item_geometry (ObmcJob * job);
void obmc_tiles (int variant, int w, int h, int xoff, int *tiles_x, int *tiles_y);

}


namespace schro {
struct FrameQuantTable;
struct FrameHistTable;
}

struct SchroHipContext {
  int device;
  SchroHipMemoryDomain *domain;
  static constexpr int kQueues = 4;
  hipStream_t streams[kQueues];
  hipEvent_t queue_ev[kQueues];
  static constexpr int kMarks = 16;
  hipEvent_t marks[kMarks];
  int cur;
  hipStream_t stream;
  hipEvent_t ev_begin, ev_end;
  bool stage_complete;

  struct Slot {
    void *ptr;
    size_t size;
    bool in_use;
  };
  std::vector < Slot > slots;
  size_t domain_bytes;

  struct ArgSlot {
    uint64_t hash;
    size_t bytes;
    uint64_t last_use;
    hipEvent_t copied;
    bool copy_pending;
  };
  static constexpr int kArgSlots = 256;
  static constexpr size_t kArgSlotBytes = 64u << 10;
  char *h_args;
  char *d_args;
  ArgSlot arg_slots[kArgSlots];
  uint64_t arg_clock;

  bool profile;
  struct EvPair {
    hipEvent_t a, b;
    int cls;
  };
  std::vector < EvPair > ev_pool;
  size_t ev_used;

  struct OrderSlot {
    uint64_t hash;
    uint32_t *d;
    uint32_t *h;
    size_t cap, count;
    uint64_t last_use;
    hipEvent_t copied;
    bool copy_pending;
  };
  static constexpr int kOrderSlots = 16;
  OrderSlot order_slots[kOrderSlots];

  struct ChainSlot {
    uint64_t hash;
    uint32_t *d;
    size_t cap, count;
    uint64_t last_use;
  };
  static constexpr int kChainSlots = 16;
  ChainSlot chain_slots[kChainSlots];
  uint32_t *chain_ctrl[kQueues];
  size_t chain_ctrl_words[kQueues];
  uint64_t chain_ctrl_hash[kQueues];
  uint32_t chain_runs[kQueues];

  void *scratch_q[kQueues];
  size_t scratch_size_q[kQueues];
  void *&scratch_ref () { return scratch_q[cur]; }
  struct BigTable {
    char *h, *d;
    size_t cap;
    hipEvent_t copied;
    bool pending;
  };
  static constexpr int kBigTables = 4;
  BigTable big_q[kQueues][kBigTables];
  int big_turn[kQueues];
  void *dc_edge_q[kQueues];
  size_t dc_edge_size_q[kQueues];
  uint32_t dc_epoch;
  uint32_t *dc_gave_up;
  struct SchroHipDequantPlan *frame_dq_plan;
  void *dq_stage_q[kQueues];
  size_t dq_stage_size_q[kQueues];
  void *pack_tmp_q[kQueues];
  size_t pack_tmp_size_q[kQueues];
  static constexpr int kOvfRing = 12;
  uint32_t pred_epoch;
  uint32_t ovf_epoch[kOvfRing];
  hipEvent_t ovf_ev[kOvfRing];
  std::vector < uint32_t > ovf_unannounced, ovf_unfetched;
  long long obmc_routes[SCHRO_HIP_OBMC_ROUTES] = {};
  long long v210_routes[SCHRO_HIP_V210_ROUTES] = {};
  long long pack8_routes[SCHRO_HIP_PACK8_ROUTES] = {};
  long long wide_routes[SCHRO_HIP_WIDE_ROUTES] = {};
  int cus;
  struct schro::FrameQuantTable *frame_q_table = nullptr;
  struct schro::FrameHistTable *frame_h_table = nullptr;
};

namespace schro {
int push_args (SchroHipContext * ctx, const void *host, size_t bytes,
    void **dev);
int ensure_scratch (SchroHipContext * ctx, size_t bytes);
int push_big_table (SchroHipContext * ctx, const void *host, size_t bytes, void **dev);
int big_table_begin (SchroHipContext * ctx, size_t bytes, void **host, void **dev);
int big_table_commit (SchroHipContext * ctx, size_t bytes);
int copy_2d_async (SchroHipContext * ctx, void *dst, int dst_stride, const void *src, int src_stride, int row_bytes,
    int height, hipMemcpyKind kind);
int iwt_batch_run (SchroHipContext * ctx, const SchroHipIwtFwdPlane * planes, int nplanes, int depth, int filter, int bpp,
    bool in_place);
int rough_scan_nohint_run (SchroHipContext * ctx, const uint8_t * frame, int frame_stride, const uint8_t * ref, int ref_stride,
    int width, int height, int extension, const SchroHipParams * params, int shift, int distance, int ref_index,
    void *motion_vectors);
int rough_me_host_run (SchroHipContext * ctx, const char *who, const SchroHipRoughPlane * levels, int nlevels, int first_shift,
    const SchroHipParams * params, int ref_index, int nohint_distance, int hint_distance, const void *hint, void *const *fields);
int hbm_host_run (SchroHipContext * ctx, const char *who, const SchroHipHbmPlane * levels, int nlevels, int shift, int h_range,
    int with_level0, const SchroHipParams * params, int ref_index, const void *hint, void *const *fields);
int subpel_host_run (SchroHipContext * ctx, SchroHipSubpelChain * chains, int nchains);
bool is_wide_format (int format);
int quantise_batch_run (SchroHipContext * ctx, const SchroHipQuantPlane * planes, int nplanes, int bpp, bool allow_empty);
struct FrameQuantTable {
  std::vector < int >key;
  std::vector < SchroHipCodeblock > recs[3];
  int dc_first[3];
  size_t total;
  SchroHipCodeblockSummary *d_summary;
};
void frame_quant_table_free (SchroHipContext * ctx);
int histogram_batch_run (SchroHipContext * ctx, const SchroHipHistogramPlane * planes, int nplanes, int bpp, bool allow_empty);
struct FrameHistTable {
  std::vector < int >key;
  std::vector < SchroHipHistogramBand > bands[3];
  size_t total;
  SchroHipHistogramCounts *d_counts, *h_counts;
};
void frame_hist_table_free (SchroHipContext * ctx);
struct ProfileScope {
  ProfileScope (SchroHipContext * c, int cls);
  ~ProfileScope ();
};
}
```

Before: 202,800.

## Add tall 64-row OBMC row tiles with 512-thread workgroups for large prediction-only planes

Adds a tall variant of the row OBMC kernel that covers 64 rows per tile with 512 threads, for 3-dword single-segment prediction-only planes of at least 2048 (luma) or 1024 (chroma) rows. The thread count becomes a template parameter across the row body, and the block/item capacities scale with tile height. The aim is to amortise the per-tile setup, the weight-table load and the overlap margin across more rows. In exchange it uses more LDS per workgroup, which can lower occupancy, and it only applies when outputs are not s16.

Result: faster. 205,500, median of 6 (+1.3%).

```diff
diff --git a/schroedinger_amd/csrc/obmc.hip b/schroedinger_amd/csrc/obmc.hip
--- a/schroedinger_amd/csrc/obmc.hip
+++ b/schroedinger_amd/csrc/obmc.hip
@@ -800,8 +800,8 @@
 {
   (void) xoff;
   if (variant >= 1) {
-    const int tw = variant >= 3 ? obmc_row_tile_width (variant == 4) : kFTW;
-    const int th = variant >= 3 ? obmc_row_tile_height () : kFTH;
+    const int tw = variant >= 3 ? obmc_row_tile_width (variant == 4 || variant == 6) : kFTW;
+    const int th = variant >= 3 ? obmc_row_tile_height (variant >= 5) : kFTH;
     *tiles_x = (w + tw - 1) / tw;
     *tiles_y = (h + th - 1) / th;
   } else {
diff --git a/schroedinger_amd/csrc/obmc_row.hip b/schroedinger_amd/csrc/obmc_row.hip
--- a/schroedinger_amd/csrc/obmc_row.hip
+++ b/schroedinger_amd/csrc/obmc_row.hip
@@ -78,6 +78,8 @@
   if (pad && f == obmc_row_kernel_p_3_1_pad_form)
     return obmc_row_kernel_p_3_1_pad;
 #endif
+  if (f.tall)
+    return f.kind == 1 ? row_find (obmc_row_table_tall (), f) : nullptr;
   return row_find (f.kind == 0 ? obmc_row_table_plain () : f.kind == 3 ? obmc_row_table_eighth () : obmc_row_table_half (), f);
 }
 
@@ -96,7 +98,7 @@
     return set_error (SCHRO_HIP_EINVAL, "obmc (row): reference kind %d, %d dwords per row x %d segments x %d planes unsupported", form.kind,
         form.nd, form.ns, form.np);
   static const int lds_pad = SCHRO_ENV ("SCHRO_HIP_OBMC_LDS_PAD") ? atoi (SCHRO_ENV ("SCHRO_HIP_OBMC_LDS_PAD")) : 0;
-  SCHRO_LAUNCH (k, dim3 (total_tiles), dim3 (kRThreads), (size_t) lds_pad, stream, d_jobs, njobs, d_order, overflow, d_wtabs);
+  SCHRO_LAUNCH (k, dim3 (total_tiles), dim3 (form.tall ? kRTallThreads : kRThreads), (size_t) lds_pad, stream, d_jobs, njobs, d_order, overflow, d_wtabs);
   hipError_t e = hipGetLastError ();
   if (e != hipSuccess)
     return set_error (SCHRO_HIP_EDEVICE, "obmc (row) launch: %s", hipGetErrorString (e));
@@ -159,6 +161,26 @@
   if (nbi > 255 || nbi * nbj > caps.blk || nbi * rows_col > caps.item)
     return {};
   return form;
+}
+
+RowForm
+obmc_row_tall_form (const ObmcJob & j, const RowForm & form)
+{
+  if (!form || form.tall || form.ns != 1 || form.nd != 3 || (form.np != 1 && form.np != 3))
+    return {};
+  RowForm tall = form;
+  tall.tall = true;
+  if (!row_kernel (tall))
+    return {};
+  const bool uv = form.np == 3;
+  const int tw = row_caps (3, 1, uv).tw;
+  const int blk = uv ? RowGeoT < 3, true, 1, kRTallTH >::kBlk : RowGeoT < 3, false, 1, kRTallTH >::kBlk;
+  const int item = uv ? RowGeoT < 3, true, 1, kRTallTH >::kItem : RowGeoT < 3, false, 1, kRTallTH >::kItem;
+  const int nbi = (tw - 1 + j.xblen - 1) / j.xbsep + 1, nbj = (kRTallTH - 1 + j.yblen - 1) / j.ybsep + 1;
+  const int rows_col = std::min (kRTallTH * ((j.yblen + j.ybsep - 1) / j.ybsep), kRTallTH + (kRTallTH / j.ybsep + 2) * 2 * j.yoff);
+  if (nbi > 255 || nbj > 255 || nbi * nbj > blk || nbi * rows_col > item)
+    return {};
+  return tall;
 }
 
 int
@@ -232,10 +254,10 @@
 }
 
 void
-obmc_row_tile_record (const ObmcJob & j, bool uv, int ns, int tx, int ty, uint32_t * rec)
-{
-  const int tw = obmc_row_tile_width (uv);
-  const int x_lo = tx * tw, y_lo = ty * kRTH, x_hi = std::min (x_lo + tw, j.w), y_hi = std::min (y_lo + kRTH, j.h);
+obmc_row_tile_record (const ObmcJob & j, bool uv, int ns, int tx, int ty, uint32_t * rec, bool tall)
+{
+  const int tw = obmc_row_tile_width (uv), th = obmc_row_tile_height (tall);
+  const int x_lo = tx * tw, y_lo = ty * th, x_hi = std::min (x_lo + tw, j.w), y_hi = std::min (y_lo + th, j.h);
   const int i_lo = std::max (0, (x_lo + j.xoff - j.xblen + 2 * j.xbsep) / j.xbsep - 1);
   const int i_hi = std::min (j.nbx - 1, (x_hi - 1 + j.xoff) / j.xbsep);
   const int j_lo = std::max (0, (y_lo + j.yoff - j.yblen + 2 * j.ybsep) / j.ybsep - 1);
@@ -248,9 +270,9 @@
 }
 
 int
-obmc_row_tile_height ()
-{
-  return kRTH;
+obmc_row_tile_height (bool tall)
+{
+  return tall ? kRTallTH : kRTH;
 }
 
 int
diff --git a/schroedinger_amd/csrc/obmc_row_body.h b/schroedinger_amd/csrc/obmc_row_body.h
--- a/schroedinger_amd/csrc/obmc_row_body.h
+++ b/schroedinger_amd/csrc/obmc_row_body.h
@@ -11,6 +11,7 @@
 
 constexpr int kRThreads = 256;
 constexpr int kRTH = 32;
+constexpr int kRTallTH = 64, kRTallThreads = 512;
 template < int ND, bool UV, int NS = 1 > struct RowGeo {
   static constexpr int kTW = UV ? 64 : 128;
   static constexpr int kMargin = UV ? (ND <= 3 && NS == 1 ? 5 : 8) : (ND <= 2 ? 8 : 16);
@@ -23,6 +24,9 @@
   static constexpr bool kPadBlk = UV || ND > 2;
   static constexpr int kWFoldY = kWCap + 4 * kXF, kWRampX = kWFoldY + 128, kWRampY = kWRampX + kWxN;
   static constexpr int kWTab = kWRampY + 32;
+};
+template < int ND, bool UV, int NS, int TH > struct RowGeoT : RowGeo < ND, UV, NS > {
+  static constexpr int kBlk = RowGeo < ND, UV, NS >::kBlk * TH / kRTH, kItem = RowGeo < ND, UV, NS >::kItem * TH / kRTH;
 };
 constexpr int kRBoth = 0, kRRef0 = 1, kRRef1 = 2, kRDc = 3, kREdge = 4, kRRim = 5;
 constexpr int kRSlots = 16 + 4 + 4 + 3;
@@ -528,14 +532,14 @@
   }
 }
 
-template < int ND, bool UV, int CLS, int RK, int NS, bool WP, bool PAD = false >
+template < int ND, bool UV, int CLS, int RK, int NS, bool WP, bool PAD = false, int NT = kRThreads >
 __device__ __forceinline__ void
 row_class (const ObmcJob & job, int pl, const RowRefs & refs, const uint16_t * s_item, const RowBlkT < RowGeo < ND, UV, NS >::kPadBlk > *s_hot,
     const uint32_t * s_wp, uint32_t * acc, int par, int lo, int hi, bool exact, int *turn)
 {
   const int wave = __builtin_amdgcn_readfirstlane ((int) (threadIdx.x >> 6)), lane = threadIdx.x & 63;
   const int npass = (hi - lo + 63) >> 6;
-  constexpr int kWaves = kRThreads / 64;
+  constexpr int kWaves = NT / 64;
   const int k0 = (wave - *turn) & (kWaves - 1);
   *turn = (*turn + npass) & (kWaves - 1);
 #if defined (SCHRO_HIP_EXPERIMENTS) && defined (SCHRO_ROW_PRIO_PASS)
@@ -635,16 +639,16 @@
       && ((((uintptr_t) io.out) | (uintptr_t) io.out_stride) & 7) == 0;
 }
 
-template < int TH, typename G > constexpr int kRFinishRounds = (TH * (G::kTW / 8) + kRThreads - 1) / kRThreads;
-
-template < int TH, typename G, int STEP, int FIRST >
+template < int TH, typename G, int NT = kRThreads > constexpr int kRFinishRounds = (TH * (G::kTW / 8) + NT - 1) / NT;
+
+template < int TH, typename G, int STEP, int FIRST, int NT = kRThreads >
 __device__ __forceinline__ void
 row_finish_prefetch (const PlaneIO & io, int tid, int x_lo, int y_lo, int y_hi, u32x4 * res)
 {
   constexpr int kG = G::kTW / 8;
 #pragma unroll
-  for (int n = 0; n < kRFinishRounds < TH, G >; n++) {
-    const int it = tid + n * kRThreads, g = it & (kG - 1), y = y_lo + it / kG;
+  for (int n = 0; n < kRFinishRounds < TH, G, NT >; n++) {
+    const int it = tid + n * NT, g = it & (kG - 1), y = y_lo + it / kG;
     if (!io.residual)
       res[STEP * n + FIRST] = (u32x4) { 0u, 0u, 0u, 0u };
     else if (y < y_hi && it < TH * kG)
@@ -652,12 +656,12 @@
   }
 }
 
-template < int TH, typename G, bool UV >
+template < int TH, typename G, bool UV, int NT = kRThreads >
 __device__ __forceinline__ void
 row_finish_plain (const ObmcJob & job, const PlaneIO & io, int cb, const uint32_t * acc, int par, int tid, int x_lo, int y_lo,
     int x_hi, int y_hi)
 {
-  for (int it = tid; it < TH * G::kTW; it += kRThreads) {
+  for (int it = tid; it < TH * G::kTW; it += NT) {
     const int xx = it & (G::kTW - 1), yy = it / G::kTW;
     const int x = x_lo + xx, y = y_lo + yy;
     if (y >= y_hi || x >= x_hi)
@@ -677,7 +681,7 @@
   }
 }
 
-template < int TH, typename G, bool NOCLAMP = false >
+template < int TH, typename G, bool NOCLAMP = false, int NT = kRThreads >
 __device__ __forceinline__ void
 row_finish (const ObmcJob & job, const PlaneIO & io, uint32_t * acc, int par, int tid, int x_lo, int y_lo,
     int x_hi, int y_hi, bool fast, const u32x4 * res)
@@ -685,8 +689,8 @@
   constexpr int kG = G::kTW / 8;
   if (fast) {
 #pragma unroll
-    for (int n = 0; n < kRFinishRounds < TH, G >; n++) {
-      const int it = tid + n * kRThreads;
+    for (int n = 0; n < kRFinishRounds < TH, G, NT >; n++) {
+      const int it = tid + n * NT;
       const int g = it & (kG - 1), yy = it / kG;
       const int y = y_lo + yy;
       if (y >= y_hi || it >= TH * kG)
@@ -724,17 +728,17 @@
     }
     return;
   }
-  row_finish_plain < TH, G, false > (job, io, 0, acc, par, tid, x_lo, y_lo, x_hi, y_hi);
-}
-
-template < int TH, typename G, bool NOCLAMP = false >
+  row_finish_plain < TH, G, false, NT > (job, io, 0, acc, par, tid, x_lo, y_lo, x_hi, y_hi);
+}
+
+template < int TH, typename G, bool NOCLAMP = false, int NT = kRThreads >
 __device__ __forceinline__ void
 row_finish_uv (const PlaneIO & iou, const PlaneIO & iov, const uint32_t * acc, int tid, int x_lo, int y_lo, int y_hi, const u32x4 * res)
 {
   constexpr int kG = G::kTW / 8;
 #pragma unroll
-  for (int n = 0; n < kRFinishRounds < TH, G >; n++) {
-    const int it = tid + n * kRThreads;
+  for (int n = 0; n < kRFinishRounds < TH, G, NT >; n++) {
+    const int it = tid + n * NT;
     const int g = it & (kG - 1), yy = it / kG;
     const int y = y_lo + yy;
     if (y >= y_hi || it >= TH * kG)
@@ -772,11 +776,11 @@
   return x_hi - x_lo == G::kTW && ((((uintptr_t) io.out) | (uintptr_t) io.out_stride) & 15) == 0;
 }
 
-template < int TH, typename G, bool UV >
+template < int TH, typename G, bool UV, int NT = kRThreads >
 __device__ __forceinline__ void
 row_finish_s16_plain (const PlaneIO & io, int cb, const uint32_t * acc, int par, int tid, int x_lo, int y_lo, int x_hi, int y_hi)
 {
-  for (int it = tid; it < TH * G::kTW; it += kRThreads) {
+  for (int it = tid; it < TH * G::kTW; it += NT) {
     const int xx = it & (G::kTW - 1), yy = it / G::kTW;
     const int x = x_lo + xx, y = y_lo + yy;
     if (y >= y_hi || x >= x_hi)
@@ -790,15 +794,15 @@
   }
 }
 
-template < int TH, typename G >
+template < int TH, typename G, int NT = kRThreads >
 __device__ __forceinline__ void
 row_finish_s16 (const PlaneIO & io, const uint32_t * acc, int par, int tid, int x_lo, int y_lo, int x_hi, int y_hi, bool fast)
 {
   constexpr int kG = G::kTW / 8;
   if (fast) {
 #pragma unroll
-    for (int n = 0; n < kRFinishRounds < TH, G >; n++) {
-      const int it = tid + n * kRThreads;
+    for (int n = 0; n < kRFinishRounds < TH, G, NT >; n++) {
+      const int it = tid + n * NT;
       const int g = it & (kG - 1), yy = it / kG;
       const int y = y_lo + yy;
       if (y >= y_hi || it >= TH * kG)
@@ -827,17 +831,17 @@
     }
     return;
   }
-  row_finish_s16_plain < TH, G, false > (io, 0, acc, par, tid, x_lo, y_lo, x_hi, y_hi);
-}
-
-template < int TH, typename G >
+  row_finish_s16_plain < TH, G, false, NT > (io, 0, acc, par, tid, x_lo, y_lo, x_hi, y_hi);
+}
+
+template < int TH, typename G, int NT = kRThreads >
 __device__ __forceinline__ void
 row_finish_s16_uv (const PlaneIO & iou, const PlaneIO & iov, const uint32_t * acc, int tid, int x_lo, int y_lo, int y_hi)
 {
   constexpr int kG = G::kTW / 8;
 #pragma unroll
-  for (int n = 0; n < kRFinishRounds < TH, G >; n++) {
-    const int it = tid + n * kRThreads;
+  for (int n = 0; n < kRFinishRounds < TH, G, NT >; n++) {
+    const int it = tid + n * NT;
     const int g = it & (kG - 1), yy = it / kG;
     const int y = y_lo + yy;
     if (y >= y_hi || it >= TH * kG)
@@ -864,13 +868,15 @@
 
 constexpr int kRPadItems = 344;
 
-template < int ND, int NP, bool UV = false, int TH = kRTH, bool NORES = false, int RK = 1, int NS = 1, bool WP = false, bool PAD = false >
+template < int ND, int NP, bool UV = false, int TH = kRTH, bool NORES = false, int RK = 1, int NS = 1, bool WP = false, bool PAD = false, int NT = kRThreads >
 __device__ __forceinline__ void
 obmc_row_body (const ObmcJob * __restrict__ jobs, int njobs, const uint32_t * __restrict__ order, uint32_t * __restrict__ overflow,
     const uint32_t * __restrict__ wtabs)
 {
-  typedef RowGeo < ND, UV, NS > G;
+  typedef RowGeoT < ND, UV, NS, TH > G;
   static_assert (!UV || NP == 1, "a UV job is one virtual plane of (U, V) samples");
+  static_assert (NT >= 256 && NT % 64 == 0 && (NT & (NT - 1)) == 0, "whole waves, a power of two of them (row_class's turn)");
+  static_assert (G::kBlk <= 512 && G::kItem + (PAD ? kRPadItems : 0) <= 2048 && TH <= 128 && (G::kAccW & 1), "a tile's tables fit their packed fields");
   static_assert (NS == 1 || (NS == 2 && (ND == 3 || ND == 4)), "segments: halves of 12 or 16 bytes");
   constexpr int kRTW = G::kTW, ps = UV ? 1 : 0;
   __shared__ __attribute__ ((aligned (16))) uint32_t acc[TH * G::kAccW + 3];
@@ -944,16 +950,16 @@
   for (int rep_ = 0; rep_ < kRepSetup; rep_++) {
   if (rep_)
     __syncthreads ();
-  for (int it = tid; it < kAccQuads; it += kRThreads)
+  for (int it = tid; it < kAccQuads; it += NT)
     reinterpret_cast < u32x4 * >(acc)[it] = (u32x4) { 0u, 0u, 0u, 0u };
-  constexpr int kWQuads = G::kWTab / 4, kWQ = (kWQuads + kRThreads / 2 - 1) / (kRThreads / 2);
+  constexpr int kWQuads = G::kWTab / 4, kWQ = (kWQuads + NT / 2 - 1) / (NT / 2);
   static_assert (G::kWTab % 4 == 0 && kWQ <= 2, "one or two quads of the weight table per lane of the last two waves");
   u32x4 wq[kWQ];
 #pragma unroll
   for (int n = 0; n < kWQ; n++) {
     wq[n] = (u32x4) { 0u, 0u, 0u, 0u };
-    const int q = tid - kRThreads / 2 + n * (kRThreads / 2);
-    if (tid >= kRThreads / 2 && q < kWQuads)
+    const int q = tid - NT / 2 + n * (NT / 2);
+    if (tid >= NT / 2 && q < kWQuads)
       wq[n] = gload < u32x4 > (wtabs + (size_t) job.ipw * G::kWTab + 4 * q);
   }
   if (tid >= 128 && tid < 128 + kRSlots)
@@ -999,17 +1005,17 @@
     RSTAMP (8);
 #pragma unroll
     for (int n = 0; n < kWQ; n++) {
-      const int q = tid - kRThreads / 2 + n * (kRThreads / 2);
-      if (tid >= kRThreads / 2 && q < kWQuads)
+      const int q = tid - NT / 2 + n * (NT / 2);
+      if (tid >= NT / 2 && q < kWQuads)
         reinterpret_cast < u32x4 * >(s_wp)[q] = wq[n];
     }
     RSTAMP (1);
-    for (int blk = tid; blk < nblk; blk += kRThreads) {
+    for (int blk = tid; blk < nblk; blk += NT) {
       const int bj = nbi == 1 ? blk : (int) (((uint32_t) blk * m16_nbi) >> 16);
       const int vi = blk - bj * nbi, seg = NS > 1 ? vi % NS : 0;
       const int i = i_lo + vi / NS, jj = j_lo + bj;
       uint32_t flags = mv_pre[0], v01 = mv_pre[1], v23 = mv_pre[2];
-      if (blk >= kRThreads) {
+      if (blk >= NT) {
         const uint8_t *mvp = job.mvs + (size_t) 20 * ((size_t) jj * job.nbx + i);
         flags = gload < uint32_t > (mvp);
         v01 = gload < uint32_t > (mvp + 12);
@@ -1146,7 +1152,7 @@
 #pragma unroll
   for (int c = 0; c <= kRRim; c++)
     ibase[c] = __builtin_amdgcn_readlane (sbase, row_slot_base (c));
-  for (int b0 = 0; b0 < nblk; b0 += kRThreads) {
+  for (int b0 = 0; b0 < nblk; b0 += NT) {
     const int blk = b0 + tid;
     const bool have = blk < nblk;
     const int meta = have ? s_meta[blk] : 0, slot = meta & 31;
@@ -1216,14 +1222,14 @@
     const bool s16 = !NORES && job.out_s16;
     const bool fast = s16 ? row_finish_s16_is_fast < G > (io, x_lo, x_hi) && (!UV || row_finish_s16_is_fast < G > (iov, x_lo, x_hi))
         : row_finish_is_fast < G > (job, io, x_lo, x_hi) && (!UV || row_finish_is_fast < G > (job, iov, x_lo, x_hi));
-    constexpr int kRounds = kRFinishRounds < TH, G >;
+    constexpr int kRounds = kRFinishRounds < TH, G, NT >;
     u32x4 res[UV ? 2 * kRounds : kRounds];
 #define SCHRO_ROW_PREFETCH() do { \
       if constexpr (UV) { \
-        row_finish_prefetch < TH, G, 2, 0 > (io, tid, x_lo, y_lo, y_hi, res); \
-        row_finish_prefetch < TH, G, 2, 1 > (iov, tid, x_lo, y_lo, y_hi, res); \
+        row_finish_prefetch < TH, G, 2, 0, NT > (io, tid, x_lo, y_lo, y_hi, res); \
+        row_finish_prefetch < TH, G, 2, 1, NT > (iov, tid, x_lo, y_lo, y_hi, res); \
       } else { \
-        row_finish_prefetch < TH, G, 1, 0 > (io, tid, x_lo, y_lo, y_hi, res); \
+        row_finish_prefetch < TH, G, 1, 0, NT > (io, tid, x_lo, y_lo, y_hi, res); \
       } } while (0)
     if constexpr (kEarlyRes) {
       if (fast)
@@ -1242,7 +1248,7 @@
       if constexpr (UV && RK == 0)
         refs.rsrc_b[r] = __builtin_amdgcn_make_buffer_rsrc ((void *) iov.ref[r], 0, (int) bytes, 0x00020000);
     }
-#define SCHRO_ROW_CLASS(C) row_class < ND, UV, C, RK, NS, WP, PAD > (job, pl, refs, s_item, s_hot, s_wp, acc, par, \
+#define SCHRO_ROW_CLASS(C) row_class < ND, UV, C, RK, NS, WP, PAD, NT > (job, pl, refs, s_item, s_hot, s_wp, acc, par, \
     ibase[C], ibase[C + 1], exact, &turn)
 #pragma unroll
     for (int rep_ = 0; rep_ < kRepPasses; rep_++) {
@@ -1257,7 +1263,7 @@
     if (nrim > 0) {
       const int nseg = (xblen + 3) >> 2, per_block = yblen * nseg;
       const uint32_t m_per_block = div_magic (per_block), m_nseg = div_magic (nseg);
-      for (int item = tid; item < nrim * per_block; item += kRThreads) {
+      for (int item = tid; item < nrim * per_block; item += NT) {
         const int b = mdiv (item, per_block, m_per_block);
         const int rem = item - b * per_block;
         const int r2 = mdiv (rem, nseg, m_nseg), s2 = rem - r2 * nseg;
@@ -1302,33 +1308,33 @@
     if (s16) {
       if constexpr (UV) {
         if (fast) {
-          row_finish_s16_uv < TH, G > (io, iov, acc, tid, x_lo, y_lo, y_hi);
+          row_finish_s16_uv < TH, G, NT > (io, iov, acc, tid, x_lo, y_lo, y_hi);
         } else {
-          row_finish_s16_plain < TH, G, true > (io, 0, acc, par, tid, x_lo, y_lo, x_hi, y_hi);
-          row_finish_s16_plain < TH, G, true > (iov, 1, acc, par, tid, x_lo, y_lo, x_hi, y_hi);
+          row_finish_s16_plain < TH, G, true, NT > (io, 0, acc, par, tid, x_lo, y_lo, x_hi, y_hi);
+          row_finish_s16_plain < TH, G, true, NT > (iov, 1, acc, par, tid, x_lo, y_lo, x_hi, y_hi);
         }
       } else {
-        row_finish_s16 < TH, G > (io, acc, par, tid, x_lo, y_lo, x_hi, y_hi, fast);
+        row_finish_s16 < TH, G, NT > (io, acc, par, tid, x_lo, y_lo, x_hi, y_hi, fast);
       }
     } else if constexpr (UV) {
       if (fast) {
         if (NORES && !exact)
-          row_finish_uv < TH, G, NORES > (io, iov, acc, tid, x_lo, y_lo, y_hi, res);
+          row_finish_uv < TH, G, NORES, NT > (io, iov, acc, tid, x_lo, y_lo, y_hi, res);
         else
-          row_finish_uv < TH, G > (io, iov, acc, tid, x_lo, y_lo, y_hi, res);
+          row_finish_uv < TH, G, false, NT > (io, iov, acc, tid, x_lo, y_lo, y_hi, res);
       } else {
-        row_finish_plain < TH, G, true > (job, io, 0, acc, par, tid, x_lo, y_lo, x_hi, y_hi);
-        row_finish_plain < TH, G, true > (job, iov, 1, acc, par, tid, x_lo, y_lo, x_hi, y_hi);
+        row_finish_plain < TH, G, true, NT > (job, io, 0, acc, par, tid, x_lo, y_lo, x_hi, y_hi);
+        row_finish_plain < TH, G, true, NT > (job, iov, 1, acc, par, tid, x_lo, y_lo, x_hi, y_hi);
       }
     } else {
       if (NORES && !exact)
-        row_finish < TH, G, NORES > (job, io, acc, par, tid, x_lo, y_lo, x_hi, y_hi, fast, res);
+        row_finish < TH, G, NORES, NT > (job, io, acc, par, tid, x_lo, y_lo, x_hi, y_hi, fast, res);
       else
-        row_finish < TH, G > (job, io, acc, par, tid, x_lo, y_lo, x_hi, y_hi, fast, res);
+        row_finish < TH, G, false, NT > (job, io, acc, par, tid, x_lo, y_lo, x_hi, y_hi, fast, res);
     }
     if (pl + 1 < nplanes) {
       __syncthreads ();
-      for (int it = tid; it < kAccQuads; it += kRThreads)
+      for (int it = tid; it < kAccQuads; it += NT)
         reinterpret_cast < u32x4 * >(acc)[it] = (u32x4) { 0u, 0u, 0u, 0u };
       __syncthreads ();
     }
@@ -1347,11 +1353,12 @@
 #undef RSTAMP
 }
 
-template < int ND, int NP, bool UV = false, int TH = kRTH, bool NORES = false, int RK = 1, int NS = 1, bool WP = false, bool PAD = false >
+template < int ND, int NP, bool UV = false, int TH = kRTH, bool NORES = false, int RK = 1, int NS = 1, bool WP = false, bool PAD = false, int NT = kRThreads >
 constexpr RowForm
 row_form ()
 {
-  return RowForm { RK, ND, UV ? 3 : NP, NS, NORES, WP };
+  static_assert ((TH == kRTallTH) == (NT == kRTallThreads), "tall tiles go with the tall workgroup");
+  return RowForm { RK, ND, UV ? 3 : NP, NS, NORES, WP, TH == kRTallTH };
 }
 
 #define SCHRO_ROW_KERNEL(name, waves, ...) \
@@ -1377,6 +1384,7 @@
   int n;
 };
 RowTable obmc_row_table_half (), obmc_row_table_plain (), obmc_row_table_eighth ();
+RowTable obmc_row_table_tall ();
 
 constexpr RowKernel
 row_find (const RowTable & t, const RowForm & f)
diff --git a/schroedinger_amd/csrc/obmc_row_tall.hip b/schroedinger_amd/csrc/obmc_row_tall.hip
--- /dev/null
+++ b/schroedinger_amd/csrc/obmc_row_tall.hip
@@ -0,0 +1,43 @@
+
+#include "obmc_row_body.h"
+
+namespace schro {
+namespace {
+
+#define SCHRO_ROW_TALL_KERNEL(name, waves, ND, UV, NORES) \
+__global__ __launch_bounds__ (kRTallThreads) __attribute__ ((amdgpu_waves_per_eu (waves, waves))) \
+void name (const ObmcJob * __restrict__ jobs, int njobs, const uint32_t * __restrict__ order, uint32_t * __restrict__ overflow, \
+    const uint32_t * __restrict__ wtabs) \
+{ \
+  obmc_row_body < ND, 1, UV, kRTallTH, NORES, 1, 1, false, false, kRTallThreads > (jobs, njobs, order, overflow, wtabs); \
+} \
+constexpr RowForm name##_form = row_form < ND, 1, UV, kRTallTH, NORES, 1, 1, false, false, kRTallThreads > ();
+
+SCHRO_ROW_TALL_KERNEL (obmc_row_tall_p_3_1, 8, 3, false, true)
+SCHRO_ROW_TALL_KERNEL (obmc_row_tall_p_uv_3, 8, 3, true, true)
+#ifdef SCHRO_HIP_EXPERIMENTS
+SCHRO_ROW_TALL_KERNEL (obmc_row_tall_3_1, 6, 3, false, false)
+SCHRO_ROW_TALL_KERNEL (obmc_row_tall_uv_3, 6, 3, true, false)
+#endif
+
+constexpr RowEntry kTall[] = {
+  ROW_ENTRY (obmc_row_tall_p_3_1), ROW_ENTRY (obmc_row_tall_p_uv_3),
+#ifdef SCHRO_HIP_EXPERIMENTS
+  ROW_ENTRY (obmc_row_tall_3_1), ROW_ENTRY (obmc_row_tall_uv_3),
+#endif
+};
+constexpr RowTable kTallTable = { kTall, (int) std::size (kTall) };
+static_assert (row_table_ok (kTallTable, 1), "obmc_row_tall.hip: one kernel per form");
+static_assert (obmc_row_tall_p_3_1_form.tall && obmc_row_tall_p_uv_3_form.np == 3 && obmc_row_tall_p_uv_3_form.tall, "obmc_row_tall.hip: tall forms");
+static_assert (row_find (kTallTable, RowForm { 1, 3, 1, 1, true, false, true }) == obmc_row_tall_p_3_1
+    && !row_find (kTallTable, RowForm { 1, 3, 1, 1, true, false, false }), "obmc_row_tall.hip: found by tall forms only");
+
+}
+
+RowTable
+obmc_row_table_tall ()
+{
+  return kTallTable;
+}
+
+}
diff --git a/schroedinger_amd/csrc/plane_obmc.cpp b/schroedinger_amd/csrc/plane_obmc.cpp
--- a/schroedinger_amd/csrc/plane_obmc.cpp
+++ b/schroedinger_amd/csrc/plane_obmc.cpp
@@ -17,6 +17,19 @@
 {
   static const int mode = SCHRO_ENV ("SCHRO_HIP_OBMC_MERGE") ? atoi (SCHRO_ENV ("SCHRO_HIP_OBMC_MERGE")) : 1;
   return mode;
+}
+
+constexpr int kTallMinHeight[2] = { 2048, 1024 };
+static bool
+obmc_tall_wanted (const ObmcJob & j, bool uv, bool pred_only)
+{
+#ifdef SCHRO_HIP_EXPERIMENTS
+  static const int forced = SCHRO_ENV ("SCHRO_HIP_OBMC_TALL") ? atoi (SCHRO_ENV ("SCHRO_HIP_OBMC_TALL")) : -1;
+  if (forced >= 0)
+    return forced != 0;
+#endif
+  const int min_h = kTallMinHeight[uv ? 1 : 0];
+  return pred_only && min_h > 0 && j.h >= min_h;
 }
 
 static unsigned long long *g_stamps;
@@ -165,8 +178,9 @@
     static const int sup_x = SCHRO_ENV ("SCHRO_HIP_OBMC_SUPER_X") ? std::max (1, atoi (SCHRO_ENV ("SCHRO_HIP_OBMC_SUPER_X"))) : 4;
     static const int sup_y = SCHRO_ENV ("SCHRO_HIP_OBMC_SUPER_Y") ? std::max (1, atoi (SCHRO_ENV ("SCHRO_HIP_OBMC_SUPER_Y"))) : 4;
     for (size_t j = 0; j < jobs.size (); j++) {
-      const int sx = variant == 4 ? sup_x : jobs[j].nplanes == 2 ? std::max (1, sup_x / 2) : sup_x;
-      const int sy = variant == 4 ? std::max (1, sup_y / 2) : sup_y;
+      const bool pair_tiles = variant == 4 || variant == 6;
+      const int sx = pair_tiles ? sup_x : jobs[j].nplanes == 2 ? std::max (1, sup_x / 2) : sup_x;
+      const int sy = pair_tiles ? std::max (1, sup_y / 2) : sup_y;
       const int nsx = div_up (jobs[j].tiles_x, sx);
       for (int ty = 0; ty < tiles_y[j]; ty++)
         for (int tx = 0; tx < jobs[j].tiles_x; tx++)
@@ -232,7 +246,7 @@
       if (row) {
         const ObmcJob & g = jobs[keys[k].entry >> 16];
         const int t = (int) (keys[k].entry & 0xffffu);
-        obmc_row_tile_record (g, row_uv != 0, row_ns, t % g.tiles_x, t / g.tiles_x, &slot->h[k * words + 1]);
+        obmc_row_tile_record (g, row_uv != 0, row_ns, t % g.tiles_x, t / g.tiles_x, &slot->h[k * words + 1], variant >= 5);
       }
     }
     SCHRO_HIP_CHECK (hipMemcpyAsync (slot->d, slot->h, keys.size () * words * sizeof (uint32_t), hipMemcpyHostToDevice,
@@ -389,6 +403,13 @@
       }
     }
   }
+  for (int p = 0; p < nplanes; p++) {
+    const RowForm tall = key[p].out_s16 ? RowForm {} : obmc_row_tall_form (all[p], key[p].form);
+    if (tall && obmc_tall_wanted (all[p], tall.np == 3, key[p].pred_only)) {
+      key[p].form = tall;
+      key[p].variant = tall.np == 3 ? 6 : 5;
+    }
+  }
   std::vector < char >done (nplanes, 0);
   for (int first = 0; first < nplanes; first++) {
     if (done[first])
@@ -445,7 +466,7 @@
     }
 #ifdef SCHRO_HIP_EXPERIMENTS
     static const bool use_strip = SCHRO_ENV ("SCHRO_HIP_OBMC_STRIP") && atoi (SCHRO_ENV ("SCHRO_HIP_OBMC_STRIP")) != 0;
-    bool strip = use_strip && row && form.np == 1 && form.nd == 3 && form.ns == 1;
+    bool strip = use_strip && row && !form.tall && form.np == 1 && form.nd == 3 && form.ns == 1;
     for (size_t k = 0; strip && k < jobs.size (); k++)
       strip = obmc_strip_ok (jobs[k]);
     if (strip) {
diff --git a/schroedinger_amd/csrc/schro_hip_internal.h b/schroedinger_amd/csrc/schro_hip_internal.h
--- a/schroedinger_amd/csrc/schro_hip_internal.h
+++ b/schroedinger_amd/csrc/schro_hip_internal.h
@@ -671,23 +671,25 @@
 struct RowForm {
   int kind, nd, np, ns;
   bool nores, weighted;
+  bool tall = false;
   constexpr explicit operator bool () const { return nd != 0; }
   constexpr bool operator== (const RowForm & o) const
   {
-    return kind == o.kind && nd == o.nd && np == o.np && ns == o.ns && nores == o.nores && weighted == o.weighted;
+    return kind == o.kind && nd == o.nd && np == o.np && ns == o.ns && nores == o.nores && weighted == o.weighted && tall == o.tall;
   }
 };
 RowForm obmc_row_form (const ObmcJob & job, bool uv, bool nores);
 bool obmc_row_has_kernel (const RowForm & form);
+RowForm obmc_row_tall_form (const ObmcJob & job, const RowForm & form);
 bool obmc_strip_ok (const ObmcJob & j);
 void obmc_strip_tiles (const ObmcJob & j, int seg_rows, int *strips, int *segs);
 int launch_obmc_strip (hipStream_t stream, const ObmcJob * d_jobs, int njobs, int total_items, int seg_rows, bool nores, uint32_t * overflow,
     int cus);
 int obmc_row_tile_width (bool uv);
-int obmc_row_tile_height ();
+int obmc_row_tile_height (bool tall = false);
 int launch_obmc_row (hipStream_t stream, const ObmcJob * d_jobs, int njobs, int total_tiles, const RowForm & form,
     const uint32_t * d_order, uint32_t * overflow, const uint32_t * d_wtabs);
-void obmc_row_tile_record (const ObmcJob & job, bool uv, int ns, int tx, int ty, uint32_t * rec);
+void obmc_row_tile_record (const ObmcJob & job, bool uv, int ns, int tx, int ty, uint32_t * rec, bool tall = false);
 int obmc_row_weight_words (int nd, int ns);
 void obmc_row_weight_table (const ObmcJob & job, int nd, int ns, bool uv, uint32_t * out);
 void obmc_item_geometry (ObmcJob * job);
```
